# freewym/espresso

Measured on AMD Instinct MI355X. Metric: audio-hours/sec training (LibriSpeech Conformer-12 + CTC), higher is better.
Workload: dtype bf16; 1 GPU; LibriSpeech 960h Conformer-12 + CTC update step, <=26000 frames & <=24 utts per GPU, V=5004, on-GPU fbank+CMVN+SpecAugment, dropout 0.1, clip 2.0, Adam; parallelism=dp1

## Files before the change

### espresso_amd/_lib.py

```python
import ctypes
import os
import re
from typing import Dict, List, Tuple

_HERE = os.path.dirname(os.path.abspath(__file__))
HEADER_PATH = os.path.join(os.path.dirname(_HERE), "include", "espresso_amd.h")
LIB_PATH = os.path.join(_HERE, "csrc", "libespresso_amd.so")


class EspressoAmdLibraryError(RuntimeError):
    pass


class EaGemmParams(ctypes.Structure):
    _fields_ = [
        ("A", ctypes.c_void_p),
        ("B", ctypes.c_void_p),
        ("C", ctypes.c_void_p),
        ("C2", ctypes.c_void_p),
        ("bias", ctypes.c_void_p),
        ("resid", ctypes.c_void_p),
        ("aux", ctypes.c_void_p),
        ("M", ctypes.c_int),
        ("N", ctypes.c_int),
        ("K", ctypes.c_int),
        ("batch", ctypes.c_int),
        ("zdiv", ctypes.c_int),
        ("a_kstrided", ctypes.c_int),
        ("b_kstrided", ctypes.c_int),
        ("c_f32", ctypes.c_int),
        ("accumulate", ctypes.c_int),
        ("resid_f32", ctypes.c_int),
        ("act", ctypes.c_int),
        ("lda", ctypes.c_long),
        ("ldb", ctypes.c_long),
        ("ldc", ctypes.c_long),
        ("ldc2", ctypes.c_long),
        ("ldr", ctypes.c_long),
        ("ldaux", ctypes.c_long),
        ("sA_hi", ctypes.c_long),
        ("sA_lo", ctypes.c_long),
        ("sB_hi", ctypes.c_long),
        ("sB_lo", ctypes.c_long),
        ("sC_hi", ctypes.c_long),
        ("sC_lo", ctypes.c_long),
        ("sR_hi", ctypes.c_long),
        ("sR_lo", ctypes.c_long),
        ("sX_hi", ctypes.c_long),
        ("sX_lo", ctypes.c_long),
        ("alpha", ctypes.c_float),
        ("out_scale", ctypes.c_float),
        ("drop_seed", ctypes.c_uint64),
        ("drop_thr", ctypes.c_uint32),
        ("drop_scale", ctypes.c_float),
        ("splitk", ctypes.c_int),
        ("kchunk", ctypes.c_int),
        ("workspace", ctypes.c_void_p),
        ("q_u", ctypes.c_void_p),
        ("q_v", ctypes.c_void_p),
        ("pos_u", ctypes.c_void_p),
        ("pos_v", ctypes.c_void_p),
        ("ld_q", ctypes.c_long),
        ("qsplit_n", ctypes.c_int),
        ("qscale", ctypes.c_float),
    ]


_F, _V = ctypes.c_void_p, ctypes.c_void_p


def _mk(name, fields):
    return type(name, (ctypes.Structure,), {"_fields_": [(f, ctypes.c_void_p) for f in fields]})


EaFfnParams = _mk("EaFfnParams", ["ln_g", "ln_b", "w1", "b1", "w2", "b2"])
EaFfnGrads = _mk("EaFfnGrads", ["ln_g", "ln_b", "w1", "b1", "w2", "b2"])
EaAttnParams = _mk("EaAttnParams", ["ln_g", "ln_b", "wqkv", "bqkv", "wo", "bo", "pos_u", "pos_v", "wpos"])
EaAttnGrads = _mk("EaAttnGrads", ["ln_g", "ln_b", "wqkv", "bqkv", "wo", "bo", "pos_u", "pos_v", "wpos"])
EaConvParams = _mk("EaConvParams", ["ln_g", "ln_b", "pw1", "dw", "bn_g", "bn_b", "bn_rm", "bn_rv", "pw2"])
EaConvGrads = _mk("EaConvGrads", ["ln_g", "ln_b", "pw1", "dw", "bn_g", "bn_b", "pw2"])


class EaLayerGrads(ctypes.Structure):
    _fields_ = [("ffn1", EaFfnGrads), ("attn", EaAttnGrads), ("conv", EaConvGrads), ("ffn2", EaFfnGrads),
                ("final_ln_g", ctypes.c_void_p), ("final_ln_b", ctypes.c_void_p)]


class EaConformerLayer(ctypes.Structure):
    _fields_ = [("ffn1", EaFfnParams), ("attn", EaAttnParams), ("conv", EaConvParams), ("ffn2", EaFfnParams),
                ("final_ln_g", ctypes.c_void_p), ("final_ln_b", ctypes.c_void_p), ("grads", EaLayerGrads), ("wt", ctypes.c_void_p)]


class EaLayerShape(ctypes.Structure):
    _fields_ = [("B", ctypes.c_int), ("T", ctypes.c_int), ("C", ctypes.c_int), ("H", ctypes.c_int), ("F", ctypes.c_int),
                ("KW", ctypes.c_int), ("training", ctypes.c_int), ("p_drop", ctypes.c_float), ("p_act", ctypes.c_float),
                ("p_attn", ctypes.c_float), ("seed", ctypes.c_uint64), ("has_attn_mask", ctypes.c_int), ("scratch_clean", ctypes.c_int),
                ("pos_mode", ctypes.c_int), ("act", ctypes.c_int), ("S", ctypes.c_int), ("defer", ctypes.c_int), ("wt_fresh", ctypes.c_int)]


class EaLayerChain(ctypes.Structure):
    _fields_ = [("next", ctypes.c_void_p), ("next_saved", ctypes.c_void_p), ("next_saved_bytes", ctypes.c_long), ("ln1_done", ctypes.c_int),
                ("prev", ctypes.c_void_p), ("prev_saved", ctypes.c_void_p), ("prev_saved_bytes", ctypes.c_long),
                ("prev_seed", ctypes.c_uint64), ("prev_pre", ctypes.c_void_p), ("final_ln_done", ctypes.c_int), ("pre_in", ctypes.c_void_p)]


class EaStackLayer(ctypes.Structure):
    _fields_ = [("layer", ctypes.c_void_p), ("shape", EaLayerShape), ("saved", ctypes.c_void_p), ("saved_bytes", ctypes.c_long),
                ("x_in", ctypes.c_void_p)]


class EaWgradProblem(ctypes.Structure):
    _fields_ = [("dy", ctypes.c_void_p), ("x", ctypes.c_void_p), ("dW", ctypes.c_void_p), ("dbias", ctypes.c_void_p),
                ("M", ctypes.c_int), ("N", ctypes.c_int), ("K", ctypes.c_int), ("ld_dy", ctypes.c_long), ("ld_x", ctypes.c_long),
                ("ldw", ctypes.c_long)]


class EaWgradGroup(ctypes.Structure):
    _fields_ = [("count", ctypes.c_int), ("p", EaWgradProblem * 16)]


EaXAttnParams = _mk("EaXAttnParams", ["ln_g", "ln_b", "wq", "bq", "wkv", "bkv", "wo", "bo"])
EaXAttnGrads = _mk("EaXAttnGrads", ["ln_g", "ln_b", "wq", "bq", "wkv", "bkv", "wo", "bo"])


class EaDecoderLayer(ctypes.Structure):
    _fields_ = [("self_attn", EaAttnParams), ("cross", EaXAttnParams), ("ffn", EaFfnParams), ("g_self", EaAttnGrads),
                ("g_cross", EaXAttnGrads), ("g_ffn", EaFfnGrads), ("wt", ctypes.c_void_p)]


_SCALARS = {
    "int": ctypes.c_int,
    "long": ctypes.c_long,
    "float": ctypes.c_float,
    "uint64_t": ctypes.c_uint64,
    "uint32_t": ctypes.c_uint32,
    "ea_stream_t": ctypes.c_void_p,
}


def _ctype_of(decl: str):
    decl = decl.strip()
    if "*" in decl:
        if "EaGemmParams" in decl:
            return ctypes.POINTER(EaGemmParams)
        return ctypes.c_void_p
    toks = [t for t in decl.replace("const", " ").split() if t]
    ty = toks[0]
# ... 50 lines not shown
```

### espresso_amd/csrc/convmodule.hip

```cpp
#include "common.h"
#include "espresso_amd.h"

namespace {

constexpr int KMAX = 31;

__device__ __forceinline__ float sigmoid_f(float x) { return __builtin_amdgcn_rcpf(1.f + __expf(-x)); }

constexpr int CT = 64, TTILE = 64, TPT = TTILE / 4;

template <int KW>
__global__ __launch_bounds__(256) void glu_dwconv_fwd_kernel(const bf16_t* __restrict__ Y,
                                                             const float* __restrict__ w,
                                                             bf16_t* __restrict__ U, bf16_t* __restrict__ Z,
                                                             double* __restrict__ stats, int T, int C) {
  constexpr int PAD = (KW - 1) / 2, ROWS = TTILE + KW - 1;
  __shared__ __attribute__((aligned(16))) float su[ROWS][CT];
  __shared__ float sred[2][4][CT];
  const int c0 = blockIdx.x * CT, t0 = blockIdx.y * TTILE, b = blockIdx.z;
  const long rowbase = (long)b * T;
  if ((C & 7) == 0 && c0 + CT <= C) {
    bf16_t (*sub)[CT] = reinterpret_cast<bf16_t (*)[CT]>(&su[0][0]);
    bf16_t (*sz)[CT] = reinterpret_cast<bf16_t (*)[CT]>(&su[0][0]) + ROWS;
    constexpr int NCH = (ROWS * (CT / 8) + 255) / 256;
// ... 817 lines not shown
        *reinterpret_cast<uint4*>(&tile[wave][r * 128 + (((c8 >> 1) ^ c1_sw(r)) << 5) + (c8 & 1) * 16]) = o;
      }
      uint32_t bh[4], bl[4];
#pragma unroll
      for (int j = 0; j < 8; ++j) {
        const int k = 8 * g4 + j;
        float x = xv[j] ? xs[j] : 0.f;
        if (li == 9 && pb + k < npos) x = 1.f;
        const uint32_t hi = (uint32_t)f2bf(x);
        const uint32_t lo = (uint32_t)f2bf(x - __uint_as_float(hi << 16));
        if (j & 1) { bh[j >> 1] |= hi << 16; bl[j >> 1] |= lo << 16; }
        else { bh[j >> 1] = hi; bl[j >> 1] = lo; }
      }
      __builtin_amdgcn_fence(__ATOMIC_RELEASE, "wavefront");
      __builtin_amdgcn_wave_barrier();
      __builtin_amdgcn_fence(__ATOMIC_ACQUIRE, "wavefront");
      uint32_t ad[8];
      uint2 o8[8];
#pragma unroll
      for (int mt = 0; mt < 4; ++mt)
#pragma unroll
        for (int h = 0; h < 2; ++h) {
          const int r = 8 * g4 + 4 * h + (li >> 2);
          ad[mt * 2 + h] = lds0 + r * 128 + ((mt ^ c1_sw(r)) << 5) + (li & 3) * 8;
        }
      c1_tr_read8(ad, o8);
      const bf16x8_t vbh = __builtin_bit_cast(bf16x8_t, make_uint4(bh[0], bh[1], bh[2], bh[3]));
      const bf16x8_t vbl = __builtin_bit_cast(bf16x8_t, make_uint4(bl[0], bl[1], bl[2], bl[3]));
#pragma unroll
      for (int mt = 0; mt < 4; ++mt) {
        const bf16x8_t a8 = __builtin_bit_cast(bf16x8_t, make_uint4(o8[mt * 2].x, o8[mt * 2].y, o8[mt * 2 + 1].x, o8[mt * 2 + 1].y));
        acc[mt] = __builtin_amdgcn_mfma_f32_16x16x32_bf16(__builtin_bit_cast(__attribute__((ext_vector_type(8))) __bf16, a8),
                                                          __builtin_bit_cast(__attribute__((ext_vector_type(8))) __bf16, vbh), acc[mt], 0, 0, 0);
        acc[mt] = __builtin_amdgcn_mfma_f32_16x16x32_bf16(__builtin_bit_cast(__attribute__((ext_vector_type(8))) __bf16, a8),
                                                          __builtin_bit_cast(__attribute__((ext_vector_type(8))) __bf16, vbl), acc[mt], 0, 0, 0);
      }
      __builtin_amdgcn_wave_barrier();
    }
#pragma unroll
    for (int mt = 0; mt < 4; ++mt)
#pragma unroll
      for (int r = 0; r < 4; ++r) sred[wave][mt * 16 + g4 * 4 + r][li] = acc[mt][r];
    __syncthreads();
    for (int i = threadIdx.x; i < 64 * 10; i += 256) {
      const int c = i / 10, k = i % 10;
      const float a = sred[0][c][k] + sred[1][c][k] + sred[2][c][k] + sred[3][c][k];
      if (k < 9) atomicAdd(dW + (cs + c) * 9 + k, a);
      else if (dbias) atomicAdd(dbias + cs + c, a);
    }
    __syncthreads();
  }
}

__global__ void bn_param_grad_kernel(const float* __restrict__ red, float* __restrict__ dgamma, float* __restrict__ dbeta, int C) {
  const int c = blockIdx.x * blockDim.x + threadIdx.x;
  if (c >= C) return;
  if (dbeta) dbeta[c] += red[c];
  if (dgamma) dgamma[c] += red[C + c];
}
}

static void launch_bn_bwd_reduce(const void* Z, const void* dH, const float* mean_rstd, const float* gamma, const float* beta,
                                 float* red, long M, int C, int act, hipStream_t stream);

extern "C" int ea_bn_act_bwd(const void* Z, const void* dH, const float* mean_rstd, const float* gamma,
                             const float* beta, float* red, void* dZ, float* dgamma, float* dbeta, long M, int C,
                             int act, int training, hipStream_t stream) {
  if (M <= 0) return 0;
  if (C % 8) return -2;
  launch_bn_bwd_reduce(Z, dH, mean_rstd, gamma, beta, red, M, C, act, stream);
  hipLaunchKernelGGL(bn_act_bwd_apply_kernel, dim3(egrid_ch(M * (C / 8), C / 8)), dim3(256), 0, stream, (const bf16_t*)Z,
                     (const bf16_t*)dH, mean_rstd, gamma, beta, red, (bf16_t*)dZ, M, C, act,
                     training ? (float)M : 0.f);
  if (dgamma || dbeta) hipLaunchKernelGGL(bn_param_grad_kernel, dim3((C + 255) / 256), dim3(256), 0, stream, red, dgamma, dbeta, C);
  return EA_CHECK_LAUNCH();
}

extern "C" int ea_bn_act_bwd_fused(const void* Z, const void* dH, const float* mean_rstd, const float* gamma, const float* beta,
                                   float* red, void* dZ, float* dgamma, float* dbeta, long M, int C, int act, int training,
                                   float* zero_next, int zero_n, hipStream_t stream) {
  if (M <= 0) return 0;
  if (C % 8) return -2;
  launch_bn_bwd_reduce(Z, dH, mean_rstd, gamma, beta, red, M, C, act, stream);
  hipLaunchKernelGGL(bn_act_bwd_apply_kernel, dim3(egrid_ch(M * (C / 8), C / 8)), dim3(256), 0, stream, (const bf16_t*)Z,
                     (const bf16_t*)dH, mean_rstd, gamma, beta, red, (bf16_t*)dZ, M, C, act, training ? (float)M : 0.f, dgamma, dbeta,
                     zero_next, zero_n);
  return EA_CHECK_LAUNCH();
}

extern "C" int ea_conv1_bn_bwd(const float* X, const void* Z, const void* dH, const float* mean_rstd, const float* gamma,
                               const float* beta, float* red, float* dgamma, float* dbeta, float* dW, float* dbias, int B, int T,
                               int F, int CO, int sy, int sx, int act, int training, hipStream_t stream) {
  if (B <= 0 || T <= 0) return 0;
  if (CO % 64) return -2;
  const int To = (T - 1) / sy + 1, Fo = (F - 1) / sx + 1;
  const long npos = (long)B * To * Fo;
  launch_bn_bwd_reduce(Z, dH, mean_rstd, gamma, beta, red, npos, CO, act, stream);
  long nb = (npos + 127) / 128;
  if (nb > 1024) nb = 1024;
  hipLaunchKernelGGL(conv1_bn_bwd_wgrad_kernel, dim3((unsigned)nb), dim3(256), 0, stream, X, (const bf16_t*)Z,
                     (const bf16_t*)dH, mean_rstd, gamma, beta, red, dW, dbias, T, F, To, Fo, CO, sy, sx, npos, act,
                     training ? (float)npos : 0.f);
  if (dgamma || dbeta) hipLaunchKernelGGL(bn_param_grad_kernel, dim3((CO + 255) / 256), dim3(256), 0, stream, red, dgamma, dbeta, CO);
  return EA_CHECK_LAUNCH();
}

static void launch_bn_bwd_reduce(const void* Z, const void* dH, const float* mean_rstd, const float* gamma, const float* beta,
                                 float* red, long M, int C, int act, hipStream_t stream) {
  const int nch = C / 8;
  int TCH = 1;
  while (TCH < 256 && TCH < nch) TCH <<= 1;
  const int lanes = 256 / TCH;
  int rpb = 8 * lanes;
  if (rpb < 32) rpb = 32;
  const long gx = (nch + TCH - 1) / TCH;
  const long want = (M + (2048 / gx) - 1) / (2048 / gx > 0 ? 2048 / gx : 1);
  if (want > rpb) rpb = (int)((want + lanes - 1) / lanes * lanes);
  dim3 g1((unsigned)gx, (unsigned)((M + rpb - 1) / rpb));
  hipLaunchKernelGGL(bn_act_bwd_reduce_kernel, g1, dim3(256), (size_t)256 * 16 * sizeof(float), stream, (const bf16_t*)Z,
                     (const bf16_t*)dH, mean_rstd, gamma, beta, red, M, C, act, rpb, TCH);
}
extern "C" int ea_bn_param_grad(const float* red, float* dgamma, float* dbeta, int C, hipStream_t stream) {
  hipLaunchKernelGGL(bn_param_grad_kernel, dim3((C + 255) / 256), dim3(256), 0, stream, red, dgamma, dbeta, C);
  return EA_CHECK_LAUNCH();
}

constexpr int DW_TILES_PER_BLOCK = 2;
static inline int dw_time_blocks(int T) {
  const int nt = (T + TTILE - 1) / TTILE;
  return (nt + DW_TILES_PER_BLOCK - 1) / DW_TILES_PER_BLOCK;
}
extern "C" long ea_dwconv_wgrad_workspace_bytes(int B, int T, int C, int KW) {
  return (long)B * dw_time_blocks(T) * C * KW * (long)sizeof(float);
}

extern "C" int ea_glu_dwconv_bwd(const void* dZ, const void* Y, const void* U, const float* w, void* dY, float* dw,
                                 void* wgrad_ws, int B, int T, int C, int KW, hipStream_t stream) {
  if (B <= 0 || T <= 0) return 0;
  if (C % 2) return -2;
  dim3 grid((C + CT - 1) / CT, (T + TTILE - 1) / TTILE, B);
  EA_KW_DISPATCH(KW, launch_glu_dwconv_bwd_data, grid, stream, (const bf16_t*)dZ, (const bf16_t*)Y, w, (bf16_t*)dY, T, C);
  if (!dw) return EA_CHECK_LAUNCH();
  return ea_dwconv_bwd_weight(dZ, U, dw, wgrad_ws, B, T, C, KW, stream);
}
extern "C" int ea_bn_glu_dwconv_bwd_fused(const void* Z, const void* dH, const float* mean_rstd, const float* gamma, const float* beta,
                                          float* red, void* dZ, float* dgamma, float* dbeta, int act, int training, float* zero_next,
                                          int zero_n, const void* Y, const float* w, void* dY, int B, int T, int C, int KW,
                                          hipStream_t stream) {
  if (B <= 0 || T <= 0) return 0;
  const long M = (long)B * T;
  static const bool fuse = [] { const char* e = getenv("EA_BN_GLU_BWD_FUSED"); return e && e[0] == '1'; }();
  if (!fuse || C % CT != 0) {
    const int rc = ea_bn_act_bwd_fused(Z, dH, mean_rstd, gamma, beta, red, dZ, dgamma, dbeta, M, C, act, training, zero_next, zero_n, stream);
    return rc ? rc : ea_glu_dwconv_bwd(dZ, Y, nullptr, w, dY, nullptr, nullptr, B, T, C, KW, stream);
  }
  launch_bn_bwd_reduce(Z, dH, mean_rstd, gamma, beta, red, M, C, act, stream);
  BnBwdFuse fb{(const bf16_t*)Z, (const bf16_t*)dH, mean_rstd, gamma, beta, red, (bf16_t*)dZ, training ? (float)M : 0.f, act, dgamma, dbeta,
               zero_next, zero_n};
  dim3 grid(C / CT, (T + TTILE - 1) / TTILE, B);
  EA_KW_DISPATCH(KW, launch_glu_dwconv_bwd_data_bn, grid, stream, (const bf16_t*)Y, w, (bf16_t*)dY, T, C, fb);
  return EA_CHECK_LAUNCH();
}
extern "C" int ea_dwconv_bwd_weight(const void* dZ, const void* U, float* dw, void* wgrad_ws, int B, int T, int C, int KW,
                                    hipStream_t stream) {
  if (B <= 0 || T <= 0) return 0;
  dim3 gridw((C + CT - 1) / CT, dw_time_blocks(T), B);
  float* part = (float*)wgrad_ws;
  EA_KW_DISPATCH(KW, launch_dwconv_bwd_weight, gridw, stream, (const bf16_t*)dZ, (const bf16_t*)U, part, T, C, DW_TILES_PER_BLOCK);
  const int nslab = (int)(gridw.y * gridw.z);
  hipLaunchKernelGGL(dwconv_weight_reduce_kernel, dim3((C * KW + 255) / 256, nslab >= 16 ? 8 : 1), dim3(256), 0, stream, part, dw,
                     nslab, C * KW);
  return EA_CHECK_LAUNCH();
}
```

### espresso_amd/csrc/engine.hip

```cpp
#include <hip/hip_runtime.h>
#include <stdint.h>
#include <stdlib.h>
#include <string.h>

#include <functional>
#include <cstdio>
#include <map>
#include <mutex>
#include <vector>

#include "espresso_amd.h"

void ea_gemm_corun_hint(int on);

namespace {

struct Arena {
  char* base;
  size_t off;
  size_t peak;
  template <typename T>
  T* get(size_t n) {
    off = (off + 255) & ~(size_t)255;
    T* p = base ? reinterpret_cast<T*>(base + off) : nullptr;
    off += n * sizeof(T);
    if (off > peak) peak = off;
    return p;
  }
};

inline int pad8(int n) { return (n + 7) / 8 * 8; }
inline int pad_bd(int r) { return (r + 127) / 128 * 128; }

constexpr uint64_t kFfn1 = 0, kAttn = 16, kConv = 32, kCross = 32, kFfn2 = 48;
constexpr uint64_t kAct = 1, kOut = 2, kProbs = 3, kAttnOut = 4, kConvOut = 5;

struct Deferred {
  EaWgradGroup grp;
  EaLnReduceGroup ln;
  std::vector<std::function<int(hipStream_t)>> pre;
  std::vector<std::function<int(hipStream_t)>> ops;
  Deferred() { clear(); }
  void clear() { grp.count = 0; ln.count = 0; pre.clear(); ops.clear(); }
};

struct Ctx {
  hipStream_t s;
  bool dry;
  int rc;
  Arena* scratch;
  hipStream_t side;
  bool overlap;
  Deferred* df = nullptr;
  const EaLayerChain* chain = nullptr;
  bool bits_early = false;
  bool pp_early = false;
};

#define RUN(call)                         \
  do {                                    \
    if (!c.dry && c.rc == 0) c.rc = (call); \
  } while (0)

struct SideRes {
  hipStream_t stream = nullptr;
  hipEvent_t ev[32];
  int next = 0;
  bool ok = false;
  hipEvent_t done[2];
  bool pending[2] = {false, false};
};
static SideRes g_side;
__global__ void ea_queue_probe_spin(long ticks) {
  const long t0 = (long)wall_clock64();
  while ((long)wall_clock64() - t0 < ticks) __builtin_amdgcn_s_sleep(16);
}
__global__ void ea_queue_probe_nop() {}
}
extern "C" int ea_streams_share_queue(hipStream_t a, hipStream_t b) {
  if (a == b) return 1;
  hipEvent_t a0, a1, b1;
  if (hipEventCreate(&a0) != hipSuccess) return -1;
  if (hipEventCreate(&a1) != hipSuccess) { (void)hipEventDestroy(a0); return -1; }
  if (hipEventCreate(&b1) != hipSuccess) { (void)hipEventDestroy(a0); (void)hipEventDestroy(a1); return -1; }
  int rc = -1;
  float spin_ms = 0.f, b_ms = 0.f;
  hipLaunchKernelGGL(ea_queue_probe_nop, dim3(1), dim3(64), 0, b);
  if (hipStreamSynchronize(b) == hipSuccess && hipEventRecord(a0, a) == hipSuccess) {
    hipLaunchKernelGGL(ea_queue_probe_spin, dim3(1), dim3(64), 0, a, 20000L);
// ... 22 lines not shown
  bool ok = false;
  for (int t = 0; t < 8; ++t) {
    hipStream_t cand = nullptr;
    if (hipStreamCreateWithFlags(&cand, hipStreamNonBlocking) != hipSuccess) break;
    const bool unprobed = !g_side_probe || t == 7;
    if (unprobed || ea_streams_share_queue(owner, cand) != 1) {
      g_side.stream = cand;
      g_side_rejected = nrej;
      g_side_unprobed = unprobed ? 1 : 0;
      ok = true;
      break;
    }
    rejected[nrej++] = cand;
  }
  for (int i = 0; i < nrej; ++i) (void)hipStreamDestroy(rejected[i]);
  return ok;
}
static bool side_init(hipStream_t owner) {
  if (g_side.ok) return true;
  int cur = 0, dev = 0;
  if (hipGetDevice(&cur) != hipSuccess) return false;
  dev = cur;
  if (owner != nullptr) {
    hipDevice_t d;
    if (hipStreamGetDevice(owner, &d) == hipSuccess) dev = (int)d;
  }
  if (dev != cur && hipSetDevice(dev) != hipSuccess) return false;
  bool ok = side_stream_create(owner);
  for (auto& e : g_side.ev)
    ok = ok && hipEventCreateWithFlags(&e, hipEventDisableTiming) == hipSuccess;
  for (auto& e : g_side.done)
    ok = ok && hipEventCreateWithFlags(&e, hipEventDisableTiming) == hipSuccess;
  if (dev != cur) (void)hipSetDevice(cur);
  g_side.ok = ok;
  return ok;
}
static inline void stream_wait(Ctx& c, hipStream_t dst, hipStream_t src) {
  if (c.dry || c.rc != 0) return;
  hipEvent_t e = g_side.ev[g_side.next];
  g_side.next = (g_side.next + 1) % 32;
  if (hipEventRecord(e, src) != hipSuccess || hipStreamWaitEvent(dst, e, 0) != hipSuccess) c.rc = -1;
}
static inline void* ln_ws(Ctx& c, int M, int C) {
  return c.scratch->get<char>((size_t)ea_layernorm_bwd_workspace_bytes(M, C));
}
static inline hipStream_t wstream(Ctx& c) { return c.overlap ? c.side : c.s; }
static inline void fork(Ctx& c) { if (c.overlap && !c.df) stream_wait(c, c.side, c.s); }
static inline int join_half(hipStream_t main, int h) {
  if (!g_side.ok || !g_side.pending[h]) return 0;
  g_side.pending[h] = false;
  return hipStreamWaitEvent(main, g_side.done[h], 0) == hipSuccess ? 0 : -1;
}
static inline int join_all(hipStream_t main) {
  const int a = join_half(main, 0), b = join_half(main, 1);
  return a ? a : b;
}
static inline void release(Ctx& c, size_t mark) { if (!c.overlap) c.scratch->off = mark; }

inline uint32_t drop_thr(float p) {
  if (p <= 0.f) return 0;
  double t = (double)p * 4294967296.0;
  return t >= 4294967295.0 ? 4294967295u : (uint32_t)t;
}
inline float drop_scale(float p) { return p <= 0.f ? 1.f : 1.f / (1.f - p); }

struct G {
  EaGemmParams p;
  G(const void* A, const void* B, void* C, int M, int N, int K, long lda, long ldb, long ldc) {
    memset(&p, 0, sizeof(p));
    p.A = A; p.B = B; p.C = C; p.M = M; p.N = N; p.K = K; p.lda = lda; p.ldb = ldb; p.ldc = ldc;
    p.batch = 1; p.zdiv = 1; p.alpha = 1.f; p.out_scale = 1.f; p.splitk = 1; p.drop_scale = 1.f;
  }
  G& aks() { p.a_kstrided = 1; return *this; }
  G& bks() { p.b_kstrided = 1; return *this; }
  G& f32() { p.c_f32 = 1; return *this; }
  G& acc() { p.accumulate = 1; return *this; }
  G& bias(const float* b) { p.bias = b; return *this; }
  G& act(int a) { p.act = a; return *this; }
  G& alpha(float a) { p.alpha = a; return *this; }
  G& scale(float a) { p.out_scale = a; return *this; }
  G& resid(const void* r, long ldr) { p.resid = r; p.ldr = ldr; return *this; }
  G& c2(void* c, long ld) { p.C2 = c; p.ldc2 = ld; return *this; }
  G& aux(const void* x, long ld) { p.aux = x; p.ldaux = ld; return *this; }
  G& drop(float pr, uint64_t seed) { p.drop_thr = drop_thr(pr); p.drop_scale = drop_scale(pr); p.drop_seed = seed; return *this; }
  bool qsplit(void* q_u, void* q_v, const float* pos_u, const float* pos_v, int n, long ld_q, float s) {
    static const bool off = getenv("EA_NO_QSPLIT") != nullptr;
    if (off || n % 128 || p.N % 8) return false;
    p.q_u = q_u; p.q_v = q_v; p.pos_u = pos_u; p.pos_v = pos_v; p.qsplit_n = n; p.ld_q = ld_q; p.qscale = s;
    return true;
  }
  G& batch(int b, int zdiv, long ahi, long alo, long bhi, long blo, long chi, long clo) {
    p.batch = b; p.zdiv = zdiv; p.sA_hi = ahi; p.sA_lo = alo; p.sB_hi = bhi; p.sB_lo = blo; p.sC_hi = chi; p.sC_lo = clo;
    return *this;
  }
};

inline void gemm(Ctx& c, G& g) {
  if (!c.dry && c.rc == 0) ea_gemm_corun_hint(c.overlap || c.df != nullptr);
  RUN(ea_gemm_bf16(&g.p, c.s));
  if (!c.dry) ea_gemm_corun_hint(0);
}
inline void gemm_on(Ctx& c, G& g, hipStream_t st) { RUN(ea_gemm_bf16(&g.p, st)); }

inline void bias_grad(Ctx& c, const void* X, float* out, int M, int N, long ld) {
  if (c.df) {
    if (!c.dry) c.df->ops.push_back([=](hipStream_t st) { return ea_colsum_bf16(X, out, M, N, ld, st); });
    return;
  }
  RUN(ea_colsum_bf16(X, out, M, N, ld, wstream(c)));
}
inline void wgrad(Ctx& c, const void* dy, long ld_dy, const void* x, long ld_x, float* dW, int M, int N_out, int K_in,
                  float* dbias = nullptr) {
  if (c.df && c.df->grp.count < EA_WGRAD_MAX) {
    EaWgradProblem& q = c.df->grp.p[c.df->grp.count++];
    if (c.dry) return;
    q.dy = dy; q.x = x; q.dW = dW; q.dbias = dbias; q.M = M; q.N = N_out; q.K = K_in; q.ld_dy = ld_dy; q.ld_x = ld_x; q.ldw = K_in;
    return;
  }
  const int tiles = ((N_out + 63) / 64) * ((K_in + 127) / 128);
  int sk = 1;
  if (tiles < 384 && M >= 1024) {
    sk = (512 + tiles - 1) / tiles;
    if (sk > M / 256) sk = M / 256;
    if (sk < 1) sk = 1;
  }
  G g(dy, x, dW, N_out, K_in, M, ld_dy, ld_x, K_in);
  g.aks().bks().f32().acc();
  g.p.splitk = sk;
  if (sk > 1) g.p.workspace = c.scratch->get<float>((size_t)sk * N_out * K_in);
  if (c.df) {
    const EaGemmParams gp = g.p;
    if (!c.dry) c.df->ops.push_back([=](hipStream_t st) { return ea_gemm_bf16(&gp, st); });
  } else {
    gemm_on(c, g, wstream(c));
  }
  if (dbias) bias_grad(c, dy, dbias, M, N_out, ld_dy);
}
static bool g_defer_default = true;
static bool g_defer_inline = false;
static void run_deferred(Ctx& c, int half) {
  if (c.dry || !c.df) return;
  Deferred& d = *c.df;
  if (g_defer_inline) {
    RUN(ea_wgrad_group(&d.grp, c.s));
    RUN(ea_layernorm_param_reduce_group(&d.ln, c.s));
    for (auto& op : d.ops) RUN(op(c.s));
    d.clear();
    return;
  }
  stream_wait(c, c.side, c.s);
  for (auto& op : d.pre) RUN(op(c.side));
  RUN(ea_wgrad_group(&d.grp, c.side));
  RUN(ea_layernorm_param_reduce_group(&d.ln, c.side));
  for (auto& op : d.ops) RUN(op(c.side));
  d.clear();
  if (c.rc == 0) {
    if (hipEventRecord(g_side.done[half], c.side) != hipSuccess) c.rc = -1;
    g_side.pending[half] = true;
  }
  if (c.rc == 0) c.rc = join_half(c.s, half ^ 1);
}

}

extern "C" {

struct WT {
  const uint16_t *f1w1, *f2w1, *wqkv, *wo, *pw1, *pw2, *f1w2, *f2w2;
};
static WT wt_view(const EaConformerLayer* L, const EaLayerShape& sh) {
  WT w{nullptr, nullptr, nullptr, nullptr, nullptr, nullptr, nullptr, nullptr};
  if (!L->wt || !sh.training) return w;
  const size_t C = sh.C, F = sh.F;
  const uint16_t* p = (const uint16_t*)L->wt;
  w.f1w1 = p; p += C * F;
  w.f2w1 = p; p += C * F;
  w.wqkv = p; p += 3 * C * C;
  w.wo = p; p += C * C;
  w.pw1 = p; p += 2 * C * C;
  w.pw2 = p; p += C * C;
  w.f1w2 = p; p += C * F;
  w.f2w2 = p;
  return w;
}
static void wt_refresh(Ctx& c, const EaConformerLayer* L, const EaLayerShape& sh) {
  const WT w = wt_view(L, sh);
  if (!w.f1w1) return;
  const int C = sh.C, F = sh.F;
  const void* src[8] = {L->ffn1.w1, L->ffn2.w1, L->attn.wqkv, L->attn.wo, L->conv.pw1, L->conv.pw2, L->ffn1.w2, L->ffn2.w2};
  void* dst[8] = {(void*)w.f1w1, (void*)w.f2w1, (void*)w.wqkv, (void*)w.wo, (void*)w.pw1, (void*)w.pw2, (void*)w.f1w2, (void*)w.f2w2};
  const int rows[8] = {F, F, 3 * C, C, 2 * C, C, C, C}, cols[8] = {C, C, C, C, C, C, F, F};
  RUN(ea_transpose_bf16_batch(src, dst, rows, cols, 8, c.s));
}
struct Pre {
  uint16_t* buf;
  float a;
  uint64_t seed;
  float p;
};
static inline void ln_param_reduce(Ctx& c, void* lnws, float* dg, float* db, int M, int C) {
  if (c.df) {
    if (c.dry) return;
    if (c.df->ln.count < EA_LNRED_MAX) {
      EaLnReduceItem& it = c.df->ln.item[c.df->ln.count++];
      it.workspace = lnws; it.dgamma = dg; it.dbeta = db; it.M = M; it.C = C;
    } else {
      c.df->ops.push_back([=](hipStream_t st) { return ea_layernorm_param_reduce(lnws, dg, db, M, C, st); });
    }
    return;
  }
  fork(c);
  RUN(ea_layernorm_param_reduce(lnws, dg, db, M, C, wstream(c)));
}
static inline void ln_bwd_block(Ctx& c, const void* x, const void* dxn, const float* gamma, const float* mean, const float* rstd,
                                void* dx, float* dg, float* db, int M, int C, const void* dx_add, const Pre& next) {
  void* lnws = ln_ws(c, M, C);
  if (next.buf)
    RUN(ea_layernorm_bwd_dx2(x, dxn, gamma, mean, rstd, dx, dg, db, M, C, dx_add, lnws, next.buf, next.a, next.seed, drop_thr(next.p),
                             drop_scale(next.p), c.s));
  else
    RUN(ea_layernorm_bwd_dx(x, dxn, gamma, mean, rstd, dx, dg, db, M, C, nullptr, 0, 0, 1.f, dx_add, lnws, c.s));
  ln_param_reduce(c, lnws, dg, db, M, C);
// ... 382 lines not shown
    R.cap = cap;
    R.ok = true;
  }
  if (C > R.cap) return nullptr;
  if (R.dirty) {
    const size_t bytes = 2 * (size_t)(2 * R.cap) * (sizeof(double) + sizeof(float));
    if (hipMemsetAsync(R.st[0], 0, bytes, owner) != hipSuccess) return nullptr;
    R.dirty = false;
  }
  return &R;
}

struct ConvSaved {
  float *mean, *rstd, *mr;
  uint16_t *xn, *Y, *U, *Z, *Hh;
};
static ConvSaved conv_saved(Arena& sv, const EaLayerShape& sh) {
  const int M = sh.B * sh.T, C = sh.C;
  ConvSaved s;
  s.mean = sv.get<float>(M);
  s.rstd = sv.get<float>(M);
  s.mr = sv.get<float>(2 * C);
  s.xn = sv.get<uint16_t>((size_t)M * C);
  s.Y = sv.get<uint16_t>((size_t)M * 2 * C);
  s.U = sv.get<uint16_t>((size_t)M * C);
  s.Z = sv.get<uint16_t>((size_t)M * C);
  s.Hh = sv.get<uint16_t>((size_t)M * C);
  return s;
}

static void conv_fwd(Ctx& c, const ConvSaved& s, const EaLayerShape& sh, const EaConvParams& w, const void* x, void* y, uint64_t seed) {
  const int B = sh.B, T = sh.T, C = sh.C, M = B * T;
  Arena& sc = *c.scratch;
  const size_t mark = sc.off;
  RUN(ea_layernorm_fwd(x, w.ln_g, w.ln_b, s.xn, s.mean, s.rstd, M, C, 1e-5f, nullptr, 0, 0, 1.f, c.s));
  G g1(s.xn, w.pw1, s.Y, M, 2 * C, C, C, C, 2 * C);
  gemm(c, g1);
  static const bool bn_fused = getenv("EA_BN_UNFUSED") == nullptr;
  const bool ring = sh.training && bn_fused && C <= 2048;
  BnRing* R = nullptr;
  if (ring && !c.dry && c.rc == 0 && !(R = bn_ring(c.s, C))) c.rc = -1;
  double* stats = nullptr;
  if (sh.training && !ring) {
    stats = sc.get<double>(2 * C);
    if (!c.dry && c.rc == 0) c.rc = hipMemsetAsync(stats, 0, 2 * C * sizeof(double), c.s) == hipSuccess ? 0 : -1;
  }
  if (R && c.rc == 0) stats = R->st[R->si];
  RUN(ea_glu_dwconv_fwd(s.Y, w.dw, s.U, s.Z, stats, B, T, C, sh.KW, c.s));
  if (ring) {
    if (R) {
      if (c.rc == 0) RUN(ea_bn_act_fwd_train(s.Z, stats, s.mr, w.bn_rm, w.bn_rv, w.bn_g, w.bn_b, s.Hh, M, C, EA_ACT_SILU, (float)M, 1e-5f, 0.1f,
                                             R->st[R->si ^ 1], 2 * R->cap, c.s));
      if (c.rc == 0) R->si ^= 1;
      else R->dirty = true;
    }
  } else {
    if (sh.training) RUN(ea_bn_finalize(stats, s.mr, w.bn_rm, w.bn_rv, C, (float)M, 1e-5f, 0.1f, c.s));
    else RUN(ea_bn_from_running(w.bn_rm, w.bn_rv, s.mr, C, 1e-5f, c.s));
    RUN(ea_bn_act_fwd(s.Z, s.mr, w.bn_g, w.bn_b, s.Hh, M, C, EA_ACT_SILU, c.s));
  }
  G g2(s.Hh, w.pw2, y, M, C, C, C, C, C);
  g2.drop(sh.p_drop, seed + kConvOut).resid(x, C);
  gemm(c, g2);
  sc.off = mark;
}

static void conv_bwd(Ctx& c, const ConvSaved& s, const EaLayerShape& sh, const EaConvParams& w, const EaConvGrads& gw, const void* x,
                     const void* dy, void* dx, uint64_t seed, const uint16_t* pw1t, const uint16_t* pw2t, const uint16_t* pre,
                     const Pre& next) {
  const int B = sh.B, T = sh.T, C = sh.C, M = B * T;
  Arena& sc = *c.scratch;
  const size_t mark = sc.off;
  const void* g = dy;
  if (pre) {
    g = pre;
  } else if (sh.p_drop > 0.f) {
    uint16_t* gg = sc.get<uint16_t>((size_t)M * C);
    RUN(ea_scale_dropout_bf16(dy, nullptr, gg, (long)M * C, 1.f, 0.f, seed + kConvOut, drop_thr(sh.p_drop), drop_scale(sh.p_drop), c.s));
    g = gg;
  }
  fork(c);
  wgrad(c, g, C, s.Hh, C, gw.pw2, M, C, C);
  uint16_t* dH = sc.get<uint16_t>((size_t)M * C);
  dgrad(c, g, w.pw2, pw2t, dH, M, C, C);
  static const bool bn_fused = getenv("EA_BN_UNFUSED") == nullptr;
  const bool ring = bn_fused && C <= 2048;
  BnRing* R = nullptr;
  if (ring && !c.dry && c.rc == 0 && !(R = bn_ring(c.s, C))) c.rc = -1;
  float* red = nullptr;
  if (!ring) {
    red = sc.get<float>(2 * C);
    if (!c.dry && c.rc == 0) c.rc = hipMemsetAsync(red, 0, 2 * C * sizeof(float), c.s) == hipSuccess ? 0 : -1;
  }
  uint16_t* dZ = sc.get<uint16_t>((size_t)M * C);
  uint16_t* dY = sc.get<uint16_t>((size_t)M * 2 * C);
  char* wws = sc.get<char>((size_t)ea_dwconv_wgrad_workspace_bytes(B, T, C, sh.KW));
  if (ring) {
    if (R && c.rc == 0) {
      red = R->red[R->ri];
      RUN(ea_bn_glu_dwconv_bwd_fused(s.Z, dH, s.mr, w.bn_g, w.bn_b, red, dZ, gw.bn_g, gw.bn_b, EA_ACT_SILU, sh.training, R->red[R->ri ^ 1],
                                     2 * R->cap, s.Y, w.dw, dY, B, T, C, sh.KW, c.s));
      if (c.rc == 0) R->ri ^= 1;
      else R->dirty = true;
    }
  } else {
    RUN(ea_bn_act_bwd(s.Z, dH, s.mr, w.bn_g, w.bn_b, red, dZ, nullptr, nullptr, M, C, EA_ACT_SILU, sh.training, c.s));
    RUN(ea_glu_dwconv_bwd(dZ, s.Y, s.U, w.dw, dY, nullptr, wws, B, T, C, sh.KW, c.s));
  }
  if (c.df) {
    if (!c.dry) {
      const EaConvGrads gwv = gw;
      const uint16_t* U = s.U;
      const int KW = sh.KW;
      c.df->ops.push_back([=](hipStream_t st) {
        int rc = ring ? 0 : ea_bn_param_grad(red, gwv.bn_g, gwv.bn_b, C, st);
        if (rc == 0) rc = ea_dwconv_bwd_weight(dZ, U, gwv.dw, wws, B, T, C, KW, st);
        return rc;
      });
    }
  } else {
    fork(c);
    if (!ring) RUN(ea_bn_param_grad(red, gw.bn_g, gw.bn_b, C, wstream(c)));
    RUN(ea_dwconv_bwd_weight(dZ, s.U, gw.dw, wws, B, T, C, sh.KW, wstream(c)));
  }
  wgrad(c, dY, 2 * C, s.xn, C, gw.pw1, M, 2 * C, C);
  uint16_t* dxn = sc.get<uint16_t>((size_t)M * C);
  dgrad(c, dY, w.pw1, pw1t, dxn, M, C, 2 * C);
  ln_bwd_block(c, x, dxn, w.ln_g, s.mean, s.rstd, dx, gw.ln_g, gw.ln_b, M, C, dy, next);
  release(c, mark);
}

struct LayerSaved {
  uint16_t *x1, *x2, *x3, *x4;
  FfnSaved f1, f2;
  AttnSaved at;
  ConvSaved cv;
  float *fmean, *frstd;
};
static LayerSaved layer_saved(Arena& sv, const EaLayerShape& sh) {
  const size_t MC = (size_t)sh.B * sh.T * sh.C;
  LayerSaved L;
  L.x1 = sv.get<uint16_t>(MC);
  L.f1 = ffn_saved(sv, sh);
  L.x2 = sv.get<uint16_t>(MC);
  L.at = attn_saved(sv, sh);
  L.x3 = sv.get<uint16_t>(MC);
  L.cv = conv_saved(sv, sh);
  L.x4 = sv.get<uint16_t>(MC);
  L.f2 = ffn_saved(sv, sh);
  L.fmean = sv.get<float>((size_t)sh.B * sh.T);
  L.frstd = sv.get<float>((size_t)sh.B * sh.T);
  return L;
}

static int layer_fwd(Ctx& c, const EaConformerLayer* L, const EaLayerShape& sh, const void* x_in, void* x_out, const int* key_len,
                     const float* attn_mask, const void* pe, Arena& sv) {
  const int M = sh.B * sh.T, C = sh.C;
  LayerSaved S = layer_saved(sv, sh);
  const uint64_t seed = sh.seed;
  const EaLayerChain* ch = c.chain;
  static const bool bits_early = [] { const char* e = getenv("EA_KEEP_BITS_EARLY"); return !(e && e[0] == '0'); }();
  static const bool pp_early = [] { const char* e = getenv("EA_POS_PROJ_EARLY"); return !(e && e[0] == '0'); }();
  if (bits_early) c.bits_early = keep_bits_on_side(c, S.at, sh, seed + kAttn, pp_early ? &L->attn : nullptr, pe);
  ffn_fwd(c, S.f1, sh, L->ffn1, x_in, S.x1, seed + kFfn1, 0.5f, EA_ACT_SILU, ch && ch->ln1_done);
  attn_fwd(c, S.at, sh, L->attn, S.x1, S.x2, key_len, attn_mask, pe, seed + kAttn);
  conv_fwd(c, S.cv, sh, L->conv, S.x2, S.x3, seed + kConv);
  ffn_fwd(c, S.f2, sh, L->ffn2, S.x3, S.x4, seed + kFfn2, 0.5f, EA_ACT_SILU);
  if (ch && ch->next) {
    Arena nsv{(char*)ch->next_saved, 0, 0};
    const LayerSaved N = layer_saved(nsv, sh);
    RUN(ea_layernorm_fwd2(S.x4, L->final_ln_g, L->final_ln_b, x_out, S.fmean, S.frstd, ch->next->ffn1.ln_g, ch->next->ffn1.ln_b, N.f1.xn,
                          N.f1.mean, N.f1.rstd, M, C, 1e-5f, c.s));
  } else {
    RUN(ea_layernorm_fwd(S.x4, L->final_ln_g, L->final_ln_b, x_out, S.fmean, S.frstd, M, C, 1e-5f, nullptr, 0, 0, 1.f, c.s));
  }
  if (!sh.wt_fresh) wt_refresh(c, L, sh);
  return c.rc;
}

static bool g_fuse_predrop = true;
static int layer_bwd(Ctx& c, const EaConformerLayer* L, const EaLayerShape& sh, const void* x_in, const void* dy, void* dx,
                     const int* key_len, const void* pe, Arena& sv) {
  const int M = sh.B * sh.T, C = sh.C;
  LayerSaved S = layer_saved(sv, sh);
// ... 194 lines not shown
  auto flush_group = [&]() {
    if (!grouped) return;
    stream_wait(c, c.side, c.s);
    RUN(ea_wgrad_group(&local.grp, c.side));
    RUN(ea_layernorm_param_reduce_group(&local.ln, c.side));
    for (auto& op : local.ops) RUN(op(c.side));
    local.clear();
  };
  uint16_t* dA = sc.get<uint16_t>((size_t)M * C);
  uint16_t* dB = sc.get<uint16_t>((size_t)M * C);
  uint16_t* pca = dp ? sc.get<uint16_t>((size_t)M * C) : nullptr;
  uint16_t* psa = dp ? sc.get<uint16_t>((size_t)M * C) : nullptr;
  const Pre to_cross{pca, 1.f, seed + kCross + kAttnOut, sh.p_drop}, to_self{psa, 1.f, seed + kAttn + kAttnOut, sh.p_drop}, none{nullptr, 1.f, 0, 0.f};
  ffn_bwd(c, D.f, sh, L->ffn, L->g_ffn, D.x2, dy, dA, seed + kFfn1, 1.f, sh.act, wt.fc1, wt.fc2, nullptr, to_cross);
  {
    const EaXAttnParams& w = L->cross;
    const EaXAttnGrads& gw = L->g_cross;
    const void* g = dp ? (const void*)pca : (const void*)dA;
    fork(c);
    wgrad(c, g, C, D.ca.o, C, gw.wo, M, C, C, gw.bo);
    uint16_t* dO = sc.get<uint16_t>((size_t)M * C);
    dgrad(c, g, w.wo, wt.xo, dO, M, C, C);
    uint16_t* dq = sc.get<uint16_t>((size_t)M * C);
    uint16_t* dkv = sc.get<uint16_t>((size_t)Ms * 2 * C);
    float* Dd = sc.get<float>((size_t)Z * T);
    RUN(ea_flash_attention_bwd(D.ca.qs, nullptr, C, D.ca.kv, D.ca.kv + C, 2 * C, nullptr, 0, enc_len, D.ca.o, dO, C, D.ca.lse, Dd, dq,
                               nullptr, C, nullptr, 0, dkv, dkv + C, 2 * C, H, B, T, S, dh, 0, scaling, seed + kCross + kProbs, drop_thr(sh.p_attn),
                               drop_scale(sh.p_attn), nullptr, nullptr, 0, c.s));
    fork(c);
    wgrad(c, dq, C, D.ca.xn, C, gw.wq, M, C, C, gw.bq);
    wgrad(c, dkv, 2 * C, enc, C, gw.wkv, Ms, 2 * C, C, gw.bkv);
    dgrad(c, dkv, w.wkv, wt.xkv, denc, Ms, C, 2 * C);
    uint16_t* dxn = sc.get<uint16_t>((size_t)M * C);
    dgrad(c, dq, w.wq, wt.xq, dxn, M, C, C);
    ln_bwd_block(c, D.x1, dxn, w.ln_g, D.ca.mean, D.ca.rstd, dB, gw.ln_g, gw.ln_b, M, C, dA, to_self);
  }
  flush_group();
  {
    const EaAttnParams& w = L->self_attn;
    const EaAttnGrads& gw = L->g_self;
    const void* g = dp ? (const void*)psa : (const void*)dB;
    fork(c);
    wgrad(c, g, C, D.sa.o, C, gw.wo, M, C, C, gw.bo);
    uint16_t* dO = sc.get<uint16_t>((size_t)M * C);
    dgrad(c, g, w.wo, wt.wo, dO, M, C, C);
    uint16_t* dqkv = sc.get<uint16_t>((size_t)M * 3 * C);
    float* Dd = sc.get<float>((size_t)Z * T);
    RUN(ea_flash_attention_bwd(D.sa.qs, nullptr, C, D.sa.qkv + C, D.sa.qkv + 2 * C, 3 * C, nullptr, 0, nullptr, D.sa.o, dO, C, D.sa.lse,
                               Dd, dqkv, nullptr, 3 * C, nullptr, 0, dqkv + C, dqkv + 2 * C, 3 * C, H, B, T, T, dh, 1, scaling,
                               seed + kAttn + kProbs, drop_thr(sh.p_attn), drop_scale(sh.p_attn), nullptr, nullptr, 0, c.s));
    fork(c);
    wgrad(c, dqkv, 3 * C, D.sa.xn, C, gw.wqkv, M, 3 * C, C, gw.bqkv);
    uint16_t* dxn = sc.get<uint16_t>((size_t)M * C);
    dgrad(c, dqkv, w.wqkv, wt.wqkv, dxn, M, C, 3 * C);
    ln_bwd_block(c, x_in, dxn, w.ln_g, D.sa.mean, D.sa.rstd, dx, gw.ln_g, gw.ln_b, M, C, dB, none);
  }
  flush_group();
  if (grouped) c.df = nullptr;
  if (c.overlap) stream_wait(c, c.s, c.side);
  return c.rc;
}
static bool darenas_fit(const EaLayerShape& sh, bool backward, bool overlap, long saved_bytes, long scratch_bytes) {
  EaDecoderLayer L;
  memset(&L, 0, sizeof(L));
  Arena sv{nullptr, 0, 0}, sc{nullptr, 0, 0};
  Ctx c{nullptr, true, 0, &sc, nullptr, overlap};
  if (backward) dlayer_bwd(c, &L, sh, nullptr, nullptr, nullptr, nullptr, nullptr, nullptr, sv);
  else dlayer_fwd(c, &L, sh, nullptr, nullptr, nullptr, nullptr, sv);
  return (long)sv.peak <= saved_bytes && (long)sc.peak <= scratch_bytes;
}

static bool g_overlap_default = true;
int ea_set_backward_overlap(int on) {
  const int old = g_overlap_default;
  g_overlap_default = on != 0;
  return old;
}
int ea_set_backward_deferred(int on) {
  const int old = g_defer_default;
  g_defer_default = on != 0;
  return old;
}
int ea_backward_flush(hipStream_t stream) { return join_all(stream); }
int ea_set_backward_deferred_inline(int on) {
  const int old = g_defer_inline;
  g_defer_inline = on != 0;
  return old;
}

static inline bool want_deferred(const EaLayerShape& sh, bool overlap) {
  return overlap && g_defer_default && (sh.defer == 1 || sh.defer == 2);
}
static long scratch_need(const std::function<void(Ctx&)>& walk) {
  Arena sc{nullptr, 0, 0};
  Ctx c{nullptr, true, 0, &sc, nullptr, g_overlap_default};
  walk(c);
  long need = (long)sc.peak + 256;
  if (g_overlap_default && g_defer_default) {
    Arena sd{nullptr, 0, 0};
    Deferred dummy;
    Ctx d{nullptr, true, 0, &sd, nullptr, true};
    d.df = &dummy;
    walk(d);
    const long two = 2 * (((long)sd.peak + 511) & ~255L);
    if (two > need) need = two;
  }
  return need;
}

static bool shape_ok(const EaLayerShape& sh) {
  return sh.B > 0 && sh.T > 0 && sh.C % 8 == 0 && sh.H > 0 && sh.C % sh.H == 0 && sh.F % 8 == 0 && sh.T <= 1024;
}

int ea_conformer_layer_workspace(const EaLayerShape* shape, long* saved_bytes, long* scratch_bytes) {
  if (!shape_ok(*shape)) return -2;
  EaConformerLayer L;
  memset(&L, 0, sizeof(L));
  Arena sv{nullptr, 0, 0};
  EaLayerShape sh = *shape;
  sh.defer = 1;
  *scratch_bytes = scratch_need([&](Ctx& c) {
    Arena a{nullptr, 0, 0}, b{nullptr, 0, 0};
    layer_fwd(c, &L, sh, nullptr, nullptr, nullptr, nullptr, nullptr, a);
    layer_bwd(c, &L, sh, nullptr, nullptr, nullptr, nullptr, nullptr, b);
    if (a.peak > sv.peak) sv.peak = a.peak;
  });
  *saved_bytes = (long)sv.peak + 256;
  return 0;
}

static bool arenas_fit(const EaLayerShape& sh, bool backward, bool overlap, long saved_bytes, long scratch_bytes, bool transformer = false,
                       bool deferred = false) {
  EaConformerLayer L;
  memset(&L, 0, sizeof(L));
  Arena sv{nullptr, 0, 0}, sc{nullptr, 0, 0};
  Ctx c{nullptr, true, 0, &sc, nullptr, overlap};
  Deferred dummy;
  if (deferred) c.df = &dummy;
  if (transformer) {
    if (backward) tlayer_bwd(c, &L, sh, nullptr, nullptr, nullptr, nullptr, nullptr, nullptr, sv);
    else tlayer_fwd(c, &L, sh, nullptr, nullptr, nullptr, nullptr, nullptr, sv);
  } else if (backward) layer_bwd(c, &L, sh, nullptr, nullptr, nullptr, nullptr, nullptr, sv);
  else layer_fwd(c, &L, sh, nullptr, nullptr, nullptr, nullptr, nullptr, sv);
  return (long)sv.peak <= saved_bytes && (long)sc.peak <= scratch_bytes;
}

static int bwd_deferred(const EaConformerLayer* layer, const EaLayerShape& sh, const void* x_in, const void* dy, void* dx,
                        const int* key_len, const void* pe, float* dpe, void* saved, long saved_bytes, void* scratch,
                        long scratch_bytes, hipStream_t stream, bool transformer, const EaLayerChain* chain = nullptr) {
  static Deferred df;
  const int half = sh.defer - 1;
  const long half_bytes = (scratch_bytes / 2) & ~255L;
  if (!arenas_fit(sh, true, true, saved_bytes, half_bytes, transformer, true)) return -5;
  if (join_half(stream, half) != 0) return -1;
  Arena sv{(char*)saved, 0, 0}, sc{(char*)scratch + (size_t)half * half_bytes, 0, 0};
  Ctx c{stream, false, 0, &sc, g_side.stream, true};
  df.clear();
  c.df = &df;
  c.chain = chain;
  return transformer ? tlayer_bwd(c, layer, sh, x_in, dy, dx, key_len, pe, dpe, sv) : layer_bwd(c, layer, sh, x_in, dy, dx, key_len, pe, sv);
}

static int chain_ok(const EaLayerShape& sh, const EaLayerChain* ch, bool backward) {
  if (!ch) return 0;
  if ((ch->next || ch->prev || ch->ln1_done || ch->final_ln_done) && sh.C > 512) return -2;
  if (!backward && ch->next && (!ch->next_saved || !arenas_fit(sh, false, false, ch->next_saved_bytes, 1L << 60))) return -5;
// ... 219 lines not shown
```

### espresso_amd/csrc/gemm.hip

```cpp
#include <cstdio>
#include <type_traits>
#include "common.h"
#include "espresso_amd.h"
#include "gemm_common.h"
#include "gemm_epilogue.h"

int ea_gemm_w8_try(const EaGemmParams& q, int nt_flag, hipStream_t stream, int* cfg_out);
int ea_wgrad_w8_try(const EaWgradGroup& g, hipStream_t stream, int* grid_out, EaWgradGroup* rest);
static thread_local int g_gemm_corun = 0;
void ea_gemm_corun_hint(int on) { g_gemm_corun = on; }
static const int g_w8_corun = [] { const char* e = getenv("EA_GEMM_W8_CORUN"); return e ? atoi(e) : 1; }();

namespace {

constexpr int BM = 128, BN = 128;

__device__ __forceinline__ void load_kc(const bf16_t* __restrict__ p, long ld, int rows, int K,
                                        int row0, int k0, int tid, uint4 (&r)[4]) {
  const int c = tid & 7;
  const int gk = k0 + c * 8;
#pragma unroll
  for (int i = 0; i < 4; ++i) {
    const int row = row0 + (tid >> 3) + 32 * i;
    uint4 v = make_uint4(0, 0, 0, 0);
// ... 74 lines not shown
    uint4 v = make_uint4(0, 0, 0, 0);
    if (gk < K && grow < rows) {
      const bf16_t* q = p + (long)gk * ld + grow;
      if (grow + 8 <= rows && (((uintptr_t)q) & 15) == 0) {
        v = *reinterpret_cast<const uint4*>(q);
      } else {
        bf16_t t[8];
#pragma unroll
        for (int e = 0; e < 8; ++e) t[e] = (grow + e < rows) ? q[e] : (bf16_t)0;
        v.x = t[0] | ((uint32_t)t[1] << 16);
        v.y = t[2] | ((uint32_t)t[3] << 16);
        v.z = t[4] | ((uint32_t)t[5] << 16);
        v.w = t[6] | ((uint32_t)t[7] << 16);
      }
    }
    r[j] = v;
  }
}
__device__ __forceinline__ void store_ks_at(char* __restrict__ s, int r0, int kk0, const uint4 (&r)[4]) {
  const uint32_t w0[4] = {r[0].x, r[0].y, r[0].z, r[0].w};
  const uint32_t w1[4] = {r[1].x, r[1].y, r[1].z, r[1].w};
  const uint32_t w2[4] = {r[2].x, r[2].y, r[2].z, r[2].w};
  const uint32_t w3[4] = {r[3].x, r[3].y, r[3].z, r[3].w};
#pragma unroll
  for (int d = 0; d < 4; ++d) {
    uint2 lo, hi;
    lo.x = (w0[d] & 0xffffu) | (w1[d] << 16);
    lo.y = (w2[d] & 0xffffu) | (w3[d] << 16);
    hi.x = (w0[d] >> 16) | (w1[d] & 0xffff0000u);
    hi.y = (w2[d] >> 16) | (w3[d] & 0xffff0000u);
    const int ra = r0 + 2 * d, rb = ra + 1;
    *reinterpret_cast<uint2*>(s + lds_off(ra, kk0 >> 3) + (kk0 & 4) * 2) = lo;
    *reinterpret_cast<uint2*>(s + lds_off(rb, kk0 >> 3) + (kk0 & 4) * 2) = hi;
  }
}
template <int NI>
__device__ __forceinline__ void load_kc_n(const bf16_t* __restrict__ p, long ld, int rows, int K, int row0, int k0, int tid,
                                          uint4 (&r)[4]) {
  const int c = tid & 7;
  const int gk = k0 + c * 8;
#pragma unroll
  for (int i = 0; i < NI; ++i) {
    const int row = row0 + (tid >> 3) + 32 * i;
    uint4 v = make_uint4(0, 0, 0, 0);
    if (row < rows && gk < K) {
      const bf16_t* q = p + (long)row * ld + gk;
      if (gk + 8 <= K && (((uintptr_t)q) & 15) == 0) {
        v = *reinterpret_cast<const uint4*>(q);
      } else {
        bf16_t t[8];
#pragma unroll
        for (int e = 0; e < 8; ++e) t[e] = (gk + e < K) ? q[e] : (bf16_t)0;
        v.x = t[0] | ((uint32_t)t[1] << 16);
        v.y = t[2] | ((uint32_t)t[3] << 16);
        v.z = t[4] | ((uint32_t)t[5] << 16);
        v.w = t[6] | ((uint32_t)t[7] << 16);
      }
    }
    r[i] = v;
  }
}

__device__ __forceinline__ void load_kc_fast(const bf16_t* __restrict__ base, long ld, int k0, uint4 (&r)[4]) {
#pragma unroll
  for (int i = 0; i < 4; ++i) r[i] = *reinterpret_cast<const uint4*>(base + (long)(32 * i) * ld + k0);
}
__device__ __forceinline__ void load_ks_fast(const bf16_t* __restrict__ base, long ld, int k0, uint4 (&r)[4]) {
#pragma unroll
  for (int j = 0; j < 4; ++j) r[j] = *reinterpret_cast<const uint4*>(base + (long)(k0 + j) * ld);
}

template <int BM_, bool FAST>
__device__ __forceinline__ void gemm_tile_epilogue(const EaGemmParams& p, const f32x4_t (&acc)[4][BM_ == 128 ? 4 : 2], float* sC, int m0,
                                                   int n0, int z, int ks_id, int zhi, int zlo, long coff, int xcd_swizzle) {
  constexpr int NJ = BM_ == 128 ? 4 : 2;
  const int tid = threadIdx.x, lane = tid & 63, wave = tid >> 6;
  const int wm = BM_ == 128 ? (wave >> 1) : 0;
  const int wcol = BM_ == 128 ? (wave & 1) * 64 : wave * 32;
  const bool vec_ok = (p.ldc & 7) == 0 && (((uintptr_t)p.C) & 15) == 0 && ((p.sC_hi | p.sC_lo) & 7) == 0;
  float bias8[8];
  load_bias8(p, n0 + (tid & 15) * 8, bias8);
  float posu8[8], posv8[8];
  load_pos8(p, n0 + (tid & 15) * 8, posu8, posv8);
  const int pre_kind = !FAST ? 0 : p.resid ? 1 : p.aux ? 2 : 0;
  const bf16_t* pre_base = pre_kind == 1 ? reinterpret_cast<const bf16_t*>(p.resid) : reinterpret_cast<const bf16_t*>(p.aux);
  const long pre_ld = pre_kind == 1 ? p.ldr : p.ldaux;
#pragma unroll
  for (int half = 0; half < BM_ / 64; ++half) {
    uint4 pre0 = uint4{0, 0, 0, 0}, pre1 = pre0, pre2 = pre0, pre3 = pre0;
    if (FAST && pre_kind) {
      const bf16_t* q = pre_base + n0 + (tid & 15) * 8;
      const int mr = m0 + half * 64 + (tid >> 4), ml = p.M - 1;
      pre0 = *reinterpret_cast<const uint4*>(q + (long)min(mr, ml) * pre_ld);
      pre1 = *reinterpret_cast<const uint4*>(q + (long)min(mr + 16, ml) * pre_ld);
      pre2 = *reinterpret_cast<const uint4*>(q + (long)min(mr + 32, ml) * pre_ld);
      pre3 = *reinterpret_cast<const uint4*>(q + (long)min(mr + 48, ml) * pre_ld);
    }
    __syncthreads();
    if (half == 0) EA_STAMP(5);
    if (wm == half) {
#pragma unroll
      for (int i = 0; i < 4; ++i)
#pragma unroll
        for (int j = 0; j < NJ; ++j)
#pragma unroll
          for (int r = 0; r < 4; ++r)
            sC[(i * 16 + (lane >> 4) * 4 + r) * BN + wcol + j * 16 + (lane & 15)] = acc[i][j][r];
    }
    __syncthreads();
    if (half == 0) EA_STAMP(6);
    if (m0 + half * 64 < p.M) {
#pragma unroll 1
      for (int pass = 0; pass < 4; ++pass) {
        const int rl = pass * 16 + (tid >> 4);
        const int m = m0 + half * 64 + rl;
        const int n = n0 + (tid & 15) * 8;
        if (m < p.M && (FAST || n < p.N)) {
          float v[8];
          const float4 x0 = *reinterpret_cast<const float4*>(sC + rl * BN + (tid & 15) * 8);
          const float4 x1 = *reinterpret_cast<const float4*>(sC + rl * BN + (tid & 15) * 8 + 4);
          v[0] = x0.x; v[1] = x0.y; v[2] = x0.z; v[3] = x0.w; v[4] = x1.x; v[5] = x1.y; v[6] = x1.z; v[7] = x1.w;
          epilogue_chunk<FAST>(p, z, ks_id, zhi, zlo, coff, m, n, v, bias8, posu8, posv8, vec_ok, (xcd_swizzle & 2) != 0, pre_kind, pre0);
        }
        pre0 = pre1; pre1 = pre2; pre2 = pre3;
      }
    }
  }
}

template <bool A_KS, bool B_KS, int BM_, bool FAST = false>
__global__ __launch_bounds__(256, 3) void gemm_bf16_kernel(const EaGemmParams p, const int xcd_swizzle) {
  constexpr int NJ = BM_ == 128 ? 4 : 2;
  __shared__ __attribute__((aligned(16))) char smem[2 * BM * ROW_BYTES];
  char* sA = smem;
  char* sB = smem + BM * ROW_BYTES;
  EA_STAMP(0);

  const int tid = threadIdx.x;
  const int lane = tid & 63, wave = tid >> 6;
  const int wm = BM_ == 128 ? (wave >> 1) : 0;
  const int wcol = BM_ == 128 ? (wave & 1) * 64 : wave * 32;
  int tile_x = blockIdx.x, tile_y = blockIdx.y, tile_z = blockIdx.z;
  if (xcd_swizzle & 1) {
    const int gx = gridDim.x, gxy = gridDim.x * gridDim.y, total = gxy * gridDim.z;
    const int lin = (blockIdx.z * gridDim.y + blockIdx.y) * gx + blockIdx.x;
    const int xcd = lin & 7, q = total >> 3, r = total & 7;
    const int v = (xcd < r ? xcd * (q + 1) : r * (q + 1) + (xcd - r) * q) + (lin >> 3);
    tile_z = FAST ? 0 : v / gxy;
    const int rem = v - tile_z * gxy;
    tile_y = rem / gx;
    tile_x = rem - tile_y * gx;
  }
  const int m0 = tile_y * BM_, n0 = tile_x * BN;
  const int z = FAST ? 0 : tile_z / p.splitk;
  const int ks_id = FAST ? 0 : tile_z % p.splitk;
  const int zhi = FAST ? 0 : z / p.zdiv, zlo = FAST ? 0 : z % p.zdiv;

  const bf16_t* A = reinterpret_cast<const bf16_t*>(p.A) + (long)zhi * p.sA_hi + (long)zlo * p.sA_lo;
  const bf16_t* B = reinterpret_cast<const bf16_t*>(p.B) + (long)zhi * p.sB_hi + (long)zlo * p.sB_lo;
  const long coff = (long)zhi * p.sC_hi + (long)zlo * p.sC_lo;

  const int kbeg = ks_id * p.kchunk;
  const int kend = min(p.K, kbeg + p.kchunk);

  f32x4_t acc[4][NJ];
#pragma unroll
  for (int i = 0; i < 4; ++i)
#pragma unroll
    for (int j = 0; j < NJ; ++j) acc[i][j] = (f32x4_t){0.f, 0.f, 0.f, 0.f};

  uint4 ra[4], rb[4];
  const int nk = kend > kbeg ? (kend - kbeg + BK - 1) / BK : 0;
  const bool a_ok = (m0 + BM_ <= p.M) && (p.lda & 7) == 0 && ((uintptr_t)A & 15) == 0 && (!A_KS || (m0 & 7) == 0);
  const bool b_ok = (n0 + BN <= p.N) && (p.ldb & 7) == 0 && ((uintptr_t)B & 15) == 0 && (!B_KS || (n0 & 7) == 0);
  const int a_kq = BM_ == 128 ? (tid >> 4) : (tid >> 3);
  const int a_rc = BM_ == 128 ? (tid & 15) : (tid & 7);
  const bool a_ks_active = BM_ == 128 || tid < 128;
  const bf16_t* a_base = A_KS ? A + (long)(a_kq * 4) * p.lda + m0 + a_rc * 8 : A + (long)(m0 + (tid >> 3)) * p.lda + (tid & 7) * 8;
  const bf16_t* b_base = B_KS ? B + (long)((tid >> 4) * 4) * p.ldb + n0 + (tid & 15) * 8
                              : B + (long)(n0 + (tid >> 3)) * p.ldb + (tid & 7) * 8;
  auto loadA = [&](int k0, uint4 (&ra)[4]) {
    if (A_KS) {
      if (!a_ks_active) return;
      if (a_ok && k0 + BK <= kend) load_ks_fast(a_base, p.lda, k0, ra);
      else load_ks_at(A, p.lda, p.M, kend, m0 + a_rc * 8, k0 + a_kq * 4, ra);
    } else {
      if (a_ok && k0 + BK <= kend) {
#pragma unroll
        for (int i = 0; i < BM_ / 32; ++i) ra[i] = *reinterpret_cast<const uint4*>(a_base + (long)(32 * i) * p.lda + k0);
      } else {
        load_kc_n<BM_ / 32>(A, p.lda, p.M, kend, m0, k0, tid, ra);
      }
    }
  };
  auto loadB = [&](int k0, uint4 (&rb)[4]) {
    if (b_ok && k0 + BK <= kend) { if (B_KS) load_ks_fast(b_base, p.ldb, k0, rb); else load_kc_fast(b_base, p.ldb, k0, rb); }
    else { if (B_KS) load_ks(B, p.ldb, p.N, kend, n0, k0, tid, rb); else load_kc(B, p.ldb, p.N, kend, n0, k0, tid, rb); }
  };
  auto storeA = [&](const uint4 (&ra)[4]) {
    if (A_KS) {
      if (a_ks_active) store_ks_at(sA, a_rc * 8, a_kq * 4, ra);
    } else {
#pragma unroll
      for (int i = 0; i < BM_ / 32; ++i) *reinterpret_cast<uint4*>(sA + lds_off((tid >> 3) + 32 * i, tid & 7)) = ra[i];
    }
  };
  if (nk > 0) {
    loadA(kbeg, ra);
    loadB(kbeg, rb);
// ... 622 lines not shown
  if (!f) return -1;
  for (auto& r : g_prof) {
    hipEventSynchronize(r.e1);
    float t = 0.f;
    hipEventElapsedTime(&t, r.e0, r.e1);
    fprintf(f, "%d %d %d %d %d %d %d %d %d %.6f\n", r.M, r.N, r.K, r.batch, r.a_ks, r.b_ks, r.splitk, r.bm64, r.epi, t);
  }
  fclose(f);
  return (long)g_prof.size();
}

static long g_nt_store_min_bytes = 0;
extern "C" long ea_set_gemm_nt_store_min_bytes(long bytes) {
  const long old = g_nt_store_min_bytes;
  g_nt_store_min_bytes = bytes;
  return old;
}
static inline int nt_flag(const EaGemmParams& q) {
  return (g_nt_store_min_bytes > 0 && !q.c_f32 && q.splitk <= 1 && 2L * q.M * q.N * q.batch >= g_nt_store_min_bytes) ? 2 : 0;
}
static int g_xcd_swizzle = 3;
extern "C" int ea_set_gemm_xcd_swizzle(int mask) {
  const int old = g_xcd_swizzle;
  g_xcd_swizzle = mask;
  return old;
}
static int g_gemm_variant = 0;
extern "C" int ea_set_gemm_variant(int v) {
  const int old = g_gemm_variant;
  g_gemm_variant = v;
  return old;
}

static int g_gemm_glds = [] { const char* e = getenv("EA_GEMM_GLDS"); return e ? atoi(e) : 1; }();
extern "C" int ea_set_gemm_glds(int stages) {
  const int old = g_gemm_glds;
  g_gemm_glds = stages;
  return old;
}
static int g_fast_epi = [] { const char* e = getenv("EA_GEMM_FAST_EPI"); return e ? atoi(e) : 1; }();
static bool fast_epilogue_ok(const EaGemmParams& q) {
  auto al = [](const void* p) { return (reinterpret_cast<uintptr_t>(p) & 15) == 0; };
  return g_fast_epi && !q.c_f32 && q.splitk == 1 && q.batch == 1 && !q.resid_f32 && q.N % 128 == 0 && (q.ldc & 7) == 0 && al(q.C) &&
         ((q.sC_hi | q.sC_lo) & 7) == 0 && (!q.bias || al(q.bias)) &&
         (!q.aux || ((q.ldaux & 7) == 0 && al(q.aux) && ((q.sX_hi | q.sX_lo) & 7) == 0)) &&
         (!q.resid || ((q.ldr & 7) == 0 && al(q.resid) && ((q.sR_hi | q.sR_lo) & 7) == 0)) &&
         (!q.C2 || ((q.ldc2 & 7) == 0 && al(q.C2))) &&
         (!q.q_u || ((q.ld_q & 7) == 0 && al(q.q_u) && al(q.q_v) && al(q.pos_u) && al(q.pos_v)));
}
static bool w8_ragged_ok(const EaGemmParams& q) {
  auto al = [](const void* p) { return (reinterpret_cast<uintptr_t>(p) & 15) == 0; };
  return g_fast_epi && !q.c_f32 && q.splitk == 1 && q.batch == 1 && !q.resid && !q.aux && !q.C2 && !q.q_u && q.N % 4 == 0 &&
         (q.ldc & 7) == 0 && q.ldc >= (q.N + 31) / 32 * 32 && al(q.C) && (!q.bias || al(q.bias));
}
template <int BM_, int NST>
static bool launch_glds(dim3 grid, hipStream_t stream, const EaGemmParams& q, int sw) {
  constexpr int bytes = NST * (BM_ + BN) * ROW_BYTES;
  static bool attr_ok = hipFuncSetAttribute(reinterpret_cast<const void*>(&gemm_glds_kernel<BM_, NST>),
                                            hipFuncAttributeMaxDynamicSharedMemorySize, bytes) == hipSuccess &&
                        hipFuncSetAttribute(reinterpret_cast<const void*>(&gemm_glds_kernel<BM_, NST, true>),
                                            hipFuncAttributeMaxDynamicSharedMemorySize, bytes) == hipSuccess;
  if (!attr_ok) return false;
  if (fast_epilogue_ok(q)) hipLaunchKernelGGL((gemm_glds_kernel<BM_, NST, true>), grid, dim3(256), bytes, stream, q, sw);
  else hipLaunchKernelGGL((gemm_glds_kernel<BM_, NST>), grid, dim3(256), bytes, stream, q, sw);
  return true;
}
static bool glds_eligible(const EaGemmParams& q) {
  return !q.a_kstrided && !q.b_kstrided && q.K % BK == 0 && q.kchunk % BK == 0 && (q.lda & 7) == 0 && (q.ldb & 7) == 0 &&
         ((q.sA_hi | q.sA_lo | q.sB_hi | q.sB_lo) & 7) == 0 && ((reinterpret_cast<uintptr_t>(q.A) | reinterpret_cast<uintptr_t>(q.B)) & 15) == 0;
}

template <bool A_KS, bool B_KS>
static void launch_gemm(dim3 grid, bool bm64, hipStream_t stream, const EaGemmParams& q) {
  const int sw = ((g_xcd_swizzle & 2) && grid.x <= 16 && (long)grid.x * grid.y * grid.z >= 64 ? 1 : 0) | nt_flag(q);
  if (!A_KS && !B_KS && fast_epilogue_ok(q)) {
    if (bm64) hipLaunchKernelGGL((gemm_bf16_kernel<false, false, 64, true>), grid, dim3(256), 0, stream, q, sw);
    else hipLaunchKernelGGL((gemm_bf16_kernel<false, false, 128, true>), grid, dim3(256), 0, stream, q, sw);
    return;
  }
  if (bm64) hipLaunchKernelGGL((gemm_bf16_kernel<A_KS, B_KS, 64>), grid, dim3(256), 0, stream, q, sw);
  else hipLaunchKernelGGL((gemm_bf16_kernel<A_KS, B_KS, 128>), grid, dim3(256), 0, stream, q, sw);
}

extern "C" long ea_gemm_splitk_workspace_bytes(int M, int N, int batch, int splitk) {
  return splitk > 1 ? (long)splitk * batch * M * N * (long)sizeof(float) : 0;
}

extern "C" int ea_gemm_bf16(const EaGemmParams* pp, hipStream_t stream) {
  const EaGemmParams& p = *pp;
  if (p.M <= 0 || p.N <= 0 || p.batch <= 0) return 0;
  if (p.K <= 0 || p.zdiv <= 0) return -2;
  EaGemmParams q = p;
  if (q.splitk < 1) q.splitk = 1;
  if (q.q_u) {
    if (q.qsplit_n <= 0 || q.qsplit_n % 128 || q.qsplit_n > q.N || q.N % 8 || q.batch != 1 || q.splitk > 1 || q.c_f32 || q.ld_q < q.qsplit_n)
      return -4;
  } else {
    q.qsplit_n = 0;
  }
  if (q.splitk > 1) {
    if (!q.c_f32 || q.bias || q.resid || q.aux || q.C2 || q.act != EA_ACT_NONE || q.drop_thr || !q.workspace) return -4;
    int chunk = (q.K + q.splitk - 1) / q.splitk;
    chunk = (chunk + BK - 1) / BK * BK;
    q.kchunk = chunk;
    q.splitk = (q.K + chunk - 1) / chunk;
  } else {
    q.kchunk = q.K;
  }
  const long tiles128 = (long)((q.N + BN - 1) / BN) * ((q.M + BM - 1) / BM) * q.batch * q.splitk;
  static const long bm_thr = [] { const char* e = getenv("EA_GEMM_BM_THR"); return e ? atol(e) : 1536L; }();
  const bool bm64 = g_gemm_variant == 2 ? true : (g_gemm_variant == 1 ? false : (tiles128 < bm_thr));
  const int bm = bm64 ? 64 : BM;
  dim3 grid((q.N + BN - 1) / BN, (q.M + bm - 1) / bm, q.batch * q.splitk), block(256);
  GemmProf pr;
  pr.bm64 = bm64;
  if (g_prof_on) {
    hipEventCreate(&pr.e0);
    hipEventCreate(&pr.e1);
    pr.flops = 2.0 * q.M * q.N * (double)q.K * q.batch;
    pr.M = q.M; pr.N = q.N; pr.K = q.K; pr.batch = q.batch; pr.a_ks = q.a_kstrided; pr.b_ks = q.b_kstrided;
    pr.splitk = q.splitk;
    pr.epi = (q.bias ? 1 : 0) | (q.resid ? 2 : 0) | (q.aux ? 4 : 0) | (q.C2 ? 8 : 0) | (q.act != EA_ACT_NONE ? 16 : 0) |
             (q.drop_thr ? 32 : 0) | (q.c_f32 ? 64 : 0);
    const double mn = (double)q.M * q.N * q.batch;
    pr.bytes = 2.0 * q.batch * ((double)q.M * q.K + (double)q.N * q.K) + mn * (q.splitk > 1 ? 4.0 * q.splitk : (q.c_f32 ? 4.0 : 2.0)) +
               (q.resid ? 2.0 * mn : 0.0) + (q.aux ? 2.0 * mn : 0.0) + (q.C2 ? 2.0 * mn : 0.0);
    hipEventRecord(pr.e0, stream);
  }
  bool done = false;
  const bool kc_ok = glds_eligible(q);
  if (kc_ok && (fast_epilogue_ok(q) || w8_ragged_ok(q)) && (!g_gemm_corun || g_w8_corun)) {
    int cfg = 0;
    if (ea_gemm_w8_try(q, nt_flag(q), stream, &cfg)) {
      done = true;
      pr.bm64 = 100 + cfg;
    }
  }
  if (!done && g_gemm_glds && kc_ok) {
    const int sw = (((g_xcd_swizzle & 1) && grid.x <= 16 && (long)grid.x * grid.y * grid.z >= 64 && (grid.x > 1 || grid.z > 1)) ? 1 : 0) | nt_flag(q);
    int nst = g_gemm_glds;
    if (nst == 1) {
      const long blocks = (long)grid.x * grid.y * grid.z;
      const int nkt = q.kchunk / BK;
      nst = (blocks <= 512 && nkt >= 4) ? 3 : (nkt >= 16 ? 2 : 0);
    }
    if (nst == 0) {
    } else if (nst == 2) done = bm64 ? launch_glds<64, 2>(grid, stream, q, sw) : launch_glds<128, 2>(grid, stream, q, sw);
    else if (nst == 4) done = bm64 ? launch_glds<64, 4>(grid, stream, q, sw) : launch_glds<128, 4>(grid, stream, q, sw);
    else done = bm64 ? launch_glds<64, 3>(grid, stream, q, sw) : launch_glds<128, 3>(grid, stream, q, sw);
  }
  if (done) {
  } else if (p.a_kstrided) {
    if (p.b_kstrided) launch_gemm<true, true>(grid, bm64, stream, q); else launch_gemm<true, false>(grid, bm64, stream, q);
  } else {
    if (p.b_kstrided) launch_gemm<false, true>(grid, bm64, stream, q); else launch_gemm<false, false>(grid, bm64, stream, q);
  }
  if (g_prof_on) {
    hipEventRecord(pr.e1, stream);
    g_prof.push_back(pr);
  }
  if (q.splitk > 1) {
    const long per = (long)q.batch * q.M * q.N;
    const bool vec = (q.N % 4 == 0) && (q.ldc % 4 == 0) && (q.sC_hi % 4 == 0) && (q.sC_lo % 4 == 0) &&
                     ((reinterpret_cast<uintptr_t>(q.C) & 15) == 0) && ((reinterpret_cast<uintptr_t>(q.workspace) & 15) == 0);
    long blocks = (per / (vec ? 4 : 1) + 255) / 256;
    if (blocks > 4096) blocks = 4096;
    if (blocks < 1) blocks = 1;
    if (vec) hipLaunchKernelGGL(splitk_reduce_kernel<true>, dim3((unsigned)blocks), dim3(256), 0, stream, q);
    else hipLaunchKernelGGL(splitk_reduce_kernel<false>, dim3((unsigned)blocks), dim3(256), 0, stream, q);
  }
  return EA_CHECK_LAUNCH();
}

static int g_wgrad_tr = [] { const char* e = getenv("EA_WGRAD_TR"); return e ? atoi(e) : 1; }();
extern "C" int ea_set_wgrad_transposing_reads(int on) {
  const int old = g_wgrad_tr;
  g_wgrad_tr = on;
  return old;
}
extern "C" int ea_wgrad_group(const EaWgradGroup* gp, hipStream_t stream) {
  const EaWgradGroup& g = *gp;
  if (g.count <= 0) return 0;
// ... 89 lines not shown
```

### espresso_amd/csrc/gemm_epilogue.h

```cpp
#pragma once
#include "common.h"
#include "espresso_amd.h"
#include "gemm_common.h"

namespace {

__device__ __forceinline__ void load8_bf16(const bf16_t* q, bool vec, int cnt, float (&o)[8]) {
  if (vec) {
    const uint4 u = *reinterpret_cast<const uint4*>(q);
    const uint32_t w[4] = {u.x, u.y, u.z, u.w};
#pragma unroll
    for (int e = 0; e < 4; ++e) {
      o[2 * e] = __uint_as_float(w[e] << 16);
      o[2 * e + 1] = __uint_as_float(w[e] & 0xffff0000u);
    }
  } else {
#pragma unroll
    for (int e = 0; e < 8; ++e) o[e] = e < cnt ? bf2f(q[e]) : 0.f;
  }
}
__device__ __forceinline__ void unpack8_bf16(const uint4& u, float (&o)[8]) {
  const uint32_t w[4] = {u.x, u.y, u.z, u.w};
#pragma unroll
  for (int e = 0; e < 4; ++e) {
    o[2 * e] = __uint_as_float(w[e] << 16);
    o[2 * e + 1] = __uint_as_float(w[e] & 0xffff0000u);
  }
}
typedef uint32_t u32x4_t __attribute__((ext_vector_type(4)));
__device__ __forceinline__ void store8_bf16(bf16_t* q, bool vec, int cnt, const float (&v)[8], bool nt = false) {
  if (vec) {
    u32x4_t u;
    u.x = pack_bf2(v[0], v[1]); u.y = pack_bf2(v[2], v[3]); u.z = pack_bf2(v[4], v[5]); u.w = pack_bf2(v[6], v[7]);
    if (nt) __builtin_nontemporal_store(u, reinterpret_cast<u32x4_t*>(q));
    else *reinterpret_cast<u32x4_t*>(q) = u;
  } else {
#pragma unroll
    for (int e = 0; e < 8; ++e) if (e < cnt) q[e] = f2bf(v[e]);
  }
}

__device__ __forceinline__ void load_bias8(const EaGemmParams& p, int n, float (&b)[8]) {
#pragma unroll
  for (int e = 0; e < 8; ++e) b[e] = 0.f;
  if (!p.bias || n >= p.N) return;
  if (n + 8 <= p.N && (((uintptr_t)p.bias) & 15) == 0) {
    const float4 x0 = *reinterpret_cast<const float4*>(p.bias + n);
    const float4 x1 = *reinterpret_cast<const float4*>(p.bias + n + 4);
    b[0] = x0.x; b[1] = x0.y; b[2] = x0.z; b[3] = x0.w; b[4] = x1.x; b[5] = x1.y; b[6] = x1.z; b[7] = x1.w;
  } else {
#pragma unroll
    for (int e = 0; e < 8; ++e) if (n + e < p.N) b[e] = p.bias[n + e];
  }
}

__device__ __forceinline__ void load_pos8(const EaGemmParams& p, int n, float (&u)[8], float (&w)[8]) {
#pragma unroll
  for (int e = 0; e < 8; ++e) u[e] = w[e] = 0.f;
  if (!p.q_u || n >= p.qsplit_n) return;
  const bool al = ((((uintptr_t)p.pos_u) | ((uintptr_t)p.pos_v)) & 15) == 0;
  if (p.pos_u) {
    if (al) {
      const float4 x0 = *reinterpret_cast<const float4*>(p.pos_u + n), x1 = *reinterpret_cast<const float4*>(p.pos_u + n + 4);
      u[0] = x0.x; u[1] = x0.y; u[2] = x0.z; u[3] = x0.w; u[4] = x1.x; u[5] = x1.y; u[6] = x1.z; u[7] = x1.w;
    } else {
#pragma unroll
      for (int e = 0; e < 8; ++e) u[e] = p.pos_u[n + e];
    }
  }
  if (p.pos_v) {
    if (al) {
      const float4 x0 = *reinterpret_cast<const float4*>(p.pos_v + n), x1 = *reinterpret_cast<const float4*>(p.pos_v + n + 4);
      w[0] = x0.x; w[1] = x0.y; w[2] = x0.z; w[3] = x0.w; w[4] = x1.x; w[5] = x1.y; w[6] = x1.z; w[7] = x1.w;
    } else {
#pragma unroll
      for (int e = 0; e < 8; ++e) w[e] = p.pos_v[n + e];
    }
  }
}

template <bool FAST = false>
__device__ __forceinline__ void epilogue_chunk(const EaGemmParams& p, int z, int ks_id, int zhi, int zlo, long coff, int m,
                                               int n, float (&v)[8], const float (&bias8)[8], const float (&posu8)[8],
                                               const float (&posv8)[8], bool vec_ok, bool nt = false, int pre_kind = 0,
                                               uint4 pre = uint4{0, 0, 0, 0}) {
  const int cnt = FAST ? 8 : min(8, p.N - n);
  const bool vec = FAST ? true : (vec_ok && cnt == 8);
  const bool has_drop = p.drop_thr != 0;
#pragma unroll
  for (int e = 0; e < 8; ++e) v[e] = v[e] * p.alpha + bias8[e];
  if (p.q_u && n < p.qsplit_n) {
    float u8[8], b8[8];
#pragma unroll
    for (int e = 0; e < 8; ++e) {
      const float q = __uint_as_float((uint32_t)f2bf(v[e]) << 16);
      u8[e] = (q + posu8[e]) * p.qscale;
      b8[e] = (q + posv8[e]) * p.qscale;
    }
    const bool qvec = FAST ? true : ((p.ld_q & 7) == 0 && ((((uintptr_t)p.q_u) | ((uintptr_t)p.q_v)) & 15) == 0);
    store8_bf16(reinterpret_cast<bf16_t*>(p.q_u) + (long)m * p.ld_q + n, qvec, 8, u8, nt);
    if (p.q_v) store8_bf16(reinterpret_cast<bf16_t*>(p.q_v) + (long)m * p.ld_q + n, qvec, 8, b8, nt);
    return;
  }
  const uint64_t didx = ((uint64_t)z * (uint64_t)p.M + (uint64_t)m) * (uint64_t)p.N + (uint64_t)n;
  const long co = coff + (long)m * p.ldc + n;
  if (!FAST && p.splitk > 1) {
    float* W = reinterpret_cast<float*>(p.workspace) + (((long)ks_id * p.batch + z) * p.M + m) * (long)p.N + n;
    if (cnt == 8 && (p.N & 3) == 0) {
      *reinterpret_cast<float4*>(W) = make_float4(v[0], v[1], v[2], v[3]);
      *reinterpret_cast<float4*>(W + 4) = make_float4(v[4], v[5], v[6], v[7]);
    } else {
#pragma unroll
      for (int e = 0; e < 8; ++e) if (e < cnt) W[e] = v[e];
    }
    return;
  }
  float keep8[8];
  if (has_drop) {
    ea_keep8(p.drop_seed, didx, p.drop_thr, p.drop_scale, keep8);
  } else {
#pragma unroll
    for (int e = 0; e < 8; ++e) keep8[e] = 1.f;
  }
  if (p.aux) {
    float zz[8];
    if (FAST && pre_kind == 2) unpack8_bf16(pre, zz);
    else
    load8_bf16(reinterpret_cast<const bf16_t*>(p.aux) + (long)zhi * p.sX_hi + (long)zlo * p.sX_lo + (long)m * p.ldaux + n,
               FAST ? true : (vec && (p.ldaux & 7) == 0 && ((((uintptr_t)p.aux) & 15) == 0) && (((p.sX_hi | p.sX_lo) & 7) == 0)), cnt, zz);
#pragma unroll
    for (int e = 0; e < 8; ++e) v[e] *= keep8[e];
    mul_dact8(v, zz, p.act);
  } else {
    if (p.C2) {
      store8_bf16(reinterpret_cast<bf16_t*>(p.C) + co, vec, cnt, v, true);
      apply_act8(v, p.act);
#pragma unroll
      for (int e = 0; e < 8; ++e) v[e] *= keep8[e];
      store8_bf16(reinterpret_cast<bf16_t*>(p.C2) + coff + (long)m * p.ldc2 + n,
                  FAST ? true : (vec && (p.ldc2 & 7) == 0 && ((((uintptr_t)p.C2) & 15) == 0)), cnt, v, nt);
      return;
    }
    apply_act8(v, p.act);
#pragma unroll
    for (int e = 0; e < 8; ++e) v[e] *= keep8[e];
  }
#pragma unroll
  for (int e = 0; e < 8; ++e) v[e] *= p.out_scale;
  if (p.resid) {
    const long ro = (long)zhi * p.sR_hi + (long)zlo * p.sR_lo + (long)m * p.ldr + n;
    if (!FAST && p.resid_f32) {
      const float* r = reinterpret_cast<const float*>(p.resid) + ro;
      if (cnt == 8 && ((((uintptr_t)r) & 15) == 0)) {
        const float4 r0 = *reinterpret_cast<const float4*>(r), r1 = *reinterpret_cast<const float4*>(r + 4);
        v[0] += r0.x; v[1] += r0.y; v[2] += r0.z; v[3] += r0.w; v[4] += r1.x; v[5] += r1.y; v[6] += r1.z; v[7] += r1.w;
      } else {
#pragma unroll
        for (int e = 0; e < 8; ++e) if (e < cnt) v[e] += r[e];
      }
    } else {
      float rr[8];
// ... 28 lines not shown
```

### espresso_amd/csrc/gemm_w8.hip

```cpp
#include "common.h"
#include "espresso_amd.h"
#include "gemm_common.h"
#include "gemm_epilogue.h"
#include "gemm_w8_common.h"

static int g_gemm_w8 = [] { const char* e = getenv("EA_GEMM_W8"); return e ? atoi(e) : 1; }();
static long g_w8_many = [] { const char* e = getenv("EA_GEMM_W8_MANY"); return e ? atol(e) : 1024L; }();

namespace {

enum { W8_PLAIN = 0, W8_QSPLIT = 1, W8_ACT2 = 2, W8_AUX = 3, W8_RESID = 4 };

__device__ __forceinline__ void ea_keep4(uint64_t seed, uint64_t idx0, uint32_t thr, float inv_keep, float (&k)[4]) {
  const uint32_t lo = (uint32_t)idx0;
  if (__builtin_expect(lo > 0xFFFFFFFBu, 0)) {
#pragma unroll
    for (int e = 0; e < 4; ++e) k[e] = ea_keep(seed, idx0 + (uint64_t)e, thr, inv_keep);
    return;
  }
  const uint32_t hi = ((uint32_t)(idx0 >> 32) * 0x85EBCA77u) ^ (uint32_t)(seed >> 32) ^ ((uint32_t)seed * 0xC2B2AE3Du);
  const uint32_t x0 = lo * 0x9E3779B1u + (uint32_t)seed;
#pragma unroll
  for (int e = 0; e < 4; ++e) {
    uint32_t x = x0 + (uint32_t)e * 0x9E3779B1u;
    x ^= x >> 16;
    x *= 0x85EBCA6Bu;
    x ^= hi;
    x ^= x >> 13;
    x *= 0xC2B2AE35u;
    x ^= x >> 16;
    k[e] = x >= thr ? inv_keep : 0.f;
  }
}
__device__ __forceinline__ void unpack4_bf16(uint32_t w0, uint32_t w1, float (&o)[4]) {
  o[0] = __uint_as_float(w0 << 16); o[1] = __uint_as_float(w0 & 0xffff0000u);
  o[2] = __uint_as_float(w1 << 16); o[3] = __uint_as_float(w1 & 0xffff0000u);
}
template <int KIND, int MI, int NJ>
__device__ __forceinline__ void w8_reg_epilogue(const EaGemmParams& p, const f32x4_t (&acc)[MI][NJ], int m0, int n0, int row0, int col0, bool nt) {
  static_assert(NJ % 2 == 0, "tiles are stored in pairs");
  const int lane = threadIdx.x & 63, g = lane >> 4, r16 = lane & 15;
  const int nown = n0 + col0 + g * 4;
  const int npair = n0 + col0 + (g & 1) * 16 + (g >> 1) * 8;
  const bool has_drop = p.drop_thr != 0;
  float bias4[NJ][4];
#pragma unroll
  for (int j = 0; j < NJ; ++j) {
    float4 b = make_float4(0.f, 0.f, 0.f, 0.f);
    if (p.bias && nown + j * 16 < p.N) b = *reinterpret_cast<const float4*>(p.bias + nown + j * 16);
    bias4[j][0] = b.x; bias4[j][1] = b.y; bias4[j][2] = b.z; bias4[j][3] = b.w;
  }
  float posu4[KIND == W8_QSPLIT ? NJ : 1][4], posv4[KIND == W8_QSPLIT ? NJ : 1][4];
  if (KIND == W8_QSPLIT) {
#pragma unroll
    for (int j = 0; j < NJ; ++j) {
      float4 u = make_float4(0.f, 0.f, 0.f, 0.f), w = u;
      if (nown + j * 16 < p.qsplit_n) {
        if (p.pos_u) u = *reinterpret_cast<const float4*>(p.pos_u + nown + j * 16);
        if (p.pos_v) w = *reinterpret_cast<const float4*>(p.pos_v + nown + j * 16);
      }
      posu4[j][0] = u.x; posu4[j][1] = u.y; posu4[j][2] = u.z; posu4[j][3] = u.w;
      posv4[j][0] = w.x; posv4[j][1] = w.y; posv4[j][2] = w.z; posv4[j][3] = w.w;
    }
  }
  constexpr bool HAS_OP = KIND == W8_AUX || KIND == W8_RESID;
  const bf16_t* op_base = KIND == W8_AUX ? reinterpret_cast<const bf16_t*>(p.aux) : reinterpret_cast<const bf16_t*>(p.resid);
  const long op_ld = KIND == W8_AUX ? p.ldaux : p.ldr;
  uint4 opn[HAS_OP ? NJ / 2 : 1], opc[HAS_OP ? NJ / 2 : 1];
  auto fetch_ops = [&](int i) {
    const int mc = min(m0 + row0 + i * 16 + r16, p.M - 1);
#pragma unroll
    for (int jp = 0; jp < NJ / 2; ++jp) {
      const int nc = min(npair + jp * 32, p.N - 8);
      opn[jp] = *reinterpret_cast<const uint4*>(op_base + (long)mc * op_ld + nc);
    }
  };
  if (HAS_OP) fetch_ops(0);
#pragma unroll
  for (int i = 0; i < MI; ++i) {
    const int m = m0 + row0 + i * 16 + r16;
    const bool mv = m < p.M;
    if (HAS_OP) {
#pragma unroll
      for (int jp = 0; jp < NJ / 2; ++jp) opc[jp] = opn[jp];
      if (i + 1 < MI) fetch_ops(i + 1);
    }
#pragma unroll
    for (int jp = 0; jp < NJ / 2; ++jp) {
      if (n0 + col0 + jp * 32 >= p.N) continue;
      const int ns = npair + jp * 32;
      float opnd[2][4];
      if (HAS_OP) {
        const uint4 L = opc[jp];
        const auto s0 = __builtin_amdgcn_permlane16_swap(L.x, L.z, false, false);
        const auto s1 = __builtin_amdgcn_permlane16_swap(L.y, L.w, false, false);
        unpack4_bf16(s0[0], s1[0], opnd[0]);
        unpack4_bf16(s0[1], s1[1], opnd[1]);
      }
      uint2 out[2], out2[2];
#pragma unroll
      for (int t = 0; t < 2; ++t) {
        const int j = 2 * jp + t;
        const int n = nown + j * 16;
        float v[4];
#pragma unroll
        for (int e = 0; e < 4; ++e) v[e] = acc[i][j][e] * p.alpha + bias4[j][e];
        if (KIND == W8_QSPLIT && n0 + col0 + jp * 32 < p.qsplit_n) {
          float u4[4], b4[4];
#pragma unroll
          for (int e = 0; e < 4; ++e) {
            const float q = __uint_as_float((uint32_t)f2bf(v[e]) << 16);
            u4[e] = (q + posu4[KIND == W8_QSPLIT ? j : 0][e]) * p.qscale;
            b4[e] = (q + posv4[KIND == W8_QSPLIT ? j : 0][e]) * p.qscale;
          }
          out[t] = make_uint2(pack_bf2(u4[0], u4[1]), pack_bf2(u4[2], u4[3]));
          out2[t] = make_uint2(pack_bf2(b4[0], b4[1]), pack_bf2(b4[2], b4[3]));
          continue;
        }
        float keep4[4];
        if (has_drop) {
          ea_keep4(p.drop_seed, (uint64_t)m * (uint64_t)p.N + (uint64_t)n, p.drop_thr, p.drop_scale, keep4);
        } else {
#pragma unroll
          for (int e = 0; e < 4; ++e) keep4[e] = 1.f;
        }
        if (KIND == W8_AUX) {
#pragma unroll
          for (int e = 0; e < 4; ++e) v[e] *= keep4[e];
          if (p.act == EA_ACT_SILU) {
#pragma unroll
            for (int e = 0; e < 4; ++e) v[e] *= dsilu_f(opnd[t][e]);
          } else if (p.act == EA_ACT_RELU) {
#pragma unroll
            for (int e = 0; e < 4; ++e) v[e] *= opnd[t][e] > 0.f ? 1.f : 0.f;
          }
        } else {
          if (KIND == W8_ACT2) out2[t] = make_uint2(pack_bf2(v[0], v[1]), pack_bf2(v[2], v[3]));
          if (p.act == EA_ACT_SILU) {
#pragma unroll
            for (int e = 0; e < 4; ++e) v[e] = silu_f(v[e]);
          } else if (p.act == EA_ACT_RELU) {
#pragma unroll
            for (int e = 0; e < 4; ++e) v[e] = fmaxf(v[e], 0.f);
          }
#pragma unroll
          for (int e = 0; e < 4; ++e) v[e] *= keep4[e];
        }
        if (KIND != W8_ACT2) {
#pragma unroll
          for (int e = 0; e < 4; ++e) v[e] *= p.out_scale;
          if (KIND == W8_RESID) {
#pragma unroll
            for (int e = 0; e < 4; ++e) v[e] += opnd[t][e];
          }
        }
        out[t] = make_uint2(pack_bf2(v[0], v[1]), pack_bf2(v[2], v[3]));
      }
      const u32x4_t o = w8_swap_pair(out[0], out[1]);
      if (KIND == W8_QSPLIT && n0 + col0 + jp * 32 < p.qsplit_n) {
        const u32x4_t o2 = w8_swap_pair(out2[0], out2[1]);
        if (mv) {
          w8_store16(reinterpret_cast<bf16_t*>(p.q_u) + (long)m * p.ld_q + ns, o, nt);
          if (p.q_v) w8_store16(reinterpret_cast<bf16_t*>(p.q_v) + (long)m * p.ld_q + ns, o2, nt);
        }
      } else if (KIND == W8_ACT2) {
        const u32x4_t o2 = w8_swap_pair(out2[0], out2[1]);
        if (mv) {
          w8_store16(reinterpret_cast<bf16_t*>(p.C) + (long)m * p.ldc + ns, o2, true);
          w8_store16(reinterpret_cast<bf16_t*>(p.C2) + (long)m * p.ldc2 + ns, o, nt);
        }
      } else if (mv) {
        w8_store16(reinterpret_cast<bf16_t*>(p.C) + (long)m * p.ldc + ns, o, nt);
      }
    }
  }
}

template <int BM_, int BN_, int WM_, int WN_, int NST, int PIPE, int KIND>
__global__ __launch_bounds__(512, 2) void gemm_w8_kernel(const EaGemmParams p, const int tiles_n, const int flags) {
  extern __shared__ __attribute__((aligned(16))) char dsm[];
  constexpr int TM = BM_ / WM_, TN = BN_ / WN_, MI = TM / 16, NJ = TN / 16;
  constexpr int A_BYTES = BM_ * 128, STAGE = (BM_ + BN_) * 128;
  constexpr int NA = BM_ / 64, NB = BN_ / 64;
  static_assert(WM_ * WN_ == 8 && NST >= 2, "eight wavefronts");
  EA_STAMP(0);
  const int tid = threadIdx.x;
  const int lane = tid & 63;
  const int wave = __builtin_amdgcn_readfirstlane(tid >> 6);
  const int wm = wave / WN_, wn = wave % WN_;
  int tile = blockIdx.x;
  if (flags & 1) {
    const int total = gridDim.x, xcd = tile & 7, q = total >> 3, r = total & 7;
    tile = (xcd < r ? xcd * (q + 1) : r * (q + 1) + (xcd - r) * q) + (tile >> 3);
  }
  const int tile_y = tile / tiles_n, tile_x = tile - tile_y * tiles_n;
  const int m0 = tile_y * BM_, n0 = tile_x * BN_;
  const bf16_t* A = reinterpret_cast<const bf16_t*>(p.A);
  const bf16_t* B = reinterpret_cast<const bf16_t*>(p.B);
  const int nk = p.K / BK;

  f32x4_t acc[MI][NJ];
#pragma unroll
  for (int i = 0; i < MI; ++i)
#pragma unroll
    for (int j = 0; j < NJ; ++j) acc[i][j] = (f32x4_t){0.f, 0.f, 0.f, 0.f};

  const int src_chunk = (lane & 7) ^ (lane >> 3);
  const bf16_t* ap[NA];
  const bf16_t* bp[NB];
#pragma unroll
  for (int i = 0; i < NA; ++i) ap[i] = A + (long)min(m0 + (wave + 8 * i) * 8 + (lane >> 3), p.M - 1) * p.lda + src_chunk * 8;
#pragma unroll
  for (int i = 0; i < NB; ++i) bp[i] = B + (long)min(n0 + (wave + 8 * i) * 8 + (lane >> 3), p.N - 1) * p.ldb + src_chunk * 8;
  typedef const __attribute__((address_space(1))) void* gptr_t;
  typedef __attribute__((address_space(3))) void* lptr_t;
  auto issue = [&](int stage, int kt) {
    char* base = dsm + stage * STAGE + wave * 1024;
#pragma unroll
    for (int i = 0; i < NA; ++i) __builtin_amdgcn_global_load_lds((gptr_t)(ap[i] + (long)kt * BK), (lptr_t)(base + i * 8192), 16, 0, 0);
#pragma unroll
    for (int i = 0; i < NB; ++i)
      __builtin_amdgcn_global_load_lds((gptr_t)(bp[i] + (long)kt * BK), (lptr_t)(base + A_BYTES + i * 8192), 16, 0, 0);
  };
  uint32_t a_base[2], b_base[2];
#pragma unroll
  for (int ks = 0; ks < 2; ++ks) {
    a_base[ks] = w8_off(wm * TM + (lane & 15), ks * 4 + (lane >> 4));
    b_base[ks] = A_BYTES + w8_off(wn * TN + (lane & 15), ks * 4 + (lane >> 4));
  }

#pragma unroll
  for (int s = 0; s < NST - 1; ++s)
    if (s < nk) issue(s, s);
  int stage = 0, fill = NST - 1;
  for (int kt = 0; kt < nk; ++kt) {
    if (kt + NST - 2 < nk) w8_wait_vmcnt<(NST - 2) * (NA + NB)>();
    else w8_wait_vmcnt<0>();
    __builtin_amdgcn_s_barrier();
    if (kt == 0) EA_STAMP(1);
    if (kt == 4) EA_STAMP(7);
    if (kt + NST - 1 < nk) issue(fill, kt + NST - 1);
    const char* st = dsm + stage * STAGE;
    if constexpr (PIPE == 0) {
#pragma unroll
      for (int ks = 0; ks < 2; ++ks) {
        bf16x8_t af[MI], bfr[NJ];
#pragma unroll
        for (int j = 0; j < NJ; ++j) bfr[j] = *reinterpret_cast<const bf16x8_t*>(st + b_base[ks] + j * 2048);
#pragma unroll
        for (int i = 0; i < MI; ++i) af[i] = *reinterpret_cast<const bf16x8_t*>(st + a_base[ks] + i * 2048);
#pragma unroll
        for (int i = 0; i < MI; ++i)
#pragma unroll
          for (int j = 0; j < NJ; ++j)
            acc[i][j] = __builtin_amdgcn_mfma_f32_16x16x32_bf16(
                __builtin_bit_cast(__attribute__((ext_vector_type(8))) __bf16, bfr[j]),
                __builtin_bit_cast(__attribute__((ext_vector_type(8))) __bf16, af[i]), acc[i][j], 0, 0, 0);
      }
    } else {
      constexpr int AG = NJ >= 4 ? 2 : (MI >= 4 ? 4 : MI);
      constexpr int GPK = MI / AG, NG = 2 * GPK;
      bf16x8_t bq[2][NJ], aq[2][AG];
#pragma unroll
      for (int j = 0; j < NJ; ++j) bq[0][j] = *reinterpret_cast<const bf16x8_t*>(st + b_base[0] + j * 2048);
#pragma unroll
      for (int a = 0; a < AG; ++a) aq[0][a] = *reinterpret_cast<const bf16x8_t*>(st + a_base[0] + a * 2048);
#pragma unroll
      for (int g = 0; g < NG; ++g) {
        if (g + 1 < NG) {
          const int ks1 = (g + 1) / GPK, gi = (g + 1) % GPK;
          if (gi == 0) {
#pragma unroll
            for (int j = 0; j < NJ; ++j) bq[ks1][j] = *reinterpret_cast<const bf16x8_t*>(st + b_base[ks1] + j * 2048);
          }
#pragma unroll
          for (int a = 0; a < AG; ++a) aq[(g + 1) & 1][a] = *reinterpret_cast<const bf16x8_t*>(st + a_base[ks1] + (gi * AG + a) * 2048);
        }
        const int ks = g / GPK, gi0 = g % GPK;
#pragma unroll
        for (int a = 0; a < AG; ++a)
#pragma unroll
          for (int j = 0; j < NJ; ++j)
            acc[gi0 * AG + a][j] = __builtin_amdgcn_mfma_f32_16x16x32_bf16(
                __builtin_bit_cast(__attribute__((ext_vector_type(8))) __bf16, bq[ks][j]),
                __builtin_bit_cast(__attribute__((ext_vector_type(8))) __bf16, aq[g & 1][a]), acc[gi0 * AG + a][j], 0, 0, 0);
      }
      __builtin_amdgcn_sched_group_barrier(0x100, NJ + AG, 0);
      w8_sched_groups<NG, GPK, AG, NJ>();
    }
    stage = stage + 1 == NST ? 0 : stage + 1;
    fill = fill + 1 == NST ? 0 : fill + 1;
  }
  EA_STAMP(2);
  w8_reg_epilogue<KIND, MI, NJ>(p, acc, m0, n0, wm * TM, wn * TN, (flags & 2) != 0);
  EA_STAMP(3);
}

template <int BM_, int BN_, int WM_, int WN_, int NST, int PIPE, int KIND>
bool w8_launch_kind(const EaGemmParams& q, int flags, hipStream_t stream) {
  constexpr int bytes = NST * (BM_ + BN_) * 128;
  static const bool attr_ok = hipFuncSetAttribute(reinterpret_cast<const void*>(&gemm_w8_kernel<BM_, BN_, WM_, WN_, NST, PIPE, KIND>),
                                                  hipFuncAttributeMaxDynamicSharedMemorySize, bytes) == hipSuccess;
  if (!attr_ok) return false;
  const int tiles_n = (q.N + BN_ - 1) / BN_, tiles_m = (q.M + BM_ - 1) / BM_;
  hipLaunchKernelGGL((gemm_w8_kernel<BM_, BN_, WM_, WN_, NST, PIPE, KIND>), dim3(tiles_n * tiles_m), dim3(512), bytes, stream, q, tiles_n, flags);
  return true;
}
int w8_kind(const EaGemmParams& q) {
  if (q.q_u) {
    static const bool qs = [] { const char* e = getenv("EA_GEMM_W8_QSPLIT"); return e && e[0] == '1'; }();
    if (g_gemm_w8 == 1 && !qs) return -1;
    return (q.aux || q.C2 || q.resid || q.drop_thr || q.act != EA_ACT_NONE || q.out_scale != 1.f) ? -1 : W8_QSPLIT;
  }
  if (q.C2) return (q.aux || q.resid) ? -1 : W8_ACT2;
  if (q.aux) return q.resid ? -1 : W8_AUX;
  return q.resid ? W8_RESID : W8_PLAIN;
}
template <int BM_, int BN_, int WM_, int WN_, int NST, int PIPE>
bool w8_launch(const EaGemmParams& q, int flags, hipStream_t stream) {
  switch (w8_kind(q)) {
    case W8_PLAIN: return w8_launch_kind<BM_, BN_, WM_, WN_, NST, PIPE, W8_PLAIN>(q, flags, stream);
    case W8_QSPLIT: return w8_launch_kind<BM_, BN_, WM_, WN_, NST, PIPE, W8_QSPLIT>(q, flags, stream);
    case W8_ACT2: return w8_launch_kind<BM_, BN_, WM_, WN_, NST, PIPE, W8_ACT2>(q, flags, stream);
    case W8_AUX: return w8_launch_kind<BM_, BN_, WM_, WN_, NST, PIPE, W8_AUX>(q, flags, stream);
    case W8_RESID: return w8_launch_kind<BM_, BN_, WM_, WN_, NST, PIPE, W8_RESID>(q, flags, stream);
    default: return false;
  }
}

}

extern "C" int ea_set_gemm_w8(int mode) {
  const int old = g_gemm_w8;
  g_gemm_w8 = mode;
  return old;
}

int ea_gemm_w8_try(const EaGemmParams& q, int nt_flag, hipStream_t stream, int* cfg_out) {
  if (!g_gemm_w8) return 0;
  if ((long)q.M * q.lda >= (1L << 31) || (long)q.N * q.ldb >= (1L << 31)) return 0;
  int cfg = g_gemm_w8;
  if (cfg == 1) {
    const long rm256 = (q.M + 255) / 256, rm128 = (q.M + 127) / 128, cn256 = (q.N + 255) / 256, cn128 = (q.N + 127) / 128;
    auto fits = [](long tiles) { return tiles > 128 && tiles <= 256; };
    const bool whole = q.N % 128 == 0;
    if (whole && fits(rm256 * cn256)) cfg = 2;
    else if (whole && fits(rm256 * cn128)) cfg = 4;
    else if (whole && fits(rm128 * cn256)) cfg = 5;
    else if (whole && fits(rm128 * cn128)) cfg = 3;
    else if (rm256 * cn256 >= g_w8_many && q.N >= 1024) cfg = 2;
    else return 0;
  }
  const int flags = 1 | nt_flag;
  bool ok = false;
  switch (cfg) {
    case 2: ok = w8_launch<256, 256, 2, 4, 2, 1>(q, flags, stream); break;
    case 3: ok = w8_launch<128, 128, 2, 4, 4, 1>(q, flags, stream); break;
    case 4: ok = w8_launch<256, 128, 4, 2, 3, 1>(q, flags, stream); break;
    case 5: ok = w8_launch<128, 256, 2, 4, 3, 1>(q, flags, stream); break;
    default: return 0;
  }
  if (ok && cfg_out) *cfg_out = cfg;
  return ok ? 1 : 0;
}
```

### espresso_amd/kernels.py

```python
import ctypes
from typing import Optional

import torch

from . import _lib
from ._lib import EaGemmParams, check

ACT_NONE, ACT_RELU, ACT_SILU = 0, 1, 2
_ACT = {None: 0, "none": 0, "relu": 1, "silu": 2, "swish": 2}


def _stream():
    return ctypes.c_void_p(torch._C._cuda_getCurrentRawStream(torch._C._cuda_getDevice()))


def _p(t: Optional[torch.Tensor]):
    if t is None:
        return None
    if not t.is_cuda:
        raise RuntimeError("espresso_amd kernels need device tensors (no CPU path)")
    return ctypes.c_void_p(t.data_ptr())


def drop_params(p: float):
    if p <= 0.0:
        return 0, 1.0
    thr = min(int(p * 4294967296.0), 4294967295)
    return thr, 1.0 / (1.0 - p)


def gemm(
    A: torch.Tensor,
    B: torch.Tensor,
    C: torch.Tensor,
    M: int,
    N: int,
    K: int,
    *,
    lda: int,
    ldb: int,
    ldc: int,
    a_kstrided: bool = False,
    b_kstrided: bool = False,
    batch: int = 1,
    zdiv: int = 1,
    sA=(0, 0),
    sB=(0, 0),
    sC=(0, 0),
    a_off: int = 0,
    b_off: int = 0,
    c_off: int = 0,
    bias: Optional[torch.Tensor] = None,
    act=None,
    alpha: float = 1.0,
    out_scale: float = 1.0,
    resid: Optional[torch.Tensor] = None,
    ldr: int = 0,
    sR=(0, 0),
    r_off: int = 0,
    C2: Optional[torch.Tensor] = None,
    ldc2: int = 0,
    aux: Optional[torch.Tensor] = None,
    ldaux: int = 0,
    sX=(0, 0),
    accumulate: bool = False,
    drop_p: float = 0.0,
    drop_seed: int = 0,
    splitk: int = 1,
    qsplit=None,
):
    assert A.dtype == torch.bfloat16 and B.dtype == torch.bfloat16
    assert C.dtype in (torch.bfloat16, torch.float32)
    p = EaGemmParams()
    p.A = A.data_ptr() + 2 * a_off
    p.B = B.data_ptr() + 2 * b_off
    p.C = C.data_ptr() + C.element_size() * c_off
    p.C2 = (C2.data_ptr() + 2 * c_off) if C2 is not None else None
    if bias is not None:
        assert bias.dtype == torch.float32
        p.bias = bias.data_ptr()
    if resid is not None:
        assert resid.dtype in (torch.bfloat16, torch.float32)
        p.resid = resid.data_ptr() + resid.element_size() * r_off
        p.resid_f32 = 1 if resid.dtype == torch.float32 else 0
    if aux is not None:
        assert aux.dtype == torch.bfloat16
        p.aux = aux.data_ptr()
    p.M, p.N, p.K, p.batch, p.zdiv = M, N, K, batch, zdiv
    p.a_kstrided, p.b_kstrided = int(a_kstrided), int(b_kstrided)
    p.c_f32 = 1 if C.dtype == torch.float32 else 0
    p.accumulate = int(accumulate)
    p.act = _ACT[act] if not isinstance(act, int) else act
    p.lda, p.ldb, p.ldc, p.ldc2, p.ldr, p.ldaux = lda, ldb, ldc, ldc2, ldr, ldaux
    p.sA_hi, p.sA_lo = sA
    p.sB_hi, p.sB_lo = sB
    p.sC_hi, p.sC_lo = sC
    p.sR_hi, p.sR_lo = sR
    p.sX_hi, p.sX_lo = sX
    p.alpha, p.out_scale = alpha, out_scale
    thr, scale = drop_params(drop_p)
    p.drop_seed, p.drop_thr, p.drop_scale = drop_seed, thr, scale
    p.splitk = max(1, int(splitk))
    ws = None
    if p.splitk > 1:
        ws = torch.empty(p.splitk * batch * M * N, dtype=torch.float32, device=C.device)
        p.workspace = ws.data_ptr()
    if qsplit is not None:
        q_u, q_v, pos_u, pos_v, qn, ld_q, qscale = qsplit
        assert q_u.dtype == torch.bfloat16 and (q_v is None or q_v.dtype == torch.bfloat16)
        assert (pos_u is None or pos_u.dtype == torch.float32) and (pos_v is None or pos_v.dtype == torch.float32)
        p.q_u, p.q_v, p.pos_u, p.pos_v = _p(q_u), _p(q_v), _p(pos_u), _p(pos_v)
        p.qsplit_n, p.ld_q, p.qscale = int(qn), int(ld_q), float(qscale)
    check(_lib.lib().ea_gemm_bf16(ctypes.byref(p), _stream()), "ea_gemm_bf16")
    return C


def layernorm_fwd(x, gamma, beta, eps=1e-5, row_zero=None, drop_p=0.0, drop_seed=0, save_stats=True, out_f32=False):
    M, C = x.shape
    assert x.dtype == torch.bfloat16 and x.is_contiguous()
    y = torch.empty(M, C, dtype=torch.float32, device=x.device) if out_f32 else torch.empty_like(x)
    mean = torch.empty(M, dtype=torch.float32, device=x.device) if save_stats else None
    rstd = torch.empty(M, dtype=torch.float32, device=x.device) if save_stats else None
    thr, scale = drop_params(drop_p)
    fn = _lib.lib().ea_layernorm_fwd_f32out if out_f32 else _lib.lib().ea_layernorm_fwd
    check(fn(_p(x), _p(gamma), _p(beta), _p(y), _p(mean), _p(rstd), M, C, eps, _p(row_zero), drop_seed, thr, scale, _stream()),
          "ea_layernorm_fwd")
    return y, mean, rstd


def layernorm_bwd(x, dy, gamma, mean, rstd, dgamma, dbeta, row_zero=None, drop_p=0.0, drop_seed=0, dx_add=None):
    M, C = x.shape
    assert dy.is_contiguous() and dy.dtype in (torch.bfloat16, torch.float32)
    dx = torch.empty_like(x)
    thr, scale = drop_params(drop_p)
    ws = torch.empty(_lib.lib().ea_layernorm_bwd_workspace_bytes(M, C) // 4, dtype=torch.float32, device=x.device)
    fn = _lib.lib().ea_layernorm_bwd_f32dy if dy.dtype == torch.float32 else _lib.lib().ea_layernorm_bwd
    check(fn(_p(x), _p(dy), _p(gamma), _p(mean), _p(rstd), _p(dx), _p(dgamma), _p(dbeta), M, C, _p(row_zero), drop_seed, thr, scale,
             _p(dx_add), _p(ws), _stream()), "ea_layernorm_bwd")
    return dx


def cast_f32_to_bf16(src, dst=None):
    if dst is None:
        dst = torch.empty(src.shape, dtype=torch.bfloat16, device=src.device)
    check(_lib.lib().ea_cast_f32_to_bf16(_p(src), _p(dst), src.numel(), _stream()), "ea_cast_f32_to_bf16")
    return dst


def cast_f32_to_bf16_rows(src, ld_dst):
    M, N = src.shape
    assert src.dtype == torch.float32 and src.stride(1) == 1 and ld_dst >= N
    dst = torch.empty(M, ld_dst, dtype=torch.bfloat16, device=src.device)
    check(_lib.lib().ea_cast_f32_to_bf16_rows(_p(src), src.stride(0), _p(dst), ld_dst, M, N, _stream()), "ea_cast_f32_to_bf16_rows")
    return dst if ld_dst == N else dst[:, :N]


def cast_bf16_to_f32(src, dst=None):
    if dst is None:
        dst = torch.empty(src.shape, dtype=torch.float32, device=src.device)
    check(_lib.lib().ea_cast_bf16_to_f32(_p(src), _p(dst), src.numel(), _stream()), "ea_cast_bf16_to_f32")
    return dst


def scale_dropout(x, a=1.0, y=None, b=0.0, drop_p=0.0, drop_seed=0, out=None):
    assert x.dtype == torch.bfloat16 and x.is_contiguous()
    if out is None:
        out = torch.empty_like(x)
    thr, scale = drop_params(drop_p)
    check(_lib.lib().ea_scale_dropout_bf16(_p(x), _p(y), _p(out), x.numel(), a, b, drop_seed, thr, scale, _stream()),
          "ea_scale_dropout_bf16")
    return out


def colsum(X, out, M, N, ld):
    assert X.dtype == torch.bfloat16 and out.dtype == torch.float32
    check(_lib.lib().ea_colsum_bf16(_p(X), _p(out), M, N, ld, _stream()), "ea_colsum_bf16")
    return out


def colsum_ptr(X_ptr: int, out, M, N, ld):
    check(_lib.lib().ea_colsum_bf16(ctypes.c_void_p(X_ptr), _p(out), M, N, ld, _stream()), "ea_colsum_bf16")
    return out


def zero_rows(x, row_zero):
    M, C = x.shape
    check(_lib.lib().ea_zero_rows_bf16(_p(x), _p(row_zero), M, C, _stream()), "ea_zero_rows_bf16")
    return x


def relpos_q_prep(qkv, ldq, u, v, M, C, scaling, want_qv=True):
    qu = torch.empty(M, C, dtype=torch.bfloat16, device=qkv.device)
    qv = torch.empty(M, C, dtype=torch.bfloat16, device=qkv.device) if want_qv else None
    check(_lib.lib().ea_relpos_q_prep(_p(qkv), ldq, _p(u), _p(v), _p(qu), _p(qv), M, C, scaling, _stream()),
          "ea_relpos_q_prep")
# ... 49 lines not shown
    dBD = torch.empty(H * B * T, Rp, dtype=torch.bfloat16, device=qu.device) if relpos else None
    D = torch.empty(H * B, T, dtype=torch.float32, device=qu.device)
    thr, scale = drop_params(drop_p)
    check(
        _lib.lib().ea_flash_attention_bwd(_p(qu), _p(qv), ldq, _p(k), _p(v), ldkv, _p(pp), ldpp, _p(key_len), _p(out), _p(dout),
                                          C, _p(lse), _p(D), _p(t1), _p(t2), C, _p(dBD), Rp, _p(dk), _p(dv), lddkv, H, B, T, S,
                                          dh, int(causal), scaling, drop_seed, thr, scale, _p(keep_bits), _p(dq), lddq,
                                          _stream()),
        "ea_flash_attention_bwd",
    )
    return t1, t2, dBD


def relpos_softmax_bwd(P, dPd, H, B, T, S, ld_p, ld_dp, ld_bd, want_bd=True, drop_p=0.0, drop_seed=0):
    dAC = torch.empty(H * B * T, ld_p, dtype=torch.bfloat16, device=P.device)
    dBD = torch.empty(H * B * T, ld_bd, dtype=torch.bfloat16, device=P.device) if want_bd else None
    thr, scale = drop_params(drop_p)
    check(
        _lib.lib().ea_relpos_softmax_bwd(_p(P), _p(dPd), _p(dAC), _p(dBD), H, B, T, S, ld_p, ld_dp, ld_bd, drop_seed,
                                         thr, scale, _stream()),
        "ea_relpos_softmax_bwd",
    )
    return dAC, dBD


def add2_strided(a, lda, b, ldb, out, ldo, M, C, out_off=0):
    check(
        _lib.lib().ea_add2_strided_bf16(_p(a), lda, _p(b), ldb, ctypes.c_void_p(out.data_ptr() + 2 * out_off), ldo, M,
                                        C, _stream()),
        "ea_add2_strided_bf16",
    )
    return out


def glu_dwconv_fwd(Y, w, B, T, C, KW, stats):
    U = torch.empty(B * T, C, dtype=torch.bfloat16, device=Y.device)
    Z = torch.empty(B * T, C, dtype=torch.bfloat16, device=Y.device)
    check(_lib.lib().ea_glu_dwconv_fwd(_p(Y), _p(w), _p(U), _p(Z), _p(stats), B, T, C, KW, _stream()),
          "ea_glu_dwconv_fwd")
    return U, Z


def bn_finalize(stats, C, n, eps, momentum, running_mean=None, running_var=None):
    mean_rstd = torch.empty(2, C, dtype=torch.float32, device=stats.device)
    check(_lib.lib().ea_bn_finalize(_p(stats), _p(mean_rstd), _p(running_mean), _p(running_var), C, float(n), eps,
                                    momentum, _stream()), "ea_bn_finalize")
    return mean_rstd


def bn_from_running(running_mean, running_var, eps):
    C = running_mean.numel()
    mean_rstd = torch.empty(2, C, dtype=torch.float32, device=running_mean.device)
    check(_lib.lib().ea_bn_from_running(_p(running_mean), _p(running_var), _p(mean_rstd), C, eps, _stream()),
          "ea_bn_from_running")
    return mean_rstd


def bn_act_fwd(Z, mean_rstd, gamma, beta, act):
    M, C = Z.shape
    H = torch.empty_like(Z)
    check(_lib.lib().ea_bn_act_fwd(_p(Z), _p(mean_rstd), _p(gamma), _p(beta), _p(H), M, C, _ACT[act], _stream()),
          "ea_bn_act_fwd")
    return H


def conv1_bn_bwd(X, Z, dH, mean_rstd, gamma, beta, dgamma, dbeta, dW, dbias, B, T, F, CO, sy, sx, act, training=True):
    from . import functional as _F

    red = _F._pool_zeros((2, CO), torch.float32, Z.device)
    check(_lib.lib().ea_conv1_bn_bwd(_p(X), _p(Z), _p(dH), _p(mean_rstd), _p(gamma), _p(beta), _p(red), _p(dgamma), _p(dbeta), _p(dW),
                                     _p(dbias), B, T, F, CO, sy, sx, _ACT[act], int(training), _stream()), "ea_conv1_bn_bwd")


def bn_act_bwd(Z, dH, mean_rstd, gamma, beta, dgamma, dbeta, act, training=True):
    M, C = Z.shape
    from . import functional as _F

    red = _F._pool_zeros((2, C), torch.float32, Z.device)
    dZ = torch.empty_like(Z)
    check(
        _lib.lib().ea_bn_act_bwd(_p(Z), _p(dH), _p(mean_rstd), _p(gamma), _p(beta), _p(red), _p(dZ), _p(dgamma),
                                 _p(dbeta), M, C, _ACT[act], int(training), _stream()),
        "ea_bn_act_bwd",
    )
    return dZ


def glu_dwconv_bwd(dZ, Y, U, w, dw, B, T, C, KW):
    dY = torch.empty(B * T, 2 * C, dtype=torch.bfloat16, device=Y.device)
    ws = torch.empty(int(_lib.lib().ea_dwconv_wgrad_workspace_bytes(B, T, C, KW)), dtype=torch.uint8, device=Y.device)
    check(_lib.lib().ea_glu_dwconv_bwd(_p(dZ), _p(Y), _p(U), _p(w), _p(dY), _p(dw), _p(ws), B, T, C, KW, _stream()),
          "ea_glu_dwconv_bwd")
    return dY


def conv1_fwd(X, W, bias, B, T, F, CO, sy, sx, stats):
    To, Fo = (T - 1) // sy + 1, (F - 1) // sx + 1
    Z = torch.empty(B * To * Fo, CO, dtype=torch.bfloat16, device=X.device)
    check(_lib.lib().ea_conv1_fwd(_p(X), _p(W), _p(bias), _p(Z), _p(stats), B, T, F, CO, sy, sx, _stream()),
          "ea_conv1_fwd")
    return Z


def conv1_wgrad(X, dZ, dW, dbias, B, T, F, CO, sy, sx):
    check(_lib.lib().ea_conv1_wgrad(_p(X), _p(dZ), _p(dW), _p(dbias), B, T, F, CO, sy, sx, _stream()), "ea_conv1_wgrad")


def conv3x3_fwd(X, W16, bias, B, T, F, Cin, Cout, sy, sx, stats=None):
    To, Fo = (T - 1) // sy + 1, (F - 1) // sx + 1
    Z = torch.empty((B * To * Fo, Cout), dtype=torch.bfloat16, device=X.device)
    check(_lib.lib().ea_conv3x3_fwd(_p(X), _p(W16), _p(bias), _p(Z), _p(stats), B, T, F, Cin, Cout, sy, sx, _stream()), "ea_conv3x3_fwd")
    return Z


def conv3x3_dgrad(dZ, Wd16, B, T, F, Cin, Cout, sy, sx):
    dX = torch.empty((B * T * F, Cin), dtype=torch.bfloat16, device=dZ.device)
    check(_lib.lib().ea_conv3x3_dgrad(_p(dZ), _p(Wd16), _p(dX), B, T, F, Cin, Cout, sy, sx, _stream()), "ea_conv3x3_dgrad")
    return dX


def conv3x3_wgrad(X, dZ, dW, B, T, F, Cin, Cout, sy, sx, param_layout=False):
    lib = _lib.lib()
    nb = lib.ea_conv3x3_wgrad_workspace_bytes(B, T, F, Cin, Cout, sy, sx)
    ws = torch.empty(nb, dtype=torch.uint8, device=X.device)
    fn = lib.ea_conv3x3_wgrad_param_layout if param_layout else lib.ea_conv3x3_wgrad
    check(fn(_p(X), _p(dZ), _p(dW), _p(ws), B, T, F, Cin, Cout, sy, sx, _stream()), "ea_conv3x3_wgrad")
    return dW


def im2col3x3(A, B, T, F, C, sy, sx):
    To, Fo = (T - 1) // sy + 1, (F - 1) // sx + 1
    col = torch.empty(B * To * Fo, 9 * C, dtype=torch.bfloat16, device=A.device)
    check(_lib.lib().ea_im2col3x3(_p(A), _p(col), B, T, F, C, sy, sx, _stream()), "ea_im2col3x3")
    return col


def col2im3x3(dcol, B, T, F, C, sy, sx):
    dA = torch.empty(B * T * F, C, dtype=torch.bfloat16, device=dcol.device)
    check(_lib.lib().ea_col2im3x3(_p(dcol), _p(dA), B, T, F, C, sy, sx, _stream()), "ea_col2im3x3")
    return dA


def colstats(X, stats):
    M, C = X.shape
    check(_lib.lib().ea_colstats_bf16(_p(X), _p(stats), M, C, _stream()), "ea_colstats_bf16")
    return stats


def log_softmax(x, M, V, ld):
    out = torch.empty(M, V, dtype=torch.float32, device=x.device)
    if x.dtype == torch.float32:
        check(_lib.lib().ea_log_softmax_f32(_p(x), ld, _p(out), M, V, _stream()), "ea_log_softmax_f32")
    else:
        assert x.dtype == torch.bfloat16
        check(_lib.lib().ea_log_softmax_bf16(_p(x), ld, _p(out), M, V, _stream()), "ea_log_softmax_bf16")
    return out


def ctc_loss_fwd(lprobs, targets, in_len, tgt_len, B, T, V, Lmax, blank):
    assert lprobs.dtype == torch.float32 and lprobs.is_contiguous()
    assert targets.dtype == torch.int32 and in_len.dtype == torch.int32 and tgt_len.dtype == torch.int32
    dev = lprobs.device
    nll = torch.empty(B, dtype=torch.float32, device=dev)
    ws = torch.empty(int(_lib.lib().ea_ctc_workspace_bytes(B, T, Lmax)), dtype=torch.uint8, device=dev)
    check(
        _lib.lib().ea_ctc_loss(_p(lprobs), _p(targets), _p(in_len), _p(tgt_len), _p(nll), _p(ws), B, T, V, Lmax, blank,
# ... 702 lines not shown
```

### include/espresso_amd.h

```cpp
#ifndef ESPRESSO_AMD_H
#define ESPRESSO_AMD_H

#include <stdint.h>

#ifdef __cplusplus
extern "C" {
#endif

typedef struct ihipStream_t* ea_stream_t;

int ea_version(void);

enum { EA_ACT_NONE = 0, EA_ACT_RELU = 1, EA_ACT_SILU = 2 };

typedef struct EaGemmParams {
  const void* A;
  const void* B;
  void* C;
  void* C2;
  const float* bias;
  const void* resid;
  const void* aux;
  int M, N, K, batch, zdiv;
  int a_kstrided, b_kstrided, c_f32, accumulate, resid_f32, act;
  long lda, ldb, ldc, ldc2, ldr, ldaux;
  long sA_hi, sA_lo, sB_hi, sB_lo, sC_hi, sC_lo, sR_hi, sR_lo, sX_hi, sX_lo;
  float alpha, out_scale;
  uint64_t drop_seed;
  uint32_t drop_thr;
  float drop_scale;
  int splitk, kchunk;
  void* workspace;
  void* q_u;
  void* q_v;
  const float* pos_u;
  const float* pos_v;
  long ld_q;
  int qsplit_n;
  float qscale;
} EaGemmParams;

int ea_gemm_bf16(const EaGemmParams* p, ea_stream_t stream);
long ea_gemm_splitk_workspace_bytes(int M, int N, int batch, int splitk);
int ea_set_gemm_variant(int v);
int ea_set_gemm_xcd_swizzle(int mask);
int ea_set_gemm_glds(int stages);
long ea_set_gemm_nt_store_min_bytes(long bytes);
int ea_set_gemm_w8(int mode);
int ea_gemm_profile_enable(int on);
long ea_gemm_profile_read(double* total_ms, double* total_flops);
int ea_gemm_profile_bytes(double* total_bytes);
long ea_gemm_profile_dump(const char* path);

#define EA_WGRAD_MAX 16
typedef struct EaWgradProblem {
  const void* dy;
  const void* x;
  float* dW;
  float* dbias;
  int M, N, K;
  long ld_dy, ld_x, ldw;
} EaWgradProblem;
typedef struct EaWgradGroup {
  int count;
  EaWgradProblem p[EA_WGRAD_MAX];
} EaWgradGroup;
int ea_wgrad_group(const EaWgradGroup* group, ea_stream_t stream);
int ea_set_wgrad_transposing_reads(int on);
int ea_set_wgrad_w8(int mode);

int ea_layernorm_fwd(const void* x, const float* gamma, const float* beta, void* y, float* mean, float* rstd,
                     int M, int C, float eps, const uint8_t* row_zero, uint64_t drop_seed, uint32_t drop_thr,
                     float drop_scale, ea_stream_t stream);
int ea_layernorm_fwd_f32out(const void* x, const float* gamma, const float* beta, float* y, float* mean, float* rstd,
                            int M, int C, float eps, const uint8_t* row_zero, uint64_t drop_seed, uint32_t drop_thr,
                            float drop_scale, ea_stream_t stream);
int ea_layernorm_bwd_f32dy(const void* x, const float* dy, const float* gamma, const float* mean, const float* rstd,
                           void* dx, float* dgamma, float* dbeta, int M, int C, const uint8_t* row_zero,
                           uint64_t drop_seed, uint32_t drop_thr, float drop_scale, const void* dx_add,
                           void* workspace, ea_stream_t stream);
long ea_layernorm_bwd_workspace_bytes(int M, int C);
int ea_layernorm_bwd(const void* x, const void* dy, const float* gamma, const float* mean, const float* rstd,
                     void* dx, float* dgamma, float* dbeta, int M, int C, const uint8_t* row_zero,
                     uint64_t drop_seed, uint32_t drop_thr, float drop_scale, const void* dx_add,
                     void* workspace, ea_stream_t stream);
int ea_layernorm_bwd_dx(const void* x, const void* dy, const float* gamma, const float* mean, const float* rstd, void* dx,
                        float* dgamma, float* dbeta, int M, int C, const uint8_t* row_zero, uint64_t drop_seed,
                        uint32_t drop_thr, float drop_scale, const void* dx_add, void* workspace, ea_stream_t stream);
int ea_layernorm_param_reduce(const void* workspace, float* dgamma, float* dbeta, int M, int C, ea_stream_t stream);
#define EA_LNRED_MAX 8
typedef struct EaLnReduceItem { const void* workspace; float* dgamma; float* dbeta; int M, C; } EaLnReduceItem;
typedef struct EaLnReduceGroup { int count; EaLnReduceItem item[EA_LNRED_MAX]; } EaLnReduceGroup;
int ea_layernorm_param_reduce_group(const EaLnReduceGroup* group, ea_stream_t stream);
int ea_layernorm_bwd_dx2(const void* x, const void* dy, const float* gamma, const float* mean, const float* rstd, void* dx,
                         float* dgamma, float* dbeta, int M, int C, const void* dx_add, void* workspace, void* out2, float a2,
                         uint64_t seed2, uint32_t thr2, float scale2, ea_stream_t stream);
int ea_layernorm_fwd2(const void* x, const float* g1, const float* b1, void* y1, float* mean1, float* rstd1, const float* g2,
                      const float* b2, void* y2, float* mean2, float* rstd2, int M, int C, float eps, ea_stream_t stream);
int ea_layernorm_bwd2_dx(const void* x1, const void* dy1, const float* gamma1, const float* mean1, const float* rstd1,
                         const void* dx_add, void* ws1, const void* x2, const float* gamma2, const float* mean2, const float* rstd2,
                         void* ws2, void* dx, int M, int C, void* out2, float a2, uint64_t seed2, uint32_t thr2, float scale2,
                         ea_stream_t stream);

int ea_cast_f32_to_bf16(const float* src, void* dst, long n, ea_stream_t stream);
int ea_transpose_bf16_batch(const void* const* src, void* const* dst, const int* rows, const int* cols, int n, ea_stream_t stream);
int ea_audio_probe(const char* path, long* num_samples, int* sample_rate, int* channels, int* bits);
long ea_audio_read_i16(const char* path, int16_t* dst, long capacity, int* sample_rate);
int ea_audio_verify(const char* path);
int ea_audio_read_batch_i16(const char* const* paths, int n, int16_t* dst, const long* offsets, int num_threads, long* lengths,
                            int* sample_rates);

int ea_cast_f32_to_bf16_rows(const float* src, long ld_src, void* dst, long ld_dst, long M, int N, ea_stream_t stream);
int ea_cast_bf16_to_f32(const void* src, float* dst, long n, ea_stream_t stream);
int ea_scale_dropout_bf16(const void* x, const void* y, void* out, long n, float a, float b, uint64_t seed,
                          uint32_t thr, float inv_keep, ea_stream_t stream);
int ea_colsum_bf16(const void* X, float* out, int M, int N, long ld, ea_stream_t stream);
int ea_embedding_fwd(const int* tokens, const int* positions, const float* W, const float* pos_table, void* out, int M,
                     int C, float scale, ea_stream_t stream);
int ea_embedding_bwd(const int* tokens, const void* dy, float* dW, int M, int C, float scale, int pad_idx,
                     ea_stream_t stream);
int ea_zero_rows_bf16(void* x, const uint8_t* row_zero, int M, int C, ea_stream_t stream);

int ea_flash_attention_supported(int dh, int T, int S, int relpos);
int ea_flash_attention_fwd(const void* qu, const void* qv, long ldq, const void* k, const void* v, long ldkv,
                           const void* pp, long ldpp, const int* key_len, void* out, long ldo, float* lse, int H, int B,
                           int T, int S, int dh, int causal, uint64_t drop_seed, uint32_t drop_thr, float drop_scale,
                           void* keep_bits, ea_stream_t stream);
long ea_flash_keep_bits_bytes(int H, int B, int T);
int ea_set_flash_relpos(int on);
int ea_flash_keep_bits(void* keep_bits, int H, int B, int T, uint64_t drop_seed, uint32_t drop_thr, ea_stream_t stream);
int ea_flash_attention_bwd(const void* qu, const void* qv, long ldq, const void* k, const void* v, long ldkv,
                           const void* pp, long ldpp, const int* key_len, const void* out, const void* dout, long ldo,
                           const float* lse, float* D, void* t1, void* t2, long ldt, void* dBD, int ld_bd, void* dk,
                           void* dv, long lddkv, int H, int B, int T, int S, int dh, int causal, float scaling,
                           uint64_t drop_seed, uint32_t drop_thr, float drop_scale, const void* keep_bits,
                           void* dq, long lddq, ea_stream_t stream);

int ea_relpos_q_prep(const void* qkv, long ldq, const float* u, const float* v, void* qu, void* qv, int M,
                     int C, float scaling, ea_stream_t stream);
int ea_relpos_softmax_fwd(const float* ac, const float* bd, const int* key_len, const float* attn_mask, void* P,
                          void* Pd, int H, int B, int T, int S, int ld_ac, int ld_bd, int ld_p, int causal,
                          uint64_t drop_seed, uint32_t drop_thr, float drop_scale, ea_stream_t stream);
int ea_relpos_softmax_bwd(const void* P, const float* dPd, void* dAC, void* dBD, int H, int B, int T, int S,
                          int ld_p, int ld_dp, int ld_bd, uint64_t drop_seed, uint32_t drop_thr,
                          float drop_scale, ea_stream_t stream);
int ea_add2_strided_bf16(const void* a, long lda, const void* b, long ldb, void* out, long ldo, int M, int C,
                         ea_stream_t stream);

int ea_glu_dwconv_fwd(const void* Y, const float* w, void* U, void* Z, double* stats, int B, int T, int C, int KW,
                      ea_stream_t stream);
int ea_bn_finalize(const double* stats, float* mean_rstd, float* running_mean, float* running_var, int C, float n,
                   float eps, float momentum, ea_stream_t stream);
int ea_bn_from_running(const float* running_mean, const float* running_var, float* mean_rstd, int C, float eps,
                       ea_stream_t stream);
int ea_bn_act_fwd(const void* Z, const float* mean_rstd, const float* gamma, const float* beta, void* H, long M,
                  int C, int act, ea_stream_t stream);
int ea_bn_act_bwd(const void* Z, const void* dH, const float* mean_rstd, const float* gamma, const float* beta,
                  float* red, void* dZ, float* dgamma, float* dbeta, long M, int C, int act, int training,
                  ea_stream_t stream);
long ea_dwconv_wgrad_workspace_bytes(int B, int T, int C, int KW);
int ea_glu_dwconv_bwd(const void* dZ, const void* Y, const void* U, const float* w, void* dY, float* dw,
                      void* wgrad_ws, int B, int T, int C, int KW, ea_stream_t stream);
int ea_dwconv_bwd_weight(const void* dZ, const void* U, float* dw, void* wgrad_ws, int B, int T, int C, int KW, ea_stream_t stream);
int ea_bn_act_fwd_train(const void* Z, const double* stats, float* mean_rstd, float* running_mean, float* running_var,
                        const float* gamma, const float* beta, void* H, long M, int C, int act, float n, float eps,
                        float momentum, double* zero_next, int zero_n, ea_stream_t stream);
int ea_bn_act_bwd_fused(const void* Z, const void* dH, const float* mean_rstd, const float* gamma, const float* beta,
                        float* red, void* dZ, float* dgamma, float* dbeta, long M, int C, int act, int training,
                        float* zero_next, int zero_n, ea_stream_t stream);
int ea_bn_glu_dwconv_bwd_fused(const void* Z, const void* dH, const float* mean_rstd, const float* gamma, const float* beta, float* red,
                               void* dZ, float* dgamma, float* dbeta, int act, int training, float* zero_next, int zero_n,
                               const void* Y, const float* w, void* dY, int B, int T, int C, int KW, ea_stream_t stream);
int ea_bn_param_grad(const float* red, float* dgamma, float* dbeta, int C, ea_stream_t stream);
int ea_conv1_bn_bwd(const float* X, const void* Z, const void* dH, const float* mean_rstd, const float* gamma, const float* beta,
                    float* red, float* dgamma, float* dbeta, float* dW, float* dbias, int B, int T, int F, int CO, int sy, int sx,
                    int act, int training, ea_stream_t stream);

int ea_conv1_fwd(const float* X, const float* W, const float* bias, void* Z, double* stats, int B, int T, int F,
                 int CO, int sy, int sx, ea_stream_t stream);
int ea_conv1_wgrad(const float* X, const void* dZ, float* dW, float* dbias, int B, int T, int F, int CO, int sy,
                   int sx, ea_stream_t stream);
int ea_conv3x3_fwd(const void* X, const void* W, const float* bias, void* Z, double* stats, int B, int T, int F, int Cin,
                   int Cout, int sy, int sx, ea_stream_t stream);
int ea_conv3x3_dgrad(const void* dZ, const void* Wd, void* dX, int B, int T, int F, int Cin, int Cout, int sy, int sx,
                     ea_stream_t stream);
long ea_conv3x3_wgrad_workspace_bytes(int B, int T, int F, int Cin, int Cout, int sy, int sx);
int ea_conv3x3_wgrad(const void* X, const void* dZ, float* dW, void* workspace, int B, int T, int F, int Cin, int Cout, int sy,
                     int sx, ea_stream_t stream);
int ea_conv3x3_wgrad_param_layout(const void* X, const void* dZ, float* dW, void* workspace, int B, int T, int F, int Cin, int Cout,
                                  int sy, int sx, ea_stream_t stream);
int ea_im2col3x3(const void* A, void* col, int B, int T, int F, int C, int sy, int sx, ea_stream_t stream);
int ea_col2im3x3(const void* dcol, void* dA, int B, int T, int F, int C, int sy, int sx, ea_stream_t stream);
int ea_colstats_bf16(const void* X, double* stats, long M, int C, ea_stream_t stream);

int ea_log_softmax_f32(const float* in, long ld_in, float* out, long M, int V, ea_stream_t stream);
int ea_log_softmax_bf16(const void* in, long ld_in, float* out, long M, int V, ea_stream_t stream);
long ea_ctc_workspace_bytes(int B, int T, int Lmax);
int ea_ctc_loss(const float* lprobs, const int* targets, const int* in_len, const int* tgt_len, float* nll,
                void* workspace, int B, int T, int V, int Lmax, int blank, ea_stream_t stream);
int ea_ctc_grad(const float* lprobs, const void* workspace, const float* nll, const int* targets,
                const int* in_len, const int* tgt_len, void* dlogits, long ld_out, int dlogits_bf16, int B, int T,
                int V, int Lmax, int blank, float grad_scale, const float* grad_scale_dev, int zero_infinity,
                ea_stream_t stream);
int ea_ctc_greedy_decode(const void* x, long ld, int x_bf16, const int* in_len, int* best, float* bestv, int* tokens,
                         int* align, int* out_len, float* score, int B, int T, int V, int blank, int pad,
                         ea_stream_t stream);
long ea_ctc_prefix_beam_workspace_bytes(int B, int T, int beam);
int ea_ctc_prefix_beam_step(const void* x, long ld, int x_bf16, const int* in_len, void* workspace, const float* lm_rows,
                            long ld_lm, int* lm_parent, int* lm_token, void* lm_keep, int B, int T, int V, int beam, int K,
                            int blank, float lm_weight, float ins_bonus, int t0, int t1, ea_stream_t stream);
int ea_ctc_prefix_beam_finish(void* workspace, const float* lm_rows, long ld_lm, float lm_weight, float ins_bonus, int eos,
                              int B, int T, int beam, int nbest, int pad, int* tokens, int* lengths, float* scores, int* nhyp,
                              ea_stream_t stream);
long ea_ctc_prefix_beam_bias_workspace_bytes(int B, int T, int beam);
int ea_ctc_prefix_beam_bias_step(const void* x, long ld, int x_bf16, const int* in_len, void* workspace, const float* lm_rows,
                                 long ld_lm, int* lm_parent, int* lm_token, void* lm_keep, const int* cg_nodes,
                                 const int* cg_edges, const int* cg_root, int cg_n_nodes, int cg_n_edges, int B, int T, int V,
                                 int beam, int K, int blank, float lm_weight, float ins_bonus, int t0, int t1, ea_stream_t stream);
int ea_ctc_prefix_beam_bias_finish(void* workspace, const float* lm_rows, long ld_lm, float lm_weight, float ins_bonus, int eos,
                                   const int* cg_nodes, int cg_n_nodes, int B, int T, int beam, int nbest, int pad, int* tokens,
                                   int* lengths, float* scores, int* nhyp, ea_stream_t stream);
int ea_context_graph_score_host(const int* nodes_host, const int* edges_host, const int* root_host, int n_nodes, int n_edges,
                                int V, const int* tokens_host, const int* lens_host, int N, int L, float* running_host,
                                float* final_host, int* q_host);
int ea_context_graph_score(const int* nodes, const int* edges, const int* root, int n_nodes, int n_edges, int V,
                           const int* tokens, const int* lens, int N, int L, float* running, float* final_bias, int* q_out,
                           ea_stream_t stream);
long ea_rnnt_frame_beam_workspace_bytes(int B, int T, int beam);
int ea_rnnt_frame_beam_step(const float* logits, long ld, const float* lm_rows, long ld_lm, int lm_no_blank, const int* in_len,
                            void* workspace, int* parent, int* token, void* keep, int B, int T, int V, int beam, int K, int blank,
                            int eos, float temperature, float lm_weight, int t, ea_stream_t stream);
int ea_rnnt_frame_beam_finish(void* workspace, int B, int T, int beam, int nbest, int pad, int normalize, int* tokens,
                              int* lengths, float* scores, int* nhyp, ea_stream_t stream);
long ea_rnnt_frame_beam_stream_state_bytes(int max_frames, int beam);
int ea_rnnt_frame_beam_stream_reset(void* state, const int* slots, int n, int max_streams, int max_frames, int beam,
                                    ea_stream_t stream);
int ea_rnnt_frame_beam_stream_step(const float* logits, long ld, const float* lm_rows, long ld_lm, int lm_no_blank,
                                   const int* slot_idx, const int* n_new, int j, int n, void* state, int* parent, int* token,
                                   void* keep, int max_streams, int max_frames, int V, int beam, int K, int blank, int eos,
                                   float temperature, float lm_weight, ea_stream_t stream);
int ea_rnnt_frame_beam_stream_finish(const void* state, const int* slots, int n, int max_streams, int max_frames, int beam,
                                     int nbest, int pad, int normalize, int max_u, int* tokens, int* lengths, float* scores,
                                     int* nhyp, ea_stream_t stream);
int ea_rnnt_frame_beam_stream_partial(const void* state, const int* slots, int n, int max_streams, int max_frames, int beam,
                                      int pad, int max_u, int* tokens, int* lengths, float* scores, int* stable_len,
                                      ea_stream_t stream);
int ea_ngram_create(const char* path, void* handle_host, char* err_host, long err_cap);
int ea_ngram_destroy(void* handle);
int ea_ngram_info(const void* handle, int* meta_host, long* counts_host);
long ea_ngram_vocab(const void* handle, char* buf_host, long cap);
long ea_ngram_records(const void* handle, int order, int* ngrams_host, float* logp_host, float* bow_host);
int ea_ngram_upload(void* handle);
int ea_ngram_score_host(const void* handle, const int* ctx_host, const int* words_host, int N, float* out_host);
int ea_ngram_score(const void* handle, const int* ctx, const int* words, int N, float* out, ea_stream_t stream);
long ea_ctc_lexicon_beam_workspace_bytes(int B, int T, int beam);
int ea_ctc_lexicon_beam_search(const void* x, long ld, int x_bf16, const int* in_len, void* workspace, const void* ngram,
                               const int* trie_off, const int* trie_tok, const int* trie_child, const int* trie_word,
                               const float* trie_smear, const void* word_start, int space, int B, int T, int V, int beam, int K,
                               int blank, float lm_weight, float word_score, float ins_bonus, int nbest, int pad, int* tokens,
                               int* lengths, float* scores, int* nhyp, ea_stream_t stream);
long ea_ctc_lexicon_stream_state_bytes(int max_frames, int beam);
int ea_ctc_lexicon_stream_reset(void* state, const int* slots, int n, const void* ngram, int max_streams, int max_frames,
                                int beam, ea_stream_t stream);
int ea_ctc_lexicon_stream_step(const void* x, long ld, int x_bf16, long total_rows, const int* slot_idx, const int* n_new,
                               const int* row_off, int n, void* state, const void* ngram, const int* trie_off,
                               const int* trie_tok, const int* trie_child, const int* trie_word, const float* trie_smear,
                               const void* word_start, int space, int max_streams, int max_frames, int V, int beam, int K,
                               int blank, float lm_weight, float word_score, float ins_bonus, ea_stream_t stream);
int ea_ctc_lexicon_stream_finish(const void* state, const int* slots, int n, const void* ngram, const int* trie_word,
                                 const float* trie_smear, int max_streams, int max_frames, int beam, float lm_weight,
                                 float word_score, float ins_bonus, int nbest, int pad, int max_u, int* tokens, int* lengths,
                                 float* scores, int* nhyp, ea_stream_t stream);
int ea_ctc_lexicon_stream_partial(const void* state, const int* slots, int n, int max_streams, int max_frames, int beam,
                                  float ins_bonus, int pad, int max_u, int* tokens, int* lengths, float* scores, int* stable_len,
                                  ea_stream_t stream);
int ea_label_smoothed_ce(const void* logits, long ld, int logits_bf16, const int* target, float* out_loss,
                         void* dlogits, long ld_out, int dlogits_bf16, long M, int V, int pad_idx, float eps,
                         float grad_scale, int smoothing, const float* prior, int tgt_len, ea_stream_t stream);

int ea_fbank_batch(const float* wav, const long* offsets, int B, const float* window, const float* twiddle,
                   const int* mel_start, const int* mel_len, const int* mel_woff, const float* mel_w,
                   const float* cmvn_mean, const float* cmvn_std, float* feat, float* utt_sum, int* out_len,
                   int Tmax, int nmel, int frame_len, int frame_shift, float preemph, float log_floor,
                   ea_stream_t stream);
int ea_fbank_batch_i16(const int16_t* wav, const long* offsets, int B, const float* window, const float* twiddle,
                   const int* mel_start, const int* mel_len, const int* mel_woff, const float* mel_w,
                   const float* cmvn_mean, const float* cmvn_std, float* feat, float* utt_sum, int* out_len,
                   int Tmax, int nmel, int frame_len, int frame_shift, float preemph, float log_floor,
                   ea_stream_t stream);
int ea_specaugment(float* feat, const int* lengths, const float* utt_sum, const int* fmask, const int* tmask,
                   int nf, int nt, int B, int Tmax, int nmel, int use_mean, float mask_value, ea_stream_t stream);

int ea_feature_stats(const float* feat, const int* lengths, double* acc, int B, int Tmax, int nmel, ea_stream_t stream);

int ea_grad_sumsq(const float* g, long n, float* out, ea_stream_t stream);
int ea_clip_coef(const float* sumsq, float pre_scale, const float* denom_dev, float max_norm, float* coef,
                 ea_stream_t stream);
int ea_adam_step(float* p, float* g, float* m, float* v, void* p_bf16, long n, const float* coef, float lr,
                 float beta1, float beta2, float eps, float weight_decay, int step, int zero_grad,
                 ea_stream_t stream);

typedef struct EaFfnParams { const float *ln_g, *ln_b; const void* w1; const float* b1; const void* w2; const float* b2; } EaFfnParams;
typedef struct EaFfnGrads { float *ln_g, *ln_b, *w1, *b1, *w2, *b2; } EaFfnGrads;
typedef struct EaAttnParams {
  const float *ln_g, *ln_b; const void* wqkv; const float* bqkv; const void* wo; const float* bo;
  const float *pos_u, *pos_v; const void* wpos;
} EaAttnParams;
typedef struct EaAttnGrads { float *ln_g, *ln_b, *wqkv, *bqkv, *wo, *bo, *pos_u, *pos_v, *wpos; } EaAttnGrads;
typedef struct EaConvParams {
  const float *ln_g, *ln_b; const void* pw1; const float* dw; const float *bn_g, *bn_b; float *bn_rm, *bn_rv; const void* pw2;
} EaConvParams;
typedef struct EaConvGrads { float *ln_g, *ln_b, *pw1, *dw, *bn_g, *bn_b, *pw2; } EaConvGrads;
typedef struct EaLayerGrads { EaFfnGrads ffn1; EaAttnGrads attn; EaConvGrads conv; EaFfnGrads ffn2; float *final_ln_g, *final_ln_b; } EaLayerGrads;
typedef struct EaConformerLayer {
  EaFfnParams ffn1; EaAttnParams attn; EaConvParams conv; EaFfnParams ffn2; const float *final_ln_g, *final_ln_b;
  EaLayerGrads grads;
  void* wt;
} EaConformerLayer;
typedef struct EaLayerShape {
  int B, T, C, H, F, KW, training; float p_drop, p_act, p_attn; uint64_t seed; int has_attn_mask;
  int scratch_clean;
  int pos_mode, act;
  int S;
  int defer;
  int wt_fresh;
} EaLayerShape;

enum {
  EA_SITE_FFN1_ACT = 0, EA_SITE_FFN1_OUT = 1, EA_SITE_ATTN_PROBS = 2, EA_SITE_ATTN_OUT = 3, EA_SITE_CONV_OUT = 4,
  EA_SITE_FFN2_ACT = 5, EA_SITE_FFN2_OUT = 6, EA_SITE_CROSS_PROBS = 7, EA_SITE_CROSS_OUT = 8
};
uint64_t ea_layer_dropout_seed(uint64_t layer_seed, int site);
int ea_dropout_hash_host(uint64_t seed, uint64_t idx0, long n, uint32_t* out);

int ea_set_backward_overlap(int on);
int ea_set_backward_deferred(int on);
int ea_set_backward_deferred_inline(int on);
int ea_backward_flush(ea_stream_t stream);
int ea_streams_share_queue(ea_stream_t a, ea_stream_t b);
int ea_side_stream_report(int* rejected, int* unprobed);
int ea_conformer_layer_workspace(const EaLayerShape* shape, long* saved_bytes, long* scratch_bytes);
int ea_conformer_layer_refresh_wt(const EaConformerLayer* layer, const EaLayerShape* shape, ea_stream_t stream);
int ea_conformer_layer_fwd(const EaConformerLayer* layer, const EaLayerShape* shape, const void* x_in, void* x_out,
                           const int* key_len, const float* attn_mask, const void* pe, void* saved, long saved_bytes,
                           void* scratch, long scratch_bytes, ea_stream_t stream);
int ea_conformer_layer_bwd(const EaConformerLayer* layer, const EaLayerShape* shape, const void* x_in, const void* dy,
                           void* dx, const int* key_len, const void* pe, void* saved, long saved_bytes, void* scratch,
                           long scratch_bytes, ea_stream_t stream);
typedef struct EaLayerChain {
  const EaConformerLayer* next; void* next_saved; long next_saved_bytes; int ln1_done;
  const EaConformerLayer* prev; void* prev_saved; long prev_saved_bytes; uint64_t prev_seed; void* prev_pre;
  int final_ln_done; const void* pre_in;
} EaLayerChain;
int ea_conformer_layer_fwd_chained(const EaConformerLayer* layer, const EaLayerShape* shape, const EaLayerChain* chain, const void* x_in,
                                   void* x_out, const int* key_len, const float* attn_mask, const void* pe, void* saved,
                                   long saved_bytes, void* scratch, long scratch_bytes, ea_stream_t stream);
int ea_conformer_layer_bwd_chained(const EaConformerLayer* layer, const EaLayerShape* shape, const EaLayerChain* chain, const void* x_in,
                                   const void* dy, void* dx, const int* key_len, const void* pe, void* saved, long saved_bytes,
                                   void* scratch, long scratch_bytes, ea_stream_t stream);
typedef struct EaStackLayer { const EaConformerLayer* layer; EaLayerShape shape; void* saved; long saved_bytes; void* x_in; } EaStackLayer;
int ea_conformer_stack_fwd(const EaStackLayer* L, int n, void* x_out, const int* key_len, const float* attn_mask, const void* pe,
                           void* scratch, long scratch_bytes, int chain, ea_stream_t stream);
int ea_conformer_stack_bwd(const EaStackLayer* L, int n, const void* dy, void* dx, void* const* dbuf, void* const* pre,
                           const int* key_len, const void* pe, void* scratch, long scratch_bytes, int chain, ea_stream_t stream);
int ea_transformer_layer_workspace(const EaLayerShape* shape, long* saved_bytes, long* scratch_bytes);
int ea_transformer_layer_fwd(const EaConformerLayer* layer, const EaLayerShape* shape, const void* x_in, void* x_out,
                             const int* key_len, const float* attn_mask, const void* pe, void* saved, long saved_bytes,
                             void* scratch, long scratch_bytes, ea_stream_t stream);
int ea_transformer_layer_bwd(const EaConformerLayer* layer, const EaLayerShape* shape, const void* x_in, const void* dy,
                             void* dx, const int* key_len, const void* pe, float* dpe, void* saved, long saved_bytes,
                             void* scratch, long scratch_bytes, ea_stream_t stream);
typedef struct EaXAttnParams { const float *ln_g, *ln_b; const void* wq; const float* bq; const void* wkv; const float* bkv; const void* wo; const float* bo; } EaXAttnParams;
typedef struct EaXAttnGrads { float *ln_g, *ln_b, *wq, *bq, *wkv, *bkv, *wo, *bo; } EaXAttnGrads;
typedef struct EaDecoderLayer {
  EaAttnParams self_attn; EaXAttnParams cross; EaFfnParams ffn;
  EaAttnGrads g_self; EaXAttnGrads g_cross; EaFfnGrads g_ffn;
  void* wt;
} EaDecoderLayer;
int ea_decoder_layer_workspace(const EaLayerShape* shape, long* saved_bytes, long* scratch_bytes);
int ea_decoder_layer_fwd(const EaDecoderLayer* layer, const EaLayerShape* shape, const void* x_in, const void* enc, void* x_out,
                         const int* enc_len, void* saved, long saved_bytes, void* scratch, long scratch_bytes, ea_stream_t stream);
int ea_decoder_layer_bwd(const EaDecoderLayer* layer, const EaLayerShape* shape, const void* x_in, const void* enc, const void* dy,
                         void* dx, void* denc, const int* enc_len, void* saved, long saved_bytes, void* scratch, long scratch_bytes,
                         ea_stream_t stream);
int ea_set_flash_attention(int on);
int ea_set_fused_predrop(int on);

int ea_softmax_cumsum(const float* logits, long ld, const uint8_t* row_mask, float* cumsum, float* lp_tok, int N, int V, int tok,
                      ea_stream_t stream);
int ea_lookahead_advance(int* nodes, const int* prev_tok, const int* children, const int* prev_subword, int N, int D,
                         int space_idx, int root_id, ea_stream_t stream);
int ea_lookahead_logprobs(const int* nodes, const int* prev_tok, const float* cumsum, const float* lp_word_eos, const int* children,
                          const int* prev_subword, const int* word_idx, const int* word_set, float* out, int N, int Vw, int Vs,
                          int D, float oov_penalty, int open_vocab, int word_unk, int sub_space, int sub_eos, int sub_pad,
                          ea_stream_t stream);

int ea_multilevel_lm_step(const float* word_logits, long ldw, const float* sub_logits, long lds, const int* prev_tok,
                          const float* prev_out, float* word_lp, float* cum, int* nodes, float* out, const int* children,
                          const int* prev_subword, const int* word_idx, int N, int Vw, int Vs, int D, float subword_weight,
                          float log_oov_penalty, int first, int open_vocab, int word_eos, int word_unk, int sub_space, int sub_eos,
                          int root_id, ea_stream_t stream);

int ea_lstm_cell_fwd(const float* gates_pre, long ldg, const float* c_prev, float* c_out, float* h_out_f32, void* h_out_bf16,
                     long ldh, float* gates_act, const uint8_t* keep_row, const float* h_prev_f32, int frozen_out_zero, int B,
                     int H, ea_stream_t stream);
int ea_lstm_cell_bwd(const void* dh_bf16, long ld_dh, const float* dh_f32, const float* dc_in, const float* gates_act,
                     const float* c_prev, const float* c, void* dgates, long lddg, float* dc_prev, const uint8_t* frozen, int B,
                     int H, ea_stream_t stream);
int ea_lstm_seq_supported(int B, int H);
int ea_lstm_seq_fwd(const float* gx, const void* w_hh, const void* h0, const float* c0, const uint8_t* frozen, void* hs, float* cs,
                    float* act, float* h_last, unsigned* counter, int B, int U, int H, int reverse, int frozen_out_zero,
                    ea_stream_t stream);
int ea_lstm_seq_bwd(const void* dhs, const float* dh_last, const float* dc_last, const float* act, const float* cs, const float* c0,
                    const uint8_t* frozen, const void* w_hhT, void* dG, float* dh0, float* dc0, unsigned* counter, int B, int U,
                    int H, int reverse, ea_stream_t stream);
int ea_bahdanau_fwd(const void* qp, const void* key, const void* value, const float* nv, const float* bias, const int* len,
                    float* p_out, void* ctx, long ldc, int T, int B, int A, int Cv, const int* kv_col, int Bkv,
                    ea_stream_t stream);
int ea_bahdanau_bwd(const void* dctx, long ldd, const void* qp, const void* key, const void* value, const float* nv,
                    const float* bias, const int* len, const float* p, void* dqp, float* dkey_acc, float* dvalue_acc,
// ... 65 lines not shown
```

Before: 5.336 audio-hours/sec.

## Fuse BatchNorm backward reductions into the pw2 dgrad GEMM epilogue

The conv-module backward now computes the BatchNorm backward channel sums (sum of d and d*xhat through SiLU) inside the epilogue of the pw2 dgrad GEMM. It uses cross-lane reductions, LDS partials and atomics into the ring reduction buffer. A presummed path then skips the separate bn_bwd_reduce kernel and goes straight to the apply or fused GLU/dwconv step. This removes one full read pass over Z and dH per layer, at the cost of heavier GEMM epilogues, extra LDS in the w8 kernel, and float atomics that make the sums non-deterministic.

```diff
diff --git a/espresso_amd/_lib.py b/espresso_amd/_lib.py
--- a/espresso_amd/_lib.py
+++ b/espresso_amd/_lib.py
@@ -63,6 +63,12 @@
         ("ld_q", ctypes.c_long),
         ("qsplit_n", ctypes.c_int),
         ("qscale", ctypes.c_float),
+        ("bn_z", ctypes.c_void_p),
+        ("bn_mr", ctypes.c_void_p),
+        ("bn_g", ctypes.c_void_p),
+        ("bn_b", ctypes.c_void_p),
+        ("bn_red", ctypes.c_void_p),
+        ("bn_act", ctypes.c_int),
     ]
 
 
diff --git a/espresso_amd/csrc/convmodule.hip b/espresso_amd/csrc/convmodule.hip
--- a/espresso_amd/csrc/convmodule.hip
+++ b/espresso_amd/csrc/convmodule.hip
@@ -923,6 +923,13 @@
   if (M <= 0) return 0;
   if (C % 8) return -2;
   launch_bn_bwd_reduce(Z, dH, mean_rstd, gamma, beta, red, M, C, act, stream);
+  return ea_bn_act_bwd_apply(Z, dH, mean_rstd, gamma, beta, red, dZ, dgamma, dbeta, M, C, act, training, zero_next, zero_n, stream);
+}
+extern "C" int ea_bn_act_bwd_apply(const void* Z, const void* dH, const float* mean_rstd, const float* gamma, const float* beta,
+                                   const float* red, void* dZ, float* dgamma, float* dbeta, long M, int C, int act, int training,
+                                   float* zero_next, int zero_n, hipStream_t stream) {
+  if (M <= 0) return 0;
+  if (C % 8) return -2;
   hipLaunchKernelGGL(bn_act_bwd_apply_kernel, dim3(egrid_ch(M * (C / 8), C / 8)), dim3(256), 0, stream, (const bf16_t*)Z,
                      (const bf16_t*)dH, mean_rstd, gamma, beta, red, (bf16_t*)dZ, M, C, act, training ? (float)M : 0.f, dgamma, dbeta,
                      zero_next, zero_n);
@@ -984,18 +991,35 @@
   if (!dw) return EA_CHECK_LAUNCH();
   return ea_dwconv_bwd_weight(dZ, U, dw, wgrad_ws, B, T, C, KW, stream);
 }
+static int bn_glu_dwconv_bwd(const void* Z, const void* dH, const float* mean_rstd, const float* gamma, const float* beta, float* red,
+                             void* dZ, float* dgamma, float* dbeta, int act, int training, float* zero_next, int zero_n, const void* Y,
+                             const float* w, void* dY, int B, int T, int C, int KW, bool presummed, hipStream_t stream);
 extern "C" int ea_bn_glu_dwconv_bwd_fused(const void* Z, const void* dH, const float* mean_rstd, const float* gamma, const float* beta,
                                           float* red, void* dZ, float* dgamma, float* dbeta, int act, int training, float* zero_next,
                                           int zero_n, const void* Y, const float* w, void* dY, int B, int T, int C, int KW,
                                           hipStream_t stream) {
+  return bn_glu_dwconv_bwd(Z, dH, mean_rstd, gamma, beta, red, dZ, dgamma, dbeta, act, training, zero_next, zero_n, Y, w, dY, B, T, C, KW,
+                           false, stream);
+}
+extern "C" int ea_bn_glu_dwconv_bwd_presummed(const void* Z, const void* dH, const float* mean_rstd, const float* gamma,
+                                              const float* beta, float* red, void* dZ, float* dgamma, float* dbeta, int act, int training,
+                                              float* zero_next, int zero_n, const void* Y, const float* w, void* dY, int B, int T, int C,
+                                              int KW, hipStream_t stream) {
+  return bn_glu_dwconv_bwd(Z, dH, mean_rstd, gamma, beta, red, dZ, dgamma, dbeta, act, training, zero_next, zero_n, Y, w, dY, B, T, C, KW,
+                           true, stream);
+}
+static int bn_glu_dwconv_bwd(const void* Z, const void* dH, const float* mean_rstd, const float* gamma, const float* beta, float* red,
+                             void* dZ, float* dgamma, float* dbeta, int act, int training, float* zero_next, int zero_n, const void* Y,
+                             const float* w, void* dY, int B, int T, int C, int KW, bool presummed, hipStream_t stream) {
   if (B <= 0 || T <= 0) return 0;
   const long M = (long)B * T;
   static const bool fuse = [] { const char* e = getenv("EA_BN_GLU_BWD_FUSED"); return e && e[0] == '1'; }();
   if (!fuse || C % CT != 0) {
-    const int rc = ea_bn_act_bwd_fused(Z, dH, mean_rstd, gamma, beta, red, dZ, dgamma, dbeta, M, C, act, training, zero_next, zero_n, stream);
+    const int rc = presummed ? ea_bn_act_bwd_apply(Z, dH, mean_rstd, gamma, beta, red, dZ, dgamma, dbeta, M, C, act, training, zero_next, zero_n, stream)
+                             : ea_bn_act_bwd_fused(Z, dH, mean_rstd, gamma, beta, red, dZ, dgamma, dbeta, M, C, act, training, zero_next, zero_n, stream);
     return rc ? rc : ea_glu_dwconv_bwd(dZ, Y, nullptr, w, dY, nullptr, nullptr, B, T, C, KW, stream);
   }
-  launch_bn_bwd_reduce(Z, dH, mean_rstd, gamma, beta, red, M, C, act, stream);
+  if (!presummed) launch_bn_bwd_reduce(Z, dH, mean_rstd, gamma, beta, red, M, C, act, stream);
   BnBwdFuse fb{(const bf16_t*)Z, (const bf16_t*)dH, mean_rstd, gamma, beta, red, (bf16_t*)dZ, training ? (float)M : 0.f, act, dgamma, dbeta,
                zero_next, zero_n};
   dim3 grid(C / CT, (T + TTILE - 1) / TTILE, B);
diff --git a/espresso_amd/csrc/engine.hip b/espresso_amd/csrc/engine.hip
--- a/espresso_amd/csrc/engine.hip
+++ b/espresso_amd/csrc/engine.hip
@@ -5,6 +5,7 @@
 
 #include <functional>
 #include <cstdio>
+#include <atomic>
 #include <map>
 #include <mutex>
 #include <vector>
@@ -193,6 +194,10 @@
   G& resid(const void* r, long ldr) { p.resid = r; p.ldr = ldr; return *this; }
   G& c2(void* c, long ld) { p.C2 = c; p.ldc2 = ld; return *this; }
   G& aux(const void* x, long ld) { p.aux = x; p.ldaux = ld; return *this; }
+  G& bnsum(const void* Z, const float* mr, const float* gamma, const float* beta, int act, float* red) {
+    p.bn_z = Z; p.bn_mr = mr; p.bn_g = gamma; p.bn_b = beta; p.bn_act = act; p.bn_red = red;
+    return *this;
+  }
   G& drop(float pr, uint64_t seed) { p.drop_thr = drop_thr(pr); p.drop_scale = drop_scale(pr); p.drop_seed = seed; return *this; }
   bool qsplit(void* q_u, void* q_v, const float* pos_u, const float* pos_v, int n, long ld_q, float s) {
     static const bool off = getenv("EA_NO_QSPLIT") != nullptr;
@@ -249,6 +254,8 @@
 }
 static bool g_defer_default = true;
 static bool g_defer_inline = false;
+static bool g_bn_bwd_epilogue = [] { const char* e = getenv("EA_BN_BWD_EPILOGUE"); return !(e && e[0] == '0'); }();
+static std::atomic<long> g_bn_bwd_epilogue_calls{0};
 static void run_deferred(Ctx& c, int half) {
   if (c.dry || !c.df) return;
   Deferred& d = *c.df;
@@ -797,11 +804,22 @@
   fork(c);
   wgrad(c, g, C, s.Hh, C, gw.pw2, M, C, C);
   uint16_t* dH = sc.get<uint16_t>((size_t)M * C);
-  dgrad(c, g, w.pw2, pw2t, dH, M, C, C);
   static const bool bn_fused = getenv("EA_BN_UNFUSED") == nullptr;
   const bool ring = bn_fused && C <= 2048;
   BnRing* R = nullptr;
   if (ring && !c.dry && c.rc == 0 && !(R = bn_ring(c.s, C))) c.rc = -1;
+  bool presummed = false;
+  if (ring && g_bn_bwd_epilogue && pw2t && R && c.rc == 0) {
+    G gd(g, pw2t, dH, M, C, C, C, C, C);
+    gd.bnsum(s.Z, s.mr, w.bn_g, w.bn_b, EA_ACT_SILU, R->red[R->ri]);
+    presummed = ea_gemm_bn_sums_supported(&gd.p) != 0;
+    if (presummed) {
+      gemm(c, gd);
+      if (c.rc != 0) R->dirty = true;
+      else g_bn_bwd_epilogue_calls.fetch_add(1, std::memory_order_relaxed);
+    }
+  }
+  if (!presummed) dgrad(c, g, w.pw2, pw2t, dH, M, C, C);
   float* red = nullptr;
   if (!ring) {
     red = sc.get<float>(2 * C);
@@ -813,8 +831,12 @@
   if (ring) {
     if (R && c.rc == 0) {
       red = R->red[R->ri];
-      RUN(ea_bn_glu_dwconv_bwd_fused(s.Z, dH, s.mr, w.bn_g, w.bn_b, red, dZ, gw.bn_g, gw.bn_b, EA_ACT_SILU, sh.training, R->red[R->ri ^ 1],
-                                     2 * R->cap, s.Y, w.dw, dY, B, T, C, sh.KW, c.s));
+      if (presummed)
+        RUN(ea_bn_glu_dwconv_bwd_presummed(s.Z, dH, s.mr, w.bn_g, w.bn_b, red, dZ, gw.bn_g, gw.bn_b, EA_ACT_SILU, sh.training,
+                                           R->red[R->ri ^ 1], 2 * R->cap, s.Y, w.dw, dY, B, T, C, sh.KW, c.s));
+      else
+        RUN(ea_bn_glu_dwconv_bwd_fused(s.Z, dH, s.mr, w.bn_g, w.bn_b, red, dZ, gw.bn_g, gw.bn_b, EA_ACT_SILU, sh.training, R->red[R->ri ^ 1],
+                                       2 * R->cap, s.Y, w.dw, dY, B, T, C, sh.KW, c.s));
       if (c.rc == 0) R->ri ^= 1;
       else R->dirty = true;
     }
@@ -1175,6 +1197,12 @@
   return old;
 }
 int ea_backward_flush(hipStream_t stream) { return join_all(stream); }
+int ea_set_bn_bwd_epilogue(int on) {
+  const int old = g_bn_bwd_epilogue;
+  g_bn_bwd_epilogue = on != 0;
+  return old;
+}
+long ea_bn_bwd_epilogue_calls(void) { return g_bn_bwd_epilogue_calls.load(std::memory_order_relaxed); }
 int ea_set_backward_deferred_inline(int on) {
   const int old = g_defer_inline;
   g_defer_inline = on != 0;
diff --git a/espresso_amd/csrc/gemm.hip b/espresso_amd/csrc/gemm.hip
--- a/espresso_amd/csrc/gemm.hip
+++ b/espresso_amd/csrc/gemm.hip
@@ -180,9 +180,25 @@
   load_bias8(p, n0 + (tid & 15) * 8, bias8);
   float posu8[8], posv8[8];
   load_pos8(p, n0 + (tid & 15) * 8, posu8, posv8);
-  const int pre_kind = !FAST ? 0 : p.resid ? 1 : p.aux ? 2 : 0;
-  const bf16_t* pre_base = pre_kind == 1 ? reinterpret_cast<const bf16_t*>(p.resid) : reinterpret_cast<const bf16_t*>(p.aux);
-  const long pre_ld = pre_kind == 1 ? p.ldr : p.ldaux;
+  const int pre_kind = !FAST ? 0 : p.resid ? 1 : p.aux ? 2 : p.bn_red ? 3 : 0;
+  const bf16_t* pre_base = pre_kind == 1 ? reinterpret_cast<const bf16_t*>(p.resid)
+                                         : reinterpret_cast<const bf16_t*>(pre_kind == 3 ? p.bn_z : p.aux);
+  const long pre_ld = pre_kind == 1 ? p.ldr : pre_kind == 3 ? (long)p.N : p.ldaux;
+  float bmu[8], brs[8], bga[8], bbe[8], bsa[8], bsb[8];
+  if (FAST && pre_kind == 3) {
+    const int n = n0 + (tid & 15) * 8;
+#pragma unroll
+    for (int h = 0; h < 2; ++h) {
+      const float4 m4 = *reinterpret_cast<const float4*>(p.bn_mr + n + 4 * h), r4 = *reinterpret_cast<const float4*>(p.bn_mr + p.N + n + 4 * h);
+      const float4 g4 = *reinterpret_cast<const float4*>(p.bn_g + n + 4 * h), b4 = *reinterpret_cast<const float4*>(p.bn_b + n + 4 * h);
+      bmu[4 * h] = m4.x; bmu[4 * h + 1] = m4.y; bmu[4 * h + 2] = m4.z; bmu[4 * h + 3] = m4.w;
+      brs[4 * h] = r4.x; brs[4 * h + 1] = r4.y; brs[4 * h + 2] = r4.z; brs[4 * h + 3] = r4.w;
+      bga[4 * h] = g4.x; bga[4 * h + 1] = g4.y; bga[4 * h + 2] = g4.z; bga[4 * h + 3] = g4.w;
+      bbe[4 * h] = b4.x; bbe[4 * h + 1] = b4.y; bbe[4 * h + 2] = b4.z; bbe[4 * h + 3] = b4.w;
+    }
+#pragma unroll
+    for (int e = 0; e < 8; ++e) bsa[e] = bsb[e] = 0.f;
+  }
 #pragma unroll
   for (int half = 0; half < BM_ / 64; ++half) {
     uint4 pre0 = uint4{0, 0, 0, 0}, pre1 = pre0, pre2 = pre0, pre3 = pre0;
@@ -219,10 +235,32 @@
           const float4 x1 = *reinterpret_cast<const float4*>(sC + rl * BN + (tid & 15) * 8 + 4);
           v[0] = x0.x; v[1] = x0.y; v[2] = x0.z; v[3] = x0.w; v[4] = x1.x; v[5] = x1.y; v[6] = x1.z; v[7] = x1.w;
           epilogue_chunk<FAST>(p, z, ks_id, zhi, zlo, coff, m, n, v, bias8, posu8, posv8, vec_ok, (xcd_swizzle & 2) != 0, pre_kind, pre0);
+          if (FAST && pre_kind == 3) {
+            float zz[8];
+            unpack8_bf16(pre0, zz);
+#pragma unroll
+            for (int e = 0; e < 8; ++e) bn_sums_acc(zz[e], bf16_round(v[e]), bmu[e], brs[e], bga[e], bbe[e], p.bn_act, bsa[e], bsb[e]);
+          }
         }
         pre0 = pre1; pre1 = pre2; pre2 = pre3;
       }
     }
+  }
+  if (FAST && pre_kind == 3) {
+#pragma unroll
+    for (int e = 0; e < 8; ++e) { bsa[e] = groups4_sum(bsa[e]); bsb[e] = groups4_sum(bsb[e]); }
+    __syncthreads();
+    if (lane < 16) {
+#pragma unroll
+      for (int e = 0; e < 8; ++e) {
+        sC[(wave * 2 + 0) * BN + lane * 8 + e] = bsa[e];
+        sC[(wave * 2 + 1) * BN + lane * 8 + e] = bsb[e];
+      }
+    }
+    __syncthreads();
+    const int which = tid >> 7, col = tid & (BN - 1);
+    const float a = sC[(0 * 2 + which) * BN + col] + sC[(1 * 2 + which) * BN + col] + sC[(2 * 2 + which) * BN + col] + sC[(3 * 2 + which) * BN + col];
+    atomicAdd(p.bn_red + (long)which * p.N + n0 + col, a);
   }
 }
 
@@ -1011,6 +1049,15 @@
   else hipLaunchKernelGGL((gemm_bf16_kernel<A_KS, B_KS, 128>), grid, dim3(256), 0, stream, q, sw);
 }
 
+extern "C" int ea_gemm_bn_sums_supported(const EaGemmParams* pp) {
+  EaGemmParams q = *pp;
+  auto al = [](const void* p) { return p && (reinterpret_cast<uintptr_t>(p) & 15) == 0; };
+  if (q.splitk < 1) q.splitk = 1;
+  q.kchunk = q.K;
+  return q.M > 0 && q.K > 0 && glds_eligible(q) && fast_epilogue_ok(q) && !q.aux && !q.resid && !q.C2 && !q.q_u && al(q.bn_z) && al(q.bn_mr) &&
+         al(q.bn_g) && al(q.bn_b) && al(q.bn_red) && (long)q.M * q.N < (1L << 31);
+}
+
 extern "C" long ea_gemm_splitk_workspace_bytes(int M, int N, int batch, int splitk) {
   return splitk > 1 ? (long)splitk * batch * M * N * (long)sizeof(float) : 0;
 }
@@ -1027,6 +1074,7 @@
   } else {
     q.qsplit_n = 0;
   }
+  if (q.bn_red && !ea_gemm_bn_sums_supported(&q)) return -4;
   if (q.splitk > 1) {
     if (!q.c_f32 || q.bias || q.resid || q.aux || q.C2 || q.act != EA_ACT_NONE || q.drop_thr || !q.workspace) return -4;
     int chunk = (q.K + q.splitk - 1) / q.splitk;
diff --git a/espresso_amd/csrc/gemm_epilogue.h b/espresso_amd/csrc/gemm_epilogue.h
--- a/espresso_amd/csrc/gemm_epilogue.h
+++ b/espresso_amd/csrc/gemm_epilogue.h
@@ -77,6 +77,32 @@
       for (int e = 0; e < 8; ++e) w[e] = p.pos_v[n + e];
     }
   }
+}
+
+__device__ __forceinline__ void bn_sums_acc(float z, float d, float mu, float rs, float ga, float be, int act, float& sa, float& sb) {
+  const float xh = (z - mu) * rs;
+  const float y = xh * ga + be;
+  d *= act == 2 ? dsilu_f(y) : (act == 1 ? (y > 0.f ? 1.f : 0.f) : 1.f);
+  sa += d;
+  sb += d * xh;
+}
+__device__ __forceinline__ float bf16_round(float v) { return __uint_as_float((uint32_t)f2bf(v) << 16); }
+__device__ __forceinline__ float row16_sum_dpp(float v) {
+  auto dpp = [](float x, auto ctrl) {
+    return __builtin_bit_cast(float, __builtin_amdgcn_update_dpp(0, __builtin_bit_cast(int, x), decltype(ctrl)::value, 0xF, 0xF, false));
+  };
+  using std::integral_constant;
+  v += dpp(v, integral_constant<int, 0xB1>{});
+  v += dpp(v, integral_constant<int, 0x4E>{});
+  v += dpp(v, integral_constant<int, 0x124>{});
+  v += dpp(v, integral_constant<int, 0x128>{});
+  return v;
+}
+__device__ __forceinline__ float groups4_sum(float v) {
+  const auto a = __builtin_amdgcn_permlane16_swap(__float_as_uint(v), __float_as_uint(v), false, false);
+  v = __uint_as_float(a[0]) + __uint_as_float(a[1]);
+  const auto b = __builtin_amdgcn_permlane32_swap(__float_as_uint(v), __float_as_uint(v), false, false);
+  return __uint_as_float(b[0]) + __uint_as_float(b[1]);
 }
 
 template <bool FAST = false>
diff --git a/espresso_amd/csrc/gemm_w8.hip b/espresso_amd/csrc/gemm_w8.hip
--- a/espresso_amd/csrc/gemm_w8.hip
+++ b/espresso_amd/csrc/gemm_w8.hip
@@ -9,7 +9,8 @@
 
 namespace {
 
-enum { W8_PLAIN = 0, W8_QSPLIT = 1, W8_ACT2 = 2, W8_AUX = 3, W8_RESID = 4 };
+enum { W8_PLAIN = 0, W8_QSPLIT = 1, W8_ACT2 = 2, W8_AUX = 3, W8_RESID = 4, W8_BNSUM = 5 };
+__host__ __device__ constexpr int w8_bn_lds_floats(int bn, int wm) { return 4 * bn + 2 * wm * bn; }
 
 __device__ __forceinline__ void ea_keep4(uint64_t seed, uint64_t idx0, uint32_t thr, float inv_keep, float (&k)[4]) {
   const uint32_t lo = (uint32_t)idx0;
@@ -37,7 +38,8 @@
   o[2] = __uint_as_float(w1 << 16); o[3] = __uint_as_float(w1 & 0xffff0000u);
 }
 template <int KIND, int MI, int NJ>
-__device__ __forceinline__ void w8_reg_epilogue(const EaGemmParams& p, const f32x4_t (&acc)[MI][NJ], int m0, int n0, int row0, int col0, bool nt) {
+__device__ __forceinline__ void w8_reg_epilogue(const EaGemmParams& p, const f32x4_t (&acc)[MI][NJ], int m0, int n0, int row0, int col0, bool nt,
+                                                float* bn_lds = nullptr, int bn_cols = 0, int wm = 0, int nwm = 1) {
   static_assert(NJ % 2 == 0, "tiles are stored in pairs");
   const int lane = threadIdx.x & 63, g = lane >> 4, r16 = lane & 15;
   const int nown = n0 + col0 + g * 4;
@@ -63,9 +65,25 @@
       posv4[j][0] = w.x; posv4[j][1] = w.y; posv4[j][2] = w.z; posv4[j][3] = w.w;
     }
   }
-  constexpr bool HAS_OP = KIND == W8_AUX || KIND == W8_RESID;
-  const bf16_t* op_base = KIND == W8_AUX ? reinterpret_cast<const bf16_t*>(p.aux) : reinterpret_cast<const bf16_t*>(p.resid);
-  const long op_ld = KIND == W8_AUX ? p.ldaux : p.ldr;
+  constexpr bool HAS_OP = KIND == W8_AUX || KIND == W8_RESID || KIND == W8_BNSUM;
+  const bf16_t* op_base = reinterpret_cast<const bf16_t*>(KIND == W8_AUX ? p.aux : KIND == W8_BNSUM ? p.bn_z : p.resid);
+  const long op_ld = KIND == W8_AUX ? p.ldaux : KIND == W8_BNSUM ? (long)p.N : p.ldr;
+  constexpr int NBN = KIND == W8_BNSUM ? NJ : 1;
+  float bmu[NBN][4], brs[NBN][4], bga[NBN][4], bbe[NBN][4], bsa[NBN][4], bsb[NBN][4];
+  if (KIND == W8_BNSUM) {
+#pragma unroll
+    for (int j = 0; j < NBN; ++j) {
+      const int c = col0 + j * 16 + g * 4;
+      const float4 m4 = *reinterpret_cast<const float4*>(bn_lds + c), r4 = *reinterpret_cast<const float4*>(bn_lds + bn_cols + c);
+      const float4 g4 = *reinterpret_cast<const float4*>(bn_lds + 2 * bn_cols + c), b4 = *reinterpret_cast<const float4*>(bn_lds + 3 * bn_cols + c);
+      bmu[j][0] = m4.x; bmu[j][1] = m4.y; bmu[j][2] = m4.z; bmu[j][3] = m4.w;
+      brs[j][0] = r4.x; brs[j][1] = r4.y; brs[j][2] = r4.z; brs[j][3] = r4.w;
+      bga[j][0] = g4.x; bga[j][1] = g4.y; bga[j][2] = g4.z; bga[j][3] = g4.w;
+      bbe[j][0] = b4.x; bbe[j][1] = b4.y; bbe[j][2] = b4.z; bbe[j][3] = b4.w;
+#pragma unroll
+      for (int e = 0; e < 4; ++e) bsa[j][e] = bsb[j][e] = 0.f;
+    }
+  }
   uint4 opn[HAS_OP ? NJ / 2 : 1], opc[HAS_OP ? NJ / 2 : 1];
   auto fetch_ops = [&](int i) {
     const int mc = min(m0 + row0 + i * 16 + r16, p.M - 1);
@@ -155,6 +173,14 @@
           }
         }
         out[t] = make_uint2(pack_bf2(v[0], v[1]), pack_bf2(v[2], v[3]));
+        if (KIND == W8_BNSUM) {
+          float d4[4];
+          unpack4_bf16(out[t].x, out[t].y, d4);
+          const int jb = KIND == W8_BNSUM ? j : 0;
+#pragma unroll
+          for (int e = 0; e < 4; ++e)
+            bn_sums_acc(opnd[t][e], mv ? d4[e] : 0.f, bmu[jb][e], brs[jb][e], bga[jb][e], bbe[jb][e], p.bn_act, bsa[jb][e], bsb[jb][e]);
+        }
       }
       const u32x4_t o = w8_swap_pair(out[0], out[1]);
       if (KIND == W8_QSPLIT && n0 + col0 + jp * 32 < p.qsplit_n) {
@@ -171,6 +197,29 @@
         }
       } else if (mv) {
         w8_store16(reinterpret_cast<bf16_t*>(p.C) + (long)m * p.ldc + ns, o, nt);
+      }
+    }
+  }
+  if (KIND == W8_BNSUM) {
+    float* part = bn_lds + 4 * bn_cols;
+#pragma unroll
+    for (int j = 0; j < NBN; ++j) {
+#pragma unroll
+      for (int e = 0; e < 4; ++e) { bsa[j][e] = row16_sum_dpp(bsa[j][e]); bsb[j][e] = row16_sum_dpp(bsb[j][e]); }
+      if (r16 == 0) {
+        const int c = col0 + j * 16 + g * 4;
+        *reinterpret_cast<float4*>(part + wm * bn_cols + c) = make_float4(bsa[j][0], bsa[j][1], bsa[j][2], bsa[j][3]);
+        *reinterpret_cast<float4*>(part + (nwm + wm) * bn_cols + c) = make_float4(bsb[j][0], bsb[j][1], bsb[j][2], bsb[j][3]);
+      }
+    }
+    __syncthreads();
+    const int tid = threadIdx.x;
+    if (tid < 2 * bn_cols) {
+      const int which = tid / bn_cols, col = tid - which * bn_cols;
+      if (n0 + col < p.N) {
+        float a = 0.f;
+        for (int w = 0; w < nwm; ++w) a += part[(which * nwm + w) * bn_cols + col];
+        atomicAdd(p.bn_red + (long)which * p.N + n0 + col, a);
       }
     }
   }
@@ -229,9 +278,19 @@
     b_base[ks] = A_BYTES + w8_off(wn * TN + (lane & 15), ks * 4 + (lane >> 4));
   }
 
+  float* bn_lds = reinterpret_cast<float*>(dsm + NST * STAGE);
+  float bnc[4] = {0.f, 0.f, 0.f, 0.f};
+  if (KIND == W8_BNSUM && tid < BN_ && n0 + tid < p.N) {
+    const int n = n0 + tid;
+    bnc[0] = p.bn_mr[n]; bnc[1] = p.bn_mr[p.N + n]; bnc[2] = p.bn_g[n]; bnc[3] = p.bn_b[n];
+  }
 #pragma unroll
   for (int s = 0; s < NST - 1; ++s)
     if (s < nk) issue(s, s);
+  if (KIND == W8_BNSUM && tid < BN_) {
+#pragma unroll
+    for (int k = 0; k < 4; ++k) bn_lds[k * BN_ + tid] = bnc[k];
+  }
   int stage = 0, fill = NST - 1;
   for (int kt = 0; kt < nk; ++kt) {
     if (kt + NST - 2 < nk) w8_wait_vmcnt<(NST - 2) * (NA + NB)>();
@@ -292,13 +351,18 @@
     fill = fill + 1 == NST ? 0 : fill + 1;
   }
   EA_STAMP(2);
-  w8_reg_epilogue<KIND, MI, NJ>(p, acc, m0, n0, wm * TM, wn * TN, (flags & 2) != 0);
+  if constexpr (KIND == W8_BNSUM) {
+    __syncthreads();
+    w8_reg_epilogue<KIND, MI, NJ>(p, acc, m0, n0, wm * TM, wn * TN, (flags & 2) != 0, bn_lds, BN_, wm, WM_);
+  } else {
+    w8_reg_epilogue<KIND, MI, NJ>(p, acc, m0, n0, wm * TM, wn * TN, (flags & 2) != 0);
+  }
   EA_STAMP(3);
 }
 
 template <int BM_, int BN_, int WM_, int WN_, int NST, int PIPE, int KIND>
 bool w8_launch_kind(const EaGemmParams& q, int flags, hipStream_t stream) {
-  constexpr int bytes = NST * (BM_ + BN_) * 128;
+  constexpr int bytes = NST * (BM_ + BN_) * 128 + (KIND == W8_BNSUM ? w8_bn_lds_floats(BN_, WM_) * (int)sizeof(float) : 0);
   static const bool attr_ok = hipFuncSetAttribute(reinterpret_cast<const void*>(&gemm_w8_kernel<BM_, BN_, WM_, WN_, NST, PIPE, KIND>),
                                                   hipFuncAttributeMaxDynamicSharedMemorySize, bytes) == hipSuccess;
   if (!attr_ok) return false;
@@ -312,6 +376,7 @@
     if (g_gemm_w8 == 1 && !qs) return -1;
     return (q.aux || q.C2 || q.resid || q.drop_thr || q.act != EA_ACT_NONE || q.out_scale != 1.f) ? -1 : W8_QSPLIT;
   }
+  if (q.bn_red) return W8_BNSUM;
   if (q.C2) return (q.aux || q.resid) ? -1 : W8_ACT2;
   if (q.aux) return q.resid ? -1 : W8_AUX;
   return q.resid ? W8_RESID : W8_PLAIN;
@@ -324,6 +389,9 @@
     case W8_ACT2: return w8_launch_kind<BM_, BN_, WM_, WN_, NST, PIPE, W8_ACT2>(q, flags, stream);
     case W8_AUX: return w8_launch_kind<BM_, BN_, WM_, WN_, NST, PIPE, W8_AUX>(q, flags, stream);
     case W8_RESID: return w8_launch_kind<BM_, BN_, WM_, WN_, NST, PIPE, W8_RESID>(q, flags, stream);
+    case W8_BNSUM:
+      if constexpr (BM_ == 128 && BN_ == 128) return w8_launch_kind<BM_, BN_, WM_, WN_, NST, PIPE, W8_BNSUM>(q, flags, stream);
+      else return false;
     default: return false;
   }
 }
diff --git a/espresso_amd/kernels.py b/espresso_amd/kernels.py
--- a/espresso_amd/kernels.py
+++ b/espresso_amd/kernels.py
@@ -68,6 +68,7 @@
     drop_seed: int = 0,
     splitk: int = 1,
     qsplit=None,
+    bn_sums=None,
 ):
     assert A.dtype == torch.bfloat16 and B.dtype == torch.bfloat16
     assert C.dtype in (torch.bfloat16, torch.float32)
@@ -111,6 +112,15 @@
         assert (pos_u is None or pos_u.dtype == torch.float32) and (pos_v is None or pos_v.dtype == torch.float32)
         p.q_u, p.q_v, p.pos_u, p.pos_v = _p(q_u), _p(q_v), _p(pos_u), _p(pos_v)
         p.qsplit_n, p.ld_q, p.qscale = int(qn), int(ld_q), float(qscale)
+    if bn_sums is not None:
+        Z, mr, bn_g, bn_b, bn_act, red = bn_sums
+        assert Z.dtype == torch.bfloat16 and Z.is_contiguous() and Z.shape == (M, N)
+        assert all(t.dtype == torch.float32 and t.is_contiguous() for t in (mr, bn_g, bn_b, red))
+        assert mr.numel() == 2 * N and red.numel() == 2 * N and bn_g.numel() == N and bn_b.numel() == N
+        p.bn_z, p.bn_mr, p.bn_g, p.bn_b, p.bn_red = _p(Z), _p(mr), _p(bn_g), _p(bn_b), _p(red)
+        p.bn_act = _ACT[bn_act] if not isinstance(bn_act, int) else bn_act
+        if not _lib.lib().ea_gemm_bn_sums_supported(ctypes.byref(p)):
+            raise RuntimeError("ea_gemm_bf16: the BatchNorm-sums epilogue does not take this launch (see ea_gemm_bn_sums_supported)")
     check(_lib.lib().ea_gemm_bf16(ctypes.byref(p), _stream()), "ea_gemm_bf16")
     return C
 
@@ -326,6 +336,17 @@
         _lib.lib().ea_bn_act_bwd(_p(Z), _p(dH), _p(mean_rstd), _p(gamma), _p(beta), _p(red), _p(dZ), _p(dgamma),
                                  _p(dbeta), M, C, _ACT[act], int(training), _stream()),
         "ea_bn_act_bwd",
+    )
+    return dZ
+
+
+def bn_act_bwd_apply(Z, dH, mean_rstd, gamma, beta, red, dgamma, dbeta, act, training=True):
+    M, C = Z.shape
+    dZ = torch.empty_like(Z)
+    check(
+        _lib.lib().ea_bn_act_bwd_apply(_p(Z), _p(dH), _p(mean_rstd), _p(gamma), _p(beta), _p(red), _p(dZ), _p(dgamma), _p(dbeta), M, C,
+                                       _ACT[act], int(training), None, 0, _stream()),
+        "ea_bn_act_bwd_apply",
     )
     return dZ
 
diff --git a/include/espresso_amd.h b/include/espresso_amd.h
--- a/include/espresso_amd.h
+++ b/include/espresso_amd.h
@@ -38,9 +38,16 @@
   long ld_q;
   int qsplit_n;
   float qscale;
+  const void* bn_z;
+  const float* bn_mr;
+  const float* bn_g;
+  const float* bn_b;
+  float* bn_red;
+  int bn_act;
 } EaGemmParams;
 
 int ea_gemm_bf16(const EaGemmParams* p, ea_stream_t stream);
+int ea_gemm_bn_sums_supported(const EaGemmParams* p);
 long ea_gemm_splitk_workspace_bytes(int M, int N, int batch, int splitk);
 int ea_set_gemm_variant(int v);
 int ea_set_gemm_xcd_swizzle(int mask);
@@ -168,9 +175,16 @@
 int ea_bn_act_bwd_fused(const void* Z, const void* dH, const float* mean_rstd, const float* gamma, const float* beta,
                         float* red, void* dZ, float* dgamma, float* dbeta, long M, int C, int act, int training,
                         float* zero_next, int zero_n, ea_stream_t stream);
+int ea_bn_act_bwd_apply(const void* Z, const void* dH, const float* mean_rstd, const float* gamma, const float* beta,
+                        const float* red, void* dZ, float* dgamma, float* dbeta, long M, int C, int act, int training,
+                        float* zero_next, int zero_n, ea_stream_t stream);
 int ea_bn_glu_dwconv_bwd_fused(const void* Z, const void* dH, const float* mean_rstd, const float* gamma, const float* beta, float* red,
                                void* dZ, float* dgamma, float* dbeta, int act, int training, float* zero_next, int zero_n,
                                const void* Y, const float* w, void* dY, int B, int T, int C, int KW, ea_stream_t stream);
+int ea_bn_glu_dwconv_bwd_presummed(const void* Z, const void* dH, const float* mean_rstd, const float* gamma, const float* beta,
+                                   float* red, void* dZ, float* dgamma, float* dbeta, int act, int training, float* zero_next,
+                                   int zero_n, const void* Y, const float* w, void* dY, int B, int T, int C, int KW,
+                                   ea_stream_t stream);
 int ea_bn_param_grad(const float* red, float* dgamma, float* dbeta, int C, ea_stream_t stream);
 int ea_conv1_bn_bwd(const float* X, const void* Z, const void* dH, const float* mean_rstd, const float* gamma, const float* beta,
                     float* red, float* dgamma, float* dbeta, float* dW, float* dbias, int B, int T, int F, int CO, int sy, int sx,
@@ -336,6 +350,8 @@
 int ea_set_backward_overlap(int on);
 int ea_set_backward_deferred(int on);
 int ea_set_backward_deferred_inline(int on);
+int ea_set_bn_bwd_epilogue(int on);
+long ea_bn_bwd_epilogue_calls(void);
 int ea_backward_flush(ea_stream_t stream);
 int ea_streams_share_queue(ea_stream_t a, ea_stream_t b);
 int ea_side_stream_report(int* rejected, int* unprobed);
```

Result: no change. 5.355 audio-hours/sec (median of 4 runs) (+0.4%).
